# aexoden/snesimage

Measured on AMD Instinct MI355X. Metric: candidate palettes scored/sec, higher is better.
Workload: dtype f32

## Files before the change

### snesimage_amd/csrc/batch_host.inc

```

struct snesimage_batch {
    std::vector<snesimage_ctx *> ctx;
    int device = 0;
    hipStream_t stream = nullptr;
    static constexpr int kRing = 4;
    snes::BatchArgs *h_args[kRing] = {nullptr, nullptr, nullptr, nullptr}, *d_args[kRing] = {nullptr, nullptr, nullptr, nullptr};
    hipEvent_t used[kRing] = {nullptr, nullptr, nullptr, nullptr};
    uint64_t calls = 0;
    bool busy = false, dead = false;
};

namespace {

int32_t batch_quiesce(snesimage_batch *b) {
    if (b && b->busy) { HIPCHK(hipStreamSynchronize(b->stream)); b->busy = false; }
    return SNES_OK;
}

snes::PrepParams make_prep(snesimage_ctx *c, int mode, int sp, int si) {
    snes::PrepParams P{};
    P.orig = c->d_target; P.tile_pal = c->d_tile_pal; P.pal_rgb8 = c->d_pal_rgb8; P.map = c->d_map; P.pack = c->d_pack; P.packT = c->d_packT; P.packC4 = c->d_packC4; P.packR4 = c->d_packR4;
    P.subC4 = c->d_subC4; P.subR4 = c->d_subR4; P.labpx = c->d_labpx_t; P.pal_lab = c->d_pal_lab;
    P.W = (int)c->W; P.H = (int)c->H; P.sub_size = (int)c->sub_size; P.ncol = c->ncol; P.mode = mode; P.sp = sp; P.si = si; P.perceptual = c->perceptual ? 1 : 0;
    return P;
// ... 16 lines not shown
        auto &sp = c->sp;
        const uint32_t j0 = c->sub_size > 1 ? (index + 1u) % c->sub_size : index;
        a.bcolor = c->d_colors + 3 * (size_t)(palette * c->sub_size + j0); a.btab = sp.cand_tab + 8 * (size_t)(sp.lanes * sp.cap);
        a.win_pack = sp.dpack; a.zero = sp.plist_count; a.nzero = 1;
        DitherParams D{};
        D.orig = c->d_orig; D.tile_pal = c->d_tile_pal; D.pal_rgb8 = c->d_pal_rgb8; D.W = (int)c->W; D.H = (int)c->H; D.sub_size = (int)c->sub_size; D.ncol = c->ncol; D.slot_ci = sp.slot_ci;
        a.Db = D; a.Db.cand_tab = a.btab; a.Db.maps = sp.bmap; a.Db.mapsC4 = sp.bmapC4; a.Db.rec_pack = sp.dpack; a.Db.ck_out = sp.ckd;
        a.Db.excl_sub = (int)palette; a.Db.excl_si = (int)index; a.Db.excl_j0 = (int)j0;
        a.Dc = D; a.Dc.cand_tab = sp.cand_tab; a.Dc.maps = const_cast<uint8_t *>(a.Pc.maps); a.Dc.mapsC4 = const_cast<uint8_t *>(a.Pc.mapsC4);
        a.Dc.first_group = sp.first; a.Dc.first_k0 = 0; a.Dc.rec_in = c->dither_rec ? sp.dpack : nullptr; a.Dc.ck_in = sp.ckd; a.Dc.bmap = sp.bmap; a.Dc.bmapC4 = sp.bmapC4; a.Dc.order = sp.lpt ? sp.order : nullptr;
        if (c->perceptual) {
            a.Db.pal_lab = c->d_pal_lab; a.Db.cand_lab = sp.cand_lab + 3 * (size_t)(sp.lanes * sp.cap); a.Db.lab_eotf = c->d_lab_eotf; a.Db.perceptual = 1; a.Db.rec_lab = sp.rec_lab;
            a.Dc.pal_lab = c->d_pal_lab; a.Dc.cand_lab = sp.cand_lab; a.Dc.lab_eotf = c->d_lab_eotf; a.Dc.perceptual = 1;
        }
    }
    a.method = (int)method; a.n = (int)n; a.slot = (int)(palette * c->sub_size + index); a.channel = (int)channel; a.nes = method == SNES_METHOD_NES ? 1 : 0; a.npx = (int)c->npx;
    return SNES_OK;
}

struct BatchSide { hipStream_t stream; hipEvent_t in, h, v, narrow; bool whole; hipStream_t aux = nullptr; hipEvent_t a_scan = nullptr, a_h0 = nullptr, a_v0 = nullptr; };
int32_t enqueue_batched_scoring(hipStream_t st, const snes::BatchArgs *A, uint32_t K, uint32_t n, snesimage_ctx *c0, const BatchSide *side = nullptr, const int *dead = nullptr, bool member_packs = false) {
    const Geom &G = c0->G;
    const unsigned npx_blocks = (unsigned)((c0->npx + 255) / 256);
    const int s_first = sparse_params(c0, 0).s_first;
    hipStream_t bs = side && side->stream ? side->stream : st;
    const bool split = bs != st;
    const bool dith = c0->dither;
    const bool sub16 = c0->sub_size == 16;
    const bool sub15 = c0->sub_size == 15;
    const bool whole = split && side->whole;
    hipStream_t ps = whole ? bs : st;
    const int *bdead = whole ? nullptr : dead;
    if (!dith) hipLaunchKernelGGL(kb_prep, dim3(npx_blocks, 1, K), dim3(256), 0, ps, A, bdead);
    else {
        if (member_packs) hipLaunchKernelGGL(kb_prep, dim3(npx_blocks, 1, K), dim3(256), 0, ps, A, bdead);
        hipLaunchKernelGGL(kb_dither_prep, dim3(1, 1, K), dim3(64), 0, ps, A, bdead);
        if (c0->perceptual) hipLaunchKernelGGL(kb_dither_base_lab, dim3(1, 1, K), dim3(512), 0, ps, A, bdead);
        else if (sub15) hipLaunchKernelGGL(kb_dither_base<15>, dim3(1, 1, K), dim3(512), 0, ps, A, bdead);
        else if (sub16) hipLaunchKernelGGL(kb_dither_base<16>, dim3(1, 1, K), dim3(512), 0, ps, A, bdead);
        else hipLaunchKernelGGL(kb_dither_base<0>, dim3(1, 1, K), dim3(512), 0, ps, A, bdead);
    }
    hipLaunchKernelGGL(kb_build_plist, dim3(npx_blocks, 1, K), dim3(256), 0, ps, A, bdead);
    hipLaunchKernelGGL(kb_base_down, dim3(down_grid(G), 1, K), dim3(256), 0, ps, A, bdead);
    if (split) { HIPCHK(hipEventRecord(side->in, ps)); HIPCHK(hipStreamWaitEvent(whole ? st : bs, side->in, 0)); }
    const bool quad = (size_t)n * K <= c0->sp.h2q_max;
    if (quad) hipLaunchKernelGGL(kb_sparse_h2q_base, dim3((unsigned)((G.sh[0] / 4 * 3 + 3) / 4), (unsigned)(s_first * kColBuckets), K), dim3(64), h2_lds(c0), bs, A, bdead);
    else hipLaunchKernelGGL(kb_sparse_h2_base, dim3((unsigned)((G.sh[0] / 4 * 3 + 15) / 16), (unsigned)(s_first * kColBuckets), K), dim3(64), h2_lds(c0), bs, A, bdead);
    if (split) HIPCHK(hipEventRecord(side->h, bs));
    if (s_first > 0 && c0->sp.vsplit) hipLaunchKernelGGL(kb_sparse_v_base_split, dim3((unsigned)(G.W >> 6), (unsigned)(3 * s_first), K), dim3(128), 0, bs, A, bdead);
    else if (s_first > 0) hipLaunchKernelGGL(kb_sparse_v_base, dim3(3, (unsigned)s_first, K), dim3(256), 0, bs, A, bdead);
    if (split) HIPCHK(hipEventRecord(side->v, bs));
    if (s_first < G.nscales) hipLaunchKernelGGL(kb_sparse_h, dim3((unsigned)((G.sh[s_first] / 4 * 3 + 15) / 16), (unsigned)((G.nscales - s_first) * kColBuckets), K), dim3(64), 0, bs, A, 1, bdead);
    if (s_first < G.nscales) hipLaunchKernelGGL(kb_sparse_v_base_narrow, dim3(3, (unsigned)(G.nscales - s_first), K), dim3(256), 0, bs, A, bdead);
    if (split) HIPCHK(hipEventRecord(side->narrow, bs));
    hipLaunchKernelGGL(kb_candidate_tables, dim3((n + 63) / 64, 1, K), dim3(64), 0, st, A, dead);
    if (dith && c0->perceptual) {
        hipLaunchKernelGGL(kb_candidate_lab, dim3((n + 63) / 64, 1, K), dim3(64), 0, st, A, dead);
        hipLaunchKernelGGL(kb_dither_first_lab, dim3(n, 1, K), dim3(256), 0, st, A, dead);
        if (c0->sp.lpt) hipLaunchKernelGGL(kb_sparse_order, dim3(1, 1, K), dim3(1024), 0, st, A, dead);
        if (c0->dither4 && (size_t)n * K <= c0->dither4_max) hipLaunchKernelGGL(kb_dither_run4_lab, dim3(n, 1, K), dim3(512), 0, st, A, dead);
        else hipLaunchKernelGGL(kb_dither_run_lab, dim3(n, 1, K), dim3(128), 0, st, A, dead);
        hipLaunchKernelGGL(kb_dither_diff, dim3((n + 3) / 4, 1, K), dim3(1024), 0, st, A, dead);
    } else
    if (c0->perceptual) {
        hipLaunchKernelGGL(kb_candidate_lab, dim3((n + 63) / 64, 1, K), dim3(64), 0, st, A, dead);
        hipLaunchKernelGGL(kb_clear_bitmaps, dim3(64, 1, K), dim3(256), 0, st, A, dead);
        hipLaunchKernelGGL(kb_sparse_scan_lab, dim3(n, 1, K), dim3(256), 0, st, A, dead);
    } else if (dith) {
        hipLaunchKernelGGL(kb_dither_first, dim3((n + 15) / 16, 1, K), dim3(1024), 0, st, A, dead);
        if (c0->sp.lpt) hipLaunchKernelGGL(kb_sparse_order, dim3(1, 1, K), dim3(1024), 0, st, A, dead);
        const bool quad_fs = c0->dither4 && (size_t)n * K <= c0->dither4_max;
        if (quad_fs && sub15) hipLaunchKernelGGL(kb_dither_run4<15>, dim3(n, 1, K), dim3(512), 0, st, A, dead);
        else if (quad_fs && sub16) hipLaunchKernelGGL(kb_dither_run4<16>, dim3(n, 1, K), dim3(512), 0, st, A, dead);
        else if (quad_fs) hipLaunchKernelGGL(kb_dither_run4<0>, dim3(n, 1, K), dim3(512), 0, st, A, dead);
        else if (c0->ditherw && sub15) hipLaunchKernelGGL(kb_dither_runw<15>, dim3((n + 3) / 4, 1, K), dim3(256), 0, st, A, dead);
        else if (c0->ditherw && sub16) hipLaunchKernelGGL(kb_dither_runw<16>, dim3((n + 3) / 4, 1, K), dim3(256), 0, st, A, dead);
        else if (c0->ditherw && c0->sub_size > 1) hipLaunchKernelGGL(kb_dither_runw<0>, dim3((n + 3) / 4, 1, K), dim3(256), 0, st, A, dead);
        else if (sub15) hipLaunchKernelGGL(kb_dither_run<15>, dim3(n, 1, K), dim3(128), 0, st, A, dead);
        else if (sub16) hipLaunchKernelGGL(kb_dither_run<16>, dim3(n, 1, K), dim3(128), 0, st, A, dead);
        else hipLaunchKernelGGL(kb_dither_run<0>, dim3(n, 1, K), dim3(128), 0, st, A, dead);
        hipLaunchKernelGGL(kb_dither_diff, dim3((n + 3) / 4, 1, K), dim3(1024), 0, st, A, dead);
    } else if ((size_t)n * K <= c0->sp.scan4_max) hipLaunchKernelGGL(kb_sparse_scan4, dim3((n + 3) / 4, 1, K), dim3(1024), 0, st, A, dead);
    else hipLaunchKernelGGL(kb_sparse_scan, dim3((n + 15) / 16, 1, K), dim3(1024), 0, st, A, 0, dead);
    const bool two = side && side->aux && !quad && (size_t)n * K >= c0->sp.h0_min && c0->sp.h0_min > 0 && s_first > 0 && c0->sp.down1 && G.nscales > 2;
    if (two) {
        hipStream_t ax = side->aux;
        HIPCHK(hipEventRecord(side->a_scan, st)); HIPCHK(hipStreamWaitEvent(ax, side->a_scan, 0));
        if (split) HIPCHK(hipStreamWaitEvent(ax, side->h, 0));
        size_t gx = ((size_t)n * 8 * 3 + 15) / 16; if (gx > c0->sp.hgrid) gx = c0->sp.hgrid; if (gx < 8) gx = 8;
        hipLaunchKernelGGL(kb_sparse_h2_lists, dim3((unsigned)gx, (unsigned)kColBuckets, K), dim3(64), h2_lds(c0), ax, A, dead, 0);
        if (c0->sp.lpt) hipLaunchKernelGGL(kb_sparse_order, dim3(1, 1, K), dim3(1024), 0, ax, A, dead);
        HIPCHK(hipEventRecord(side->a_h0, ax));
        if (split) HIPCHK(hipStreamWaitEvent(ax, side->v, 0));
        hipLaunchKernelGGL(kb_sparse_v2_scales, dim3(n * 3, 1, K), dim3(256), 0, ax, A, dead, 0);
        HIPCHK(hipEventRecord(side->a_v0, ax));
    }
    if (c0->sp.down1 && G.nscales > 2) {
        hipLaunchKernelGGL(kb_sparse_down1, dim3(n * 8, 1, K), dim3(256), 0, st, A, dead);
        if (c0->sp.down_tiles && G.nscales >= 4) {
            unsigned gt = (n * (unsigned)(G.sh[3] / 4) + SNES_DOWN_TILES_U - 1) / SNES_DOWN_TILES_U; if (gt > c0->sp.tiles_grid) gt = c0->sp.tiles_grid;
            hipLaunchKernelGGL(kb_sparse_down_tiles, dim3(gt, 1, K), dim3(256), 0, st, A, dead);
        } else
        hipLaunchKernelGGL(kb_sparse_down, dim3(n, 1, K), dim3(256), 0, st, A, -2, dead);
    } else hipLaunchKernelGGL(kb_sparse_down, dim3(n, 1, K), dim3(256), 0, st, A, 0, dead);
    if (split) HIPCHK(hipStreamWaitEvent(st, side->h, 0));
    { size_t gx = ((size_t)n * 8 * 3 + 15) / 16; if (gx > c0->sp.hgrid) gx = c0->sp.hgrid; if (gx < 8) gx = 8;
      if (quad) hipLaunchKernelGGL(kb_sparse_h2q, dim3((unsigned)(gx * 4), (unsigned)(s_first * kColBuckets), K), dim3(64), h2_lds(c0), st, A, dead);
      else if (two) { if (s_first > 1) hipLaunchKernelGGL(kb_sparse_h2_lists, dim3((unsigned)gx, (unsigned)((s_first - 1) * kColBuckets), K), dim3(64), h2_lds(c0), st, A, dead, (int)kColBuckets); }
      else hipLaunchKernelGGL(kb_sparse_h2, dim3((unsigned)gx, (unsigned)(s_first * kColBuckets), K), dim3(64), h2_lds(c0), st, A, dead);
      if (s_first < G.nscales) hipLaunchKernelGGL(kb_sparse_h, dim3((unsigned)((gx + 7) / 8), (unsigned)((G.nscales - s_first) * kColBuckets), K), dim3(64), 0, st, A, 0, dead); }
    if (two) {
        HIPCHK(hipStreamWaitEvent(st, side->a_h0, 0));
        if (split) { HIPCHK(hipStreamWaitEvent(st, side->v, 0)); HIPCHK(hipStreamWaitEvent(st, side->narrow, 0)); }
        if (s_first < G.nscales) hipLaunchKernelGGL(kb_sparse_v, dim3((n * 3 + 7) / 8, (unsigned)(G.nscales - s_first), K), dim3(256), 0, st, A, dead);
        if (s_first > 1) hipLaunchKernelGGL(kb_sparse_v2_scales, dim3(n * 3, (unsigned)(s_first - 1), K), dim3(256), 0, st, A, dead, 1);
        HIPCHK(hipStreamWaitEvent(st, side->a_v0, 0));
    } else {
    if (c0->sp.lpt) hipLaunchKernelGGL(kb_sparse_order, dim3(1, 1, K), dim3(1024), 0, st, A, dead);
    if (split) HIPCHK(hipStreamWaitEvent(st, side->v, 0));
    hipLaunchKernelGGL(kb_sparse_v2, dim3(n * 3, (unsigned)s_first, K), dim3(256), 0, st, A, dead);
    if (split) HIPCHK(hipStreamWaitEvent(st, side->narrow, 0));
    if (s_first < G.nscales) hipLaunchKernelGGL(kb_sparse_v, dim3((n * 3 + 7) / 8, (unsigned)(G.nscales - s_first), K), dim3(256), 0, st, A, dead);
    }
    hipLaunchKernelGGL(kb_final_score, dim3((n + 3) / 4, 1, K), dim3(256), 0, st, A, dead);
    HIPCHK(hipGetLastError());
    return SNES_OK;
}

}

extern "C" {

void batch_forget(snesimage_batch *b, snesimage_ctx *c) {
    (void)batch_quiesce(b);
    for (auto *m : b->ctx) m->owner = nullptr;
    (void)c;
    b->dead = true;
}

int32_t snesimage_batch_create(snesimage_ctx **ctxs, uint32_t n, snesimage_batch **out) {
    if (!ctxs || !out || n == 0) return fail(SNES_ERR_ARG, "null pointer or empty batch");
    *out = nullptr;
    snesimage_ctx *c0 = ctxs[0];
    for (uint32_t i = 0; i < n; i++) {
        snesimage_ctx *c = ctxs[i];
        if (!c) return fail(SNES_ERR_ARG, "null context in batch");
        if (c->owner) return fail(SNES_ERR_STATE, "context already belongs to a batch");
        if (c->backdrop) return fail(SNES_ERR_UNSUPPORTED, kBackdropRefused);
        if (c->od_L > 1) return fail(SNES_ERR_ARG, kLevelsRefused);
        if (c->device != c0->device || c->W != c0->W || c->H != c0->H || c->sub_count != c0->sub_count || c->sub_size != c0->sub_size || c->chunk != c0->chunk)
            return fail(SNES_ERR_ARG, "contexts of a batch must share device, image size, palette geometry and chunk");
        if (c->perceptual != c0->perceptual) return fail(SNES_ERR_ARG, "contexts of a batch must share their flags");
        if (!c->sp.enabled || (c->dither && c->sub_size == 1)) return fail(SNES_ERR_UNSUPPORTED, "batched calls cover the group-sparse path (not with SNES_SPARSE=0), and with --dither subpalettes of two entries and more");
        if (c->dither != c0->dither) return fail(SNES_ERR_ARG, "contexts of a batch must share their flags");
        if (!ordered_tables_equal(c, c0)) return fail(SNES_ERR_ARG, "contexts of a batch must share their ordered-dither table");
    }
    std::unique_ptr<snesimage_batch> b(new snesimage_batch());
    b->device = c0->device;
    HIPCHK(hipSetDevice(b->device));
    for (uint32_t i = 0; i < n; i++) {
        snesimage_ctx *c = ctxs[i];
        CHECK(alloc_workspace(c, 1));
        CHECK(ensure_tables(c));
        CHECK(ensure_source(c));
        CHECK(sparse_alloc(c, c->chunk));
        CHECK(ensure_cand_capacity(c, c->chunk));
        if (!c->map_synced) CHECK(do_optimize(c));
        CHECK(ensure_incumbent(c));
    }
    for (uint32_t i = 0; i < n; i++) HIPCHK(hipStreamSynchronize(ctxs[i]->stream));
    HIPCHK(hipStreamCreateWithFlags(&b->stream, hipStreamNonBlocking));
    for (int r = 0; r < snesimage_batch::kRing; r++) {
        HIPCHK(hipHostMalloc(&b->h_args[r], sizeof(snes::BatchArgs) * n));
        HIPCHK(hipMalloc(&b->d_args[r], sizeof(snes::BatchArgs) * n));
        HIPCHK(hipEventCreateWithFlags(&b->used[r], hipEventDisableTiming));
    }
    b->ctx.assign(ctxs, ctxs + n);
    for (auto *c : b->ctx) c->owner = b.get();
    *out = b.release();
    return SNES_OK;
}

void snesimage_batch_destroy(snesimage_batch *b) {
    if (!b) return;
    (void)hipSetDevice(b->device);
    if (b->stream) (void)hipStreamSynchronize(b->stream);
    if (!b->dead) for (auto *c : b->ctx) c->owner = nullptr;
    for (int r = 0; r < snesimage_batch::kRing; r++) {
        if (b->h_args[r]) (void)hipHostFree(b->h_args[r]);
        if (b->d_args[r]) (void)hipFree(b->d_args[r]);
        if (b->used[r]) (void)hipEventDestroy(b->used[r]);
    }
    if (b->stream) (void)hipStreamDestroy(b->stream);
    delete b;
}

int32_t snesimage_batch_sync(snesimage_batch *b) {
    if (!b) return fail(SNES_ERR_ARG, "null batch");
    HIPCHK(hipSetDevice(b->device));
    return batch_quiesce(b);
}

}

namespace {

int32_t batch_call(snesimage_batch *b, uint32_t method, uint32_t palette, uint32_t index, uint32_t channel, const uint64_t *seeds, uint64_t step_id, uint32_t n_random, snes::StepResult *joint) {
    snesimage_ctx *c0 = b->ctx[0];
    CHECK(check_slot(c0, palette, index));
    if (method > 2 || channel > 2) return fail(SNES_ERR_ARG, "bad method or channel");
    const uint32_t n = method_count(method, n_random);
    if (n > c0->chunk) return fail(SNES_ERR_ARG, "a batched call holds at most `chunk` candidates per image");
    HIPCHK(hipSetDevice(b->device));
    const uint32_t K = (uint32_t)b->ctx.size();
    const int r = (int)(b->calls % snesimage_batch::kRing);
    if (b->calls >= (uint64_t)snesimage_batch::kRing) HIPCHK(hipEventSynchronize(b->used[r]));
    snes::BatchArgs *ha = b->h_args[r];
    for (uint32_t i = 0; i < K; i++) {
        snesimage_ctx *c = b->ctx[i];
        if (!c->tables_valid || !c->src_valid || !c->inc_valid) return fail(SNES_ERR_STATE, "a member context was modified outside the batch; call snesimage_batch_sync and recreate the batch");
        CHECK(fill_batch_args(ha[i], c, n, method, palette, index, channel, mix64(seeds[i] ^ (step_id * 0x9E3779B97F4A7C15ull) ^ 0xD1B54A32D192ED03ull)));
        if (n > c->cand_cap) return fail(SNES_ERR_STATE, "a member's candidate list is smaller than the call");
        if (c->dither) { ha[i].prep = make_prep(c, 1, -1, -1); ha[i].prep.zero = nullptr; ha[i].prep.nzero = 0; }
    }
    hipStream_t st = b->stream;
    if (!b->busy) for (auto *c : b->ctx) {
        if (!c->ev_own) HIPCHK(hipEventCreateWithFlags(&c->ev_own, hipEventDisableTiming));
        HIPCHK(hipEventRecord(c->ev_own, c->stream));
        HIPCHK(hipStreamWaitEvent(st, c->ev_own, 0));
    }
    const snes::BatchArgs *A = b->d_args[r];
    HIPCHK(hipMemcpyAsync(b->d_args[r], ha, sizeof(snes::BatchArgs) * K, hipMemcpyHostToDevice, st));
    HIPCHK(hipEventRecord(b->used[r], st));
    hipLaunchKernelGGL(kb_gen_candidates, dim3((n + 63) / 64, 1, K), dim3(64), 0, st, A, (const int *)nullptr);
    CHECK(enqueue_batched_scoring(st, A, K, n, c0, nullptr, nullptr, c0->dither));
    if (joint) hipLaunchKernelGGL(ks_commit, dim3(1), dim3(256), 0, st, A, (int)K, joint);
    else hipLaunchKernelGGL(kb_commit, dim3(1, 1, K), dim3(256), 0, st, A, (const int *)nullptr);
// ... 23 lines not shown
```

### snesimage_amd/csrc/capi.hip

```cpp
#include "../../include/snesimage_hip.h"
#include "kernels.hpp"
#include "kernels_opt.hpp"
#include "kernels_fast.hpp"
#include "kernels_sparse.hpp"
#include "kernels_sparse2.hpp"
#include "kernels_batch.hpp"
#include "kernels_shared.hpp"
#include "kernels_tile.hpp"
#include "kernels_level.hpp"
#include "kernels_char.hpp"
#include "kernels_char_set.hpp"

#include <hip/hip_runtime.h>

#include <atomic>
#include <cmath>
#include <cstdio>
#include <cstdlib>
#include <cstring>
#include <string>
#include <utility>
#include <memory>
#include <vector>

// ... 53 lines not shown
        lab_eotf[v] = x <= PALETTE_SRGB_THRESHOLD ? (float)(1.0 / PALETTE_SRGB_LINEAR_DIV_D) * x
                                                  : (float)std::pow((double)std::fmaf(x, (float)(1.0 / PALETTE_SRGB_SCALE_D), (float)(PALETTE_SRGB_OFFSET_D / PALETTE_SRGB_SCALE_D)), (double)PALETTE_SRGB_GAMMA);
    }
}

inline uint64_t mix64(uint64_t z) {
    z = (z ^ (z >> 30)) * 0xBF58476D1CE4E5B9ull;
    z = (z ^ (z >> 27)) * 0x94D049BB133111EBull;
    return z ^ (z >> 31);
}

template <typename T> void dfree(T *&p) { if (p) { (void)hipFree(p); p = nullptr; } }

std::atomic<int> g_fail_alloc_in{-1};
template <typename T> hipError_t dmalloc(T **p, size_t bytes) {
    int left = g_fail_alloc_in.load(std::memory_order_relaxed);
    while (left >= 0) {
        if (g_fail_alloc_in.compare_exchange_weak(left, left - 1, std::memory_order_relaxed)) { if (left == 0) { *p = nullptr; return hipErrorOutOfMemory; } break; }
    }
    return hipMalloc(p, bytes);
}
std::atomic<bool> g_poison_alloc{false};

}

struct snesimage_ctx {
    int device = 0;
    hipStream_t own_stream = nullptr, stream = nullptr;
    uint32_t W = 0, H = 0, sub_count = 0, sub_size = 0, flags = 0;
    int ncol = 0;
    bool dither = false, perceptual = false, nes = false;
    bool backdrop = false, tied_call = false; uint32_t user_size = 0;
    bool dither4 = true; uint32_t dither4_max = 512;
    bool ditherw = true;
    bool dither_rec = true;
    Geom G{};
    BlurK K{};
    size_t npx = 0, src_floats = 0;
    uint32_t chunk = 4096, chunk_alloc = 0;

    std::vector<uint8_t> h_orig; float h_eotf[256], h_lab_eotf[256];

    uint8_t *d_orig = nullptr, *d_tile_pal = nullptr, *d_colors = nullptr, *d_map = nullptr;
    unsigned long long *d_pack = nullptr, *d_packT = nullptr, *d_packC4 = nullptr, *d_packR4 = nullptr;
    float *d_img1C4 = nullptr, *d_mu1R4 = nullptr, *d_sd1R4 = nullptr, *d_a1 = nullptr, *d_a1R4 = nullptr; double *d_r1 = nullptr, *d_r1R4 = nullptr;
    int fast_mask = 0;
    float *d_eotf = nullptr, *d_lab_eotf = nullptr;
    uint32_t *d_pal_rgb8 = nullptr; float *d_pal_lin = nullptr, *d_pal_xyb = nullptr, *d_pal_lab = nullptr;
    float *d_lin0 = nullptr, *d_img1 = nullptr, *d_img1T = nullptr, *d_mu1 = nullptr, *d_sd1 = nullptr;
    float *d_labpx = nullptr, *d_labpxT = nullptr;
    uint8_t *d_target = nullptr, *d_target_own = nullptr; float *d_labpx_t = nullptr, *d_labpxT_t = nullptr, *d_labpx_t_own = nullptr, *d_labpxT_t_own = nullptr;
    uint32_t od_n = 0; int8_t od_tab[256] = {};
    uint32_t od_L = 0; int8_t od_bank[8 * 256] = {}; uint8_t od_level[1024] = {}; uint8_t *d_level = nullptr;
    struct snesimage_levelwork *lvl = nullptr;
    float *d_work = nullptr, *d_cand_tab = nullptr, *d_cand_lab = nullptr;
    double *d_part = nullptr;
    uint8_t *d_maps = nullptr, *d_mapsT = nullptr, *d_mapsC4 = nullptr, *d_mapsR4 = nullptr;
    uint8_t *d_subC4 = nullptr, *d_subR4 = nullptr;
    uint8_t *d_bestmap = nullptr, *d_bestmaps_all = nullptr; BestRec *d_bestrec = nullptr, *d_bestrecs_all = nullptr; int *d_skip = nullptr;
    uint4 *d_rplist = nullptr; int *d_rcount = nullptr;
    float *d_rtab = nullptr, *d_rlab = nullptr; uint32_t rtab_cap = 0;
    bool map_pending = false;
    bool best_valid = false, map_synced = false;
    struct Lane { hipStream_t stream = nullptr; float *d_work = nullptr, *d_cand_tab = nullptr, *d_cand_lab = nullptr; double *d_part = nullptr; uint8_t *d_maps = nullptr, *d_mapsT = nullptr, *d_mapsC4 = nullptr, *d_mapsR4 = nullptr, *d_bestmap = nullptr; BestRec *d_bestrec = nullptr; hipEvent_t done = nullptr; };
    std::vector<Lane> extra; uint32_t nlanes = 2; hipEvent_t ev_ready = nullptr;
    struct Sparse {
        bool lpt = true;
        bool down1 = true;
        bool counters_cleared = false;
        uint32_t h2q_max = 512;
        bool down_tiles = true;
        uint32_t h0_min = 1024;
        bool base_down_side = false;
        uint32_t h0_grid = 8192;
        hipStream_t h0_stream[8] = {}; hipEvent_t ev_scan[8] = {}, ev_h0[8] = {}, ev_hn[8] = {}, ev_vn[8] = {};
        bool v0_aside = true;
        hipEvent_t ev_v0[8] = {};
        bool vn_aside = true;
        uint32_t tiles_grid = 4096;
        uint32_t down1_grid = 32768;
        bool vsplit = true;
        uint32_t scan4_max = 2048;
        uint32_t hgrid = 8192;
        bool dedup = true; uint32_t dedup_min = 1024; int *holder = nullptr; bool holder_dirty = false;
        bool enabled = false, side = true; uint32_t min_n = 1; uint32_t cap = 0, lanes = 0;
        SparseGeom S{};
        float *store = nullptr, *cand_tab = nullptr, *cand_lab = nullptr, *ckf = nullptr, *ckh = nullptr; long long zeros_off = 0; uint32_t *bitmap = nullptr; double *cka = nullptr, *part = nullptr;
        CandMeta *meta = nullptr; unsigned int *items = nullptr; int *item_count = nullptr; long long item_stride = 0; int *order = nullptr, *first = nullptr;
        uint4 *plist = nullptr; int *plist_count = nullptr; bool plist_valid = false;
        hipStream_t base_stream = nullptr; hipEvent_t ev_base_in = nullptr, ev_base_h = nullptr, ev_base_done = nullptr, ev_base_narrow = nullptr;
        uint8_t *dmaps = nullptr, *dmapsC4 = nullptr;
        uint8_t *bmap = nullptr, *bmapC4 = nullptr, *bcand = nullptr; unsigned long long *dpack = nullptr; double *ckd = nullptr; uint32_t slot_ci = 0;
        float *rec_lab = nullptr;
        int base_sp = -1, base_si = -1;
        struct Ahead { uint8_t *bmap = nullptr, *bmapC4 = nullptr, *bcand = nullptr; unsigned long long *dpack = nullptr; double *ckd = nullptr; float *btab = nullptr, *blab = nullptr, *rec_lab = nullptr; int *ok = nullptr;
                       hipEvent_t ev = nullptr; bool on = true, have = false; int sp = -1, si = -1; unsigned long long epoch = 0; } ahead;
    } sp;
    uint8_t *d_cand = nullptr; uint32_t cand_cap = 0;
    uint8_t *d_cand_sel = nullptr;
    double *d_errs = nullptr, *d_errs_sel = nullptr;
    double *d_inc_err = nullptr;
    StepResult *d_last = nullptr;
    double *d_scratch_err = nullptr;
    uint8_t *d_dummy_cand = nullptr;
    KmeansWork km{};
    double *d_tile_cost = nullptr; int *d_tile_any = nullptr; unsigned int *d_tile_moved = nullptr;

    struct snesimage_batch *owner = nullptr;
    struct snesimage_group *group = nullptr;
    hipEvent_t ev_own = nullptr;
    struct snesimage_window *win = nullptr;
    bool win_pend = false;
    bool pack_borrowed = false;
    struct snesimage_tilework *tile = nullptr;
    struct snesimage_charwork *chr = nullptr;

    bool tables_valid = false, src_valid = false, inc_valid = false;
    unsigned long long epoch = 0; bool epoch_by_commit = false;
    int pack_mode = -1, pack_sp = -1, pack_si = -1; bool pack_valid = false;
    uint32_t pend_n = 0, pend_sp = 0, pend_si = 0, pend_method = 0; bool pend = false;

    int timing = 0;
    double t_ms[3] = {0.0, 0.0, 0.0}; uint64_t t_launches = 0, t_cands = 0;
    struct TimingRec { hipEvent_t ev[6]; uint32_t n; bool light; };
    std::vector<TimingRec> t_pending;
};

namespace {

int32_t alloc_lane(snesimage_ctx *c, uint32_t chunk, float *&d_work, float *&d_cand_tab, float *&d_cand_lab, double *&d_part, uint8_t *&d_maps, uint8_t *&d_mapsT, uint8_t *&d_mapsC4, uint8_t *&d_mapsR4) {
    dfree(d_work); dfree(d_cand_tab); dfree(d_cand_lab); dfree(d_part); dfree(d_maps); dfree(d_mapsT); dfree(d_mapsC4); dfree(d_mapsR4);
    HIPCHK(dmalloc(&d_work, sizeof(float) * (size_t)c->G.cand_stride * chunk));
    HIPCHK(dmalloc(&d_cand_tab, sizeof(float) * 8 * (size_t)chunk));
    HIPCHK(dmalloc(&d_cand_lab, sizeof(float) * 3 * (size_t)chunk));
    HIPCHK(dmalloc(&d_part, sizeof(double) * (size_t)chunk * kMaxScales * 18));
    if (c->dither) {
        HIPCHK(dmalloc(&d_maps, c->npx * (size_t)chunk));
        HIPCHK(dmalloc(&d_mapsT, c->npx * (size_t)chunk));
        HIPCHK(dmalloc(&d_mapsC4, c->npx * (size_t)chunk));
        HIPCHK(dmalloc(&d_mapsR4, c->npx * (size_t)chunk));
    }
    return SNES_OK;
}
int32_t alloc_workspace(snesimage_ctx *c, uint32_t chunk, uint32_t lanes = 1) {
    if (c->dither || c->perceptual) lanes = c->nlanes;
    if (lanes > c->nlanes) lanes = c->nlanes;
    if (lanes < c->extra.size() + 1) lanes = (uint32_t)c->extra.size() + 1;
    if (c->chunk_alloc >= chunk && c->extra.size() + 1 >= lanes) return SNES_OK;
    if (chunk < c->chunk_alloc) chunk = c->chunk_alloc;
    HIPCHK(hipStreamSynchronize(c->stream));
    for (auto &L : c->extra) HIPCHK(hipStreamSynchronize(L.stream));
    c->chunk_alloc = 0;
    CHECK(alloc_lane(c, chunk, c->d_work, c->d_cand_tab, c->d_cand_lab, c->d_part, c->d_maps, c->d_mapsT, c->d_mapsC4, c->d_mapsR4));
    if (!c->ev_ready) HIPCHK(hipEventCreateWithFlags(&c->ev_ready, hipEventDisableTiming));
    while (c->extra.size() + 1 < lanes) {
        snesimage_ctx::Lane L;
        HIPCHK(hipStreamCreateWithFlags(&L.stream, hipStreamNonBlocking));
        HIPCHK(hipEventCreateWithFlags(&L.done, hipEventDisableTiming));
        c->extra.push_back(L);
    }
    for (auto &L : c->extra) CHECK(alloc_lane(c, chunk, L.d_work, L.d_cand_tab, L.d_cand_lab, L.d_part, L.d_maps, L.d_mapsT, L.d_mapsC4, L.d_mapsR4));
    if (c->dither && !c->d_bestmaps_all) {
        HIPCHK(dmalloc(&c->d_bestmaps_all, c->npx * (size_t)c->nlanes));
        HIPCHK(dmalloc(&c->d_bestrecs_all, sizeof(BestRec) * c->nlanes));
        HIPCHK(dmalloc(&c->d_skip, sizeof(int)));
    }
// ... 222 lines not shown
        S.off_xybR[s] = off; off += 3 * N;
        S.off_hout[s] = off; off += 9 * N;
        S.off_ckf[s] = okf; okf += 3LL * (G.sh[s] / 4 + 2) * 18 * G.sw[s];
        S.off_cka[s] = oka; oka += 3LL * (G.sh[s] / 4 + 2) * 6 * G.sw[s];
        S.off_ckh[s] = okh; if (G.sw[s] >= 64) okh += 3LL * 3 * 18 * G.sh[s];
        S.goff[s] = go; go += G.sh[s] / 4;
    }
    S.cand_stride = off;
    const size_t ncap = (size_t)lanes * need + 1;
    sp.item_stride = (long long)need * (G.sh[0] / 4) * 3;
    HIPCHK(dmalloc(&sp.store, sizeof(float) * (size_t)S.cand_stride * ncap));
    if (g_poison_alloc.load()) HIPCHK(hipMemsetAsync(sp.store, 0xff, sizeof(float) * (size_t)S.cand_stride * ncap, c->stream));
    HIPCHK(dmalloc(&sp.cand_tab, sizeof(float) * 8 * ncap));
    if (c->perceptual) {
        dfree(sp.cand_lab); dfree(sp.bitmap);
        HIPCHK(dmalloc(&sp.cand_lab, sizeof(float) * 3 * ncap));
        HIPCHK(dmalloc(&sp.bitmap, sizeof(uint32_t) * (c->npx / 32) * ncap));
    }
    HIPCHK(dmalloc(&sp.ckf, sizeof(float) * (size_t)okf));
    dfree(sp.ckh); HIPCHK(dmalloc(&sp.ckh, sizeof(float) * (size_t)(okh + 12LL * G.W + 256)));
    sp.zeros_off = okh;
    HIPCHK(hipMemsetAsync(sp.ckh + okh, 0, sizeof(float) * 12 * (size_t)G.W, c->stream));
    HIPCHK(dmalloc(&sp.cka, sizeof(double) * (size_t)oka));
    HIPCHK(dmalloc(&sp.part, sizeof(double) * ncap * kMaxScales * 18));
    HIPCHK(dmalloc(&sp.meta, sizeof(CandMeta) * ncap));
    dfree(sp.order); HIPCHK(dmalloc(&sp.order, sizeof(int) * ncap));
    dfree(sp.first); HIPCHK(dmalloc(&sp.first, sizeof(int) * ncap));
    HIPCHK(dmalloc(&sp.items, sizeof(unsigned int) * (size_t)sp.item_stride * kItemLists * (c->nlanes + 1)));
    if (!sp.base_stream && sp.side) {
        int prio_lo = 0, prio_hi = 0;
        HIPCHK(hipDeviceGetStreamPriorityRange(&prio_lo, &prio_hi));
        HIPCHK(hipStreamCreateWithPriority(&sp.base_stream, hipStreamNonBlocking, prio_hi));
        HIPCHK(hipEventCreateWithFlags(&sp.ev_base_in, hipEventDisableTiming));
        HIPCHK(hipEventCreateWithFlags(&sp.ev_base_h, hipEventDisableTiming));
        HIPCHK(hipEventCreateWithFlags(&sp.ev_base_narrow, hipEventDisableTiming));
        HIPCHK(hipEventCreateWithFlags(&sp.ev_base_done, hipEventDisableTiming));
    }
    HIPCHK(dmalloc(&sp.item_count, sizeof(int) * (kItemLists * (c->nlanes + 1) + 1)));
    HIPCHK(hipMemsetAsync(sp.item_count, 0, sizeof(int) * (kItemLists * (c->nlanes + 1) + 1), c->stream));
    sp.plist_count = sp.item_count + (size_t)kItemLists * (c->nlanes + 1);
    sp.counters_cleared = true;
    HIPCHK(dmalloc(&sp.plist, sizeof(uint4) * c->npx));
    if (c->dither) {
        dfree(sp.dmaps); dfree(sp.dmapsC4); dfree(sp.bmap); dfree(sp.bmapC4); dfree(sp.bcand); dfree(sp.dpack); dfree(sp.ckd);
        HIPCHK(dmalloc(&sp.dmaps, c->npx * (size_t)need * lanes));
        HIPCHK(dmalloc(&sp.dmapsC4, c->npx * (size_t)need * lanes));
        HIPCHK(dmalloc(&sp.bmap, c->npx)); HIPCHK(dmalloc(&sp.bmapC4, c->npx)); HIPCHK(dmalloc(&sp.bcand, 64));
        HIPCHK(dmalloc(&sp.dpack, sizeof(unsigned long long) * c->npx));
        HIPCHK(dmalloc(&sp.ckd, sizeof(double) * 3 * c->W * (c->H / 4 + 1)));
        dfree(sp.rec_lab); if (c->perceptual) HIPCHK(dmalloc(&sp.rec_lab, sizeof(float) * 3 * c->npx));
        auto &ah = sp.ahead;
        dfree(ah.bmap); dfree(ah.bmapC4); dfree(ah.bcand); dfree(ah.dpack); dfree(ah.ckd); dfree(ah.btab); dfree(ah.blab); dfree(ah.rec_lab); dfree(ah.ok); ah.have = false;
        if (ah.on && sp.side && c->sub_size > 1) {
            HIPCHK(dmalloc(&ah.bmap, c->npx)); HIPCHK(dmalloc(&ah.bmapC4, c->npx)); HIPCHK(dmalloc(&ah.bcand, 64)); HIPCHK(dmalloc(&ah.btab, sizeof(float) * 8)); HIPCHK(dmalloc(&ah.ok, sizeof(int)));
            HIPCHK(dmalloc(&ah.dpack, sizeof(unsigned long long) * c->npx));
            HIPCHK(dmalloc(&ah.ckd, sizeof(double) * 3 * c->W * (c->H / 4 + 1)));
            if (c->perceptual) { HIPCHK(dmalloc(&ah.blab, sizeof(float) * 3)); HIPCHK(dmalloc(&ah.rec_lab, sizeof(float) * 3 * c->npx)); }
            if (!ah.ev) HIPCHK(hipEventCreateWithFlags(&ah.ev, hipEventDisableTiming));
        }
    }
    sp.cap = need; sp.lanes = lanes; sp.plist_valid = false;
    {
        SparseParams P = sparse_params(c, c->nlanes);
        P.is_base = 1; P.ncand = 1; P.k0 = P.base;
        hipLaunchKernelGGL(k_sparse_scan, dim3(1), dim3(1024), 0, c->stream, P);
        HIPCHK(hipGetLastError());
    }
    HIPCHK(hipStreamSynchronize(c->stream));
    return SNES_OK;
}

SparseParams sparse_params(snesimage_ctx *c, uint32_t lane) {
    auto &sp = c->sp;
    SparseParams P{};
    P.G = c->G; P.S = sp.S; P.K = c->K; P.ncol = c->ncol; P.base = (int)(sp.lanes * sp.cap);
    P.pack = c->d_pack; P.packC4 = c->d_packC4; P.packR4 = c->d_packR4; P.plist = sp.plist; P.plist_count = sp.plist_count;
    P.pal_lin = c->d_pal_lin; P.pal_xyb = c->d_pal_xyb; P.cand_tab = sp.cand_tab;
    P.perceptual = c->perceptual ? 1 : 0; P.labpx = c->d_labpx_t; P.cand_lab = sp.cand_lab; P.bitmap = sp.bitmap;
    P.img1C4 = c->d_img1C4; P.mu1R4 = c->d_mu1R4; P.sd1R4 = c->d_sd1R4; P.a1R4 = c->d_a1R4; P.r1R4 = c->d_r1R4;
    P.store = sp.store; P.meta = sp.meta;
    P.items = sp.items + (size_t)lane * sp.item_stride * kItemLists; P.item_count = sp.item_count + (size_t)lane * kItemLists; P.item_stride = sp.item_stride;
    P.ckf = sp.ckf; P.cka = sp.cka; P.part = sp.part; P.first = sp.first; P.ckh = sp.ckh; P.zeros = sp.ckh + sp.zeros_off; P.trash = sp.ckh + sp.zeros_off + 12LL * c->G.W;
    for (P.s_first = 0; P.s_first < c->G.nscales && c->G.sw[P.s_first] >= 64; P.s_first++) {}
    if (c->dither) {
        const uint32_t l = lane < c->nlanes ? lane : 0;
        P.use_maps = 1; P.sub_size = (int)c->sub_size; P.slot_ci = sp.slot_ci; P.subC4 = c->d_subC4; P.tile_pal = c->d_tile_pal;
        P.perceptual = 0; P.labpx = sp.rec_lab;
        P.maps = sp.dmaps + (size_t)l * sp.cap * c->npx; P.mapsC4 = sp.dmapsC4 + (size_t)l * sp.cap * c->npx; P.bmap = sp.bmap; P.bmapC4 = sp.bmapC4;
    }
    return P;
}

static size_t h2_lds(const snesimage_ctx *c) { return sizeof(float) * 3 * (size_t)(c->ncol + 2); }

int32_t sparse_base_pass(snesimage_ctx *c, int sp_idx, int si, uint32_t n_cand) {
    auto &sp = c->sp;
    const Geom &G = c->G;
    if (!sp.plist_valid) {
        if (!sp.counters_cleared) HIPCHK(hipMemsetAsync(sp.plist_count, 0, sizeof(int), c->stream));
        sp.counters_cleared = false;
        const unsigned long long *win_pack = c->d_pack;
        if (c->dither) {
            const uint32_t j0 = c->sub_size > 1 ? ((uint32_t)si + 1u) % c->sub_size : (uint32_t)si;
            sp.slot_ci = (uint32_t)(sp_idx * (int)c->sub_size + si);
            auto &ah = sp.ahead;
            const int *b_done = nullptr;
            const bool same_state = ah.epoch == c->epoch;
            if (ah.have && ah.sp == sp_idx && ah.si == si && (same_state || (ah.epoch + 1 == c->epoch && c->epoch_by_commit))) {
                std::swap(sp.bmap, ah.bmap); std::swap(sp.bmapC4, ah.bmapC4); std::swap(sp.dpack, ah.dpack); std::swap(sp.ckd, ah.ckd); std::swap(sp.rec_lab, ah.rec_lab);
                hipLaunchKernelGGL(k_ahead_ok, dim3(1), dim3(1), 0, c->stream, same_state ? (const StepResult *)nullptr : c->d_last, ah.ok);
                HIPCHK(hipStreamWaitEvent(c->stream, ah.ev, 0));
                b_done = ah.ok;
            }
            ah.have = false;
            HIPCHK(hipMemcpyAsync(sp.bcand, c->d_colors + 3 * (size_t)(sp_idx * (int)c->sub_size + (int)j0), 3, hipMemcpyDeviceToDevice, c->stream));
            float *btab = sp.cand_tab + 8 * (size_t)(sp.lanes * sp.cap);
            hipLaunchKernelGGL(k_candidate_tables, dim3(1), dim3(64), 0, c->stream, sp.bcand, 1, c->d_eotf, btab);
            DitherParams Dp{};
            Dp.orig = c->d_orig; Dp.tile_pal = c->d_tile_pal; Dp.pal_rgb8 = c->d_pal_rgb8; Dp.cand_tab = btab; Dp.maps = sp.bmap; Dp.mapsC4 = sp.bmapC4;
            Dp.W = (int)c->W; Dp.H = (int)c->H; Dp.sub_size = (int)c->sub_size; Dp.ncol = c->ncol; Dp.slot_ci = sp.slot_ci;
            Dp.rec_pack = sp.dpack; Dp.ck_out = sp.ckd; Dp.excl_sub = sp_idx; Dp.excl_si = si; Dp.excl_j0 = (int)j0; Dp.skip = b_done;
            if (c->perceptual) {
                float *blab = sp.cand_lab + 3 * (size_t)(sp.lanes * sp.cap);
                hipLaunchKernelGGL(k_candidate_lab, dim3(1), dim3(64), 0, c->stream, btab, 1, c->d_lab_eotf, blab);
                Dp.pal_lab = c->d_pal_lab; Dp.cand_lab = blab; Dp.lab_eotf = c->d_lab_eotf; Dp.perceptual = 1; Dp.rec_lab = sp.rec_lab;
                if (c->dither4) hipLaunchKernelGGL((k_dither4_lab<1>), dim3(1), dim3(512), 0, c->stream, Dp); else hipLaunchKernelGGL((k_dither<true, 0, 1>), dim3(1), dim3(128), 0, c->stream, Dp);
            } else
            if (c->dither4 && c->sub_size == 15) hipLaunchKernelGGL((k_dither4<15, 1>), dim3(1), dim3(512), 0, c->stream, Dp);
            else if (c->dither4 && c->sub_size == 16) hipLaunchKernelGGL((k_dither4<16, 1>), dim3(1), dim3(512), 0, c->stream, Dp);
            else if (c->dither4) hipLaunchKernelGGL((k_dither4<0, 1>), dim3(1), dim3(512), 0, c->stream, Dp);
            else if (c->sub_size == 15) hipLaunchKernelGGL((k_dither<false, 15, 1>), dim3(1), dim3(128), 0, c->stream, Dp);
            else if (c->sub_size == 16) hipLaunchKernelGGL((k_dither<false, 16, 1>), dim3(1), dim3(128), 0, c->stream, Dp);
            else hipLaunchKernelGGL((k_dither<false, 0, 1>), dim3(1), dim3(128), 0, c->stream, Dp);
            win_pack = sp.dpack;
        }
        hipLaunchKernelGGL(k_build_plist, dim3((unsigned)((c->npx + 255) / 256)), dim3(256), 0, c->stream, win_pack, (int)c->npx, sp.plist, sp.plist_count);
        SparseParams P = sparse_params(c, c->nlanes);
        P.is_base = 1; P.ncand = 1; P.k0 = P.base;
        hipStream_t bs = sp.side ? sp.base_stream : c->stream;
        const bool down_with_sweeps = sp.side && n_cand >= sp.h0_min && sp.h0_min > 0;
        sp.base_down_side = down_with_sweeps;
        if (!down_with_sweeps) hipLaunchKernelGGL(k_base_down, dim3(down_grid(G)), dim3(256), 0, c->stream, P);
        if (sp.side) { HIPCHK(hipEventRecord(sp.ev_base_in, c->stream)); HIPCHK(hipStreamWaitEvent(bs, sp.ev_base_in, 0)); }
        if (down_with_sweeps) hipLaunchKernelGGL(k_base_down, dim3(down_grid(G)), dim3(256), 0, bs, P);
        if (sp.h2q_max > 0) hipLaunchKernelGGL(k_sparse_h2q_base, dim3((unsigned)((G.sh[0] / 4 * 3 + 3) / 4), (unsigned)(P.s_first * kColBuckets)), dim3(64), h2_lds(c), bs, P);
        else hipLaunchKernelGGL(k_sparse_h2_base, dim3((unsigned)((G.sh[0] / 4 * 3 + 15) / 16), (unsigned)(P.s_first * kColBuckets)), dim3(64), h2_lds(c), bs, P);
        if (sp.side) HIPCHK(hipEventRecord(sp.ev_base_h, bs));
        if (P.s_first > 0 && sp.vsplit) hipLaunchKernelGGL(k_sparse_v2_base_split, dim3((unsigned)(G.W >> 6), 3, (unsigned)P.s_first), dim3(128), 0, bs, P);
        else if (P.s_first > 0) hipLaunchKernelGGL(k_sparse_v2_base, dim3(3, (unsigned)P.s_first), dim3(256), 0, bs, P);
        if (sp.side) HIPCHK(hipEventRecord(sp.ev_base_done, bs));
        if (P.s_first < G.nscales) hipLaunchKernelGGL(k_sparse_h, dim3((unsigned)((G.sh[P.s_first] / 4 * 3 + 15) / 16), (unsigned)((G.nscales - P.s_first) * kColBuckets)), dim3(64), 0, bs, P);
        if (P.s_first < G.nscales) hipLaunchKernelGGL(k_sparse_v_base_narrow, dim3(3, (unsigned)(G.nscales - P.s_first)), dim3(256), 0, bs, P);
        HIPCHK(hipGetLastError());
        if (sp.side) HIPCHK(hipEventRecord(sp.ev_base_narrow, bs));
        if (c->dither && sp.side && sp.ahead.dpack) {
            auto &ah = sp.ahead;
            int ni = si + 1, np = sp_idx;
            if (ni == (int)c->sub_size) { ni = 0; np = (np + 1) % (int)c->sub_count; }
            const int nj0 = (ni + 1) % (int)c->sub_size;
            HIPCHK(hipMemcpyAsync(ah.bcand, c->d_colors + 3 * (size_t)(np * (int)c->sub_size + nj0), 3, hipMemcpyDeviceToDevice, bs));
            hipLaunchKernelGGL(k_candidate_tables, dim3(1), dim3(64), 0, bs, ah.bcand, 1, c->d_eotf, ah.btab);
            DitherParams Dn{};
            Dn.orig = c->d_orig; Dn.tile_pal = c->d_tile_pal; Dn.pal_rgb8 = c->d_pal_rgb8; Dn.cand_tab = ah.btab; Dn.maps = ah.bmap; Dn.mapsC4 = ah.bmapC4;
            Dn.W = (int)c->W; Dn.H = (int)c->H; Dn.sub_size = (int)c->sub_size; Dn.ncol = c->ncol; Dn.slot_ci = (uint32_t)(np * (int)c->sub_size + ni);
            Dn.rec_pack = ah.dpack; Dn.ck_out = ah.ckd; Dn.excl_sub = np; Dn.excl_si = ni; Dn.excl_j0 = nj0;
            if (c->perceptual) {
                hipLaunchKernelGGL(k_candidate_lab, dim3(1), dim3(64), 0, bs, ah.btab, 1, c->d_lab_eotf, ah.blab);
                Dn.pal_lab = c->d_pal_lab; Dn.cand_lab = ah.blab; Dn.lab_eotf = c->d_lab_eotf; Dn.perceptual = 1; Dn.rec_lab = ah.rec_lab;
                if (c->dither4) hipLaunchKernelGGL((k_dither4_lab<1>), dim3(1), dim3(512), 0, bs, Dn); else hipLaunchKernelGGL((k_dither<true, 0, 1>), dim3(1), dim3(128), 0, bs, Dn);
            } else
            if (c->dither4 && c->sub_size == 15) hipLaunchKernelGGL((k_dither4<15, 1>), dim3(1), dim3(512), 0, bs, Dn);
            else if (c->dither4 && c->sub_size == 16) hipLaunchKernelGGL((k_dither4<16, 1>), dim3(1), dim3(512), 0, bs, Dn);
            else if (c->dither4) hipLaunchKernelGGL((k_dither4<0, 1>), dim3(1), dim3(512), 0, bs, Dn);
            else if (c->sub_size == 15) hipLaunchKernelGGL((k_dither<false, 15, 1>), dim3(1), dim3(128), 0, bs, Dn);
            else if (c->sub_size == 16) hipLaunchKernelGGL((k_dither<false, 16, 1>), dim3(1), dim3(128), 0, bs, Dn);
            else hipLaunchKernelGGL((k_dither<false, 0, 1>), dim3(1), dim3(128), 0, bs, Dn);
            HIPCHK(hipGetLastError());
            HIPCHK(hipEventRecord(ah.ev, bs));
            ah.have = true; ah.sp = np; ah.si = ni; ah.epoch = c->epoch;
        }
        sp.plist_valid = true;
    }
    return SNES_OK;
}

int32_t sparse_score_chunk(snesimage_ctx *c, uint32_t lane, hipStream_t stream, const uint8_t *d_rgb5, uint32_t nc, double *d_errors, int err_stride, int err_offset, int list0 = -1) {
    auto &sp = c->sp;
    const Geom &G = c->G;
    SparseParams P = sparse_params(c, lane);
    P.is_base = 0; P.ncand = (int)nc; P.k0 = (int)(lane * sp.cap);
    if (list0 >= 0) { P.holder = sp.holder; P.list0 = list0; }
    snesimage_ctx::TimingRec tr{}; tr.n = nc;
    if (c->timing) { for (int i = 0; i < 6; i++) HIPCHK(hipEventCreate(&tr.ev[i])); if (c->timing == 1) HIPCHK(hipEventRecord(tr.ev[0], stream)); }
    if (list0 >= 0) hipLaunchKernelGGL(k_candidate_tables_mark, dim3((nc + 63) / 64), dim3(64), 0, stream, d_rgb5, (int)nc, c->d_eotf, sp.cand_tab + 8 * (size_t)P.k0, sp.holder, list0);
    else
    hipLaunchKernelGGL(k_candidate_tables, dim3((nc + 63) / 64), dim3(64), 0, stream, d_rgb5, (int)nc, c->d_eotf, sp.cand_tab + 8 * (size_t)P.k0);
    if (c->dither) {
        if (c->perceptual) {
            hipLaunchKernelGGL(k_candidate_lab, dim3((nc + 63) / 64), dim3(64), 0, stream, sp.cand_tab + 8 * (size_t)P.k0, (int)nc, c->d_lab_eotf, sp.cand_lab + 3 * (size_t)P.k0);
            hipLaunchKernelGGL(k_dither_first_lab, dim3(nc), dim3(256), 0, stream, P);
        } else
        hipLaunchKernelGGL(k_dither_first, dim3((nc + 15) / 16), dim3(1024), 0, stream, P);
        DitherParams Dp{};
        Dp.orig = c->d_orig; Dp.tile_pal = c->d_tile_pal; Dp.pal_rgb8 = c->d_pal_rgb8; Dp.cand_tab = sp.cand_tab + 8 * (size_t)P.k0;
        Dp.maps = const_cast<uint8_t *>(P.maps); Dp.mapsC4 = const_cast<uint8_t *>(P.mapsC4);
        Dp.W = (int)c->W; Dp.H = (int)c->H; Dp.sub_size = (int)c->sub_size; Dp.ncol = c->ncol; Dp.slot_ci = sp.slot_ci;
        Dp.first_group = sp.first; Dp.first_k0 = P.k0; Dp.ck_in = sp.ckd; Dp.bmap = sp.bmap; Dp.bmapC4 = sp.bmapC4; Dp.rec_in = c->dither_rec ? sp.dpack : nullptr;
        if (c->sp.lpt) {
            hipLaunchKernelGGL(k_sparse_order, dim3(1), dim3(1024), 0, stream, P, sp.order + P.k0); Dp.order = sp.order + P.k0;
        }
        if (c->perceptual) {
            Dp.pal_lab = c->d_pal_lab; Dp.cand_lab = sp.cand_lab + 3 * (size_t)P.k0; Dp.lab_eotf = c->d_lab_eotf; Dp.perceptual = 1;
            if (c->dither4 && nc <= c->dither4_max) hipLaunchKernelGGL((k_dither4_lab<2>), dim3(nc), dim3(512), 0, stream, Dp); else hipLaunchKernelGGL((k_dither<true, 0, 2>), dim3(nc), dim3(128), 0, stream, Dp);
        } else
        if (c->dither4 && nc <= c->dither4_max && c->sub_size == 15) hipLaunchKernelGGL((k_dither4<15, 2>), dim3(nc), dim3(512), 0, stream, Dp);
        else if (c->dither4 && nc <= c->dither4_max && c->sub_size == 16) hipLaunchKernelGGL((k_dither4<16, 2>), dim3(nc), dim3(512), 0, stream, Dp);
        else if (c->dither4 && nc <= c->dither4_max) hipLaunchKernelGGL((k_dither4<0, 2>), dim3(nc), dim3(512), 0, stream, Dp);
        else if (c->ditherw && c->sub_size == 15) hipLaunchKernelGGL((k_ditherw<15>), dim3((nc + 3) / 4), dim3(256), 0, stream, Dp, (int)nc);
        else if (c->ditherw && c->sub_size == 16) hipLaunchKernelGGL((k_ditherw<16>), dim3((nc + 3) / 4), dim3(256), 0, stream, Dp, (int)nc);
        else if (c->ditherw && c->sub_size > 1) hipLaunchKernelGGL((k_ditherw<0>), dim3((nc + 3) / 4), dim3(256), 0, stream, Dp, (int)nc);
        else if (c->sub_size == 15) hipLaunchKernelGGL((k_dither<false, 15, 2>), dim3(nc), dim3(128), 0, stream, Dp);
        else if (c->sub_size == 16) hipLaunchKernelGGL((k_dither<false, 16, 2>), dim3(nc), dim3(128), 0, stream, Dp);
        else hipLaunchKernelGGL((k_dither<false, 0, 2>), dim3(nc), dim3(128), 0, stream, Dp);
        hipLaunchKernelGGL(k_dither_diff, dim3((nc + 3) / 4), dim3(1024), 0, stream, P);
    } else if (c->perceptual) {
        hipLaunchKernelGGL(k_candidate_lab, dim3((nc + 63) / 64), dim3(64), 0, stream, sp.cand_tab + 8 * (size_t)P.k0, (int)nc, c->d_lab_eotf, sp.cand_lab + 3 * (size_t)P.k0);
        HIPCHK(hipMemsetAsync(sp.bitmap + (size_t)P.k0 * (c->npx / 32), 0, sizeof(uint32_t) * (c->npx / 32) * nc, stream));
        hipLaunchKernelGGL(k_sparse_scan_lab, dim3(nc), dim3(256), 0, stream, P);
    } else if (nc <= sp.scan4_max) hipLaunchKernelGGL(k_sparse_scan4, dim3((nc + 3) / 4), dim3(1024), 0, stream, P);
    else hipLaunchKernelGGL(k_sparse_scan, dim3((nc + 15) / 16), dim3(1024), 0, stream, P);
    bool vn_aside = false;
    const bool h0_ahead = sp.side && sp.h0_min > 0 && nc >= sp.h0_min && nc > sp.h2q_max && lane < 8 && P.s_first > 0;
    const bool v0_aside = h0_ahead && sp.v0_aside;
    vn_aside = h0_ahead && !v0_aside && sp.vn_aside && P.s_first < G.nscales;
    if (c->sp.lpt && nc > 512) P.order = sp.order + P.k0;
    if (h0_ahead) {
        if (!sp.h0_stream[lane]) {
            HIPCHK(hipStreamCreateWithFlags(&sp.h0_stream[lane], hipStreamNonBlocking));
            HIPCHK(hipEventCreateWithFlags(&sp.ev_scan[lane], hipEventDisableTiming));
            HIPCHK(hipEventCreateWithFlags(&sp.ev_h0[lane], hipEventDisableTiming));
            HIPCHK(hipEventCreateWithFlags(&sp.ev_hn[lane], hipEventDisableTiming));
            HIPCHK(hipEventCreateWithFlags(&sp.ev_v0[lane], hipEventDisableTiming));
            HIPCHK(hipEventCreateWithFlags(&sp.ev_vn[lane], hipEventDisableTiming));
        }
        hipStream_t hs = sp.h0_stream[lane];
        HIPCHK(hipEventRecord(sp.ev_scan[lane], stream));
        HIPCHK(hipStreamWaitEvent(hs, sp.ev_scan[lane], 0));
        HIPCHK(hipStreamWaitEvent(hs, sp.ev_base_h, 0));
        size_t gx = ((size_t)nc * (G.sh[0] / 4) * 3 + 15) / 16; if (gx > sp.h0_grid) gx = sp.h0_grid;
        hipLaunchKernelGGL(k_sparse_h2, dim3((unsigned)gx, (unsigned)kColBuckets), dim3(64), h2_lds(c), hs, P);
        if (c->sp.lpt) hipLaunchKernelGGL(k_sparse_order, dim3(1), dim3(1024), 0, hs, P, sp.order + P.k0);
        HIPCHK(hipEventRecord(sp.ev_h0[lane], hs));
        if (v0_aside) {
            HIPCHK(hipStreamWaitEvent(hs, sp.ev_base_done, 0));
            if (c->timing) HIPCHK(hipEventRecord(tr.ev[3], hs));
            hipLaunchKernelGGL(k_sparse_v2, dim3(nc * 3, 1), dim3(256), 0, hs, P);
            if (c->timing) HIPCHK(hipEventRecord(tr.ev[4], hs));
            HIPCHK(hipEventRecord(sp.ev_v0[lane], hs));
        }
    }
    if (sp.down1 && G.nscales > 2) {
        size_t gd = (size_t)nc * 8; if (gd > sp.down1_grid) gd = sp.down1_grid;
        hipLaunchKernelGGL(k_sparse_down1, dim3((unsigned)gd), dim3(256), 0, stream, P);
        if (sp.side && sp.base_down_side) HIPCHK(hipStreamWaitEvent(stream, sp.ev_base_h, 0));
        if (sp.down_tiles && G.nscales >= 4) {
            size_t gt = ((size_t)nc * (G.sh[3] / 4) + SNES_DOWN_TILES_U - 1) / SNES_DOWN_TILES_U; if (gt > sp.tiles_grid) gt = sp.tiles_grid;
            hipLaunchKernelGGL(k_sparse_down_tiles, dim3((unsigned)gt), dim3(256), 0, stream, P);
        } else
        hipLaunchKernelGGL(k_sparse_down, dim3(nc), dim3(256), 0, stream, P, -2);
    } else { if (sp.side && sp.base_down_side) HIPCHK(hipStreamWaitEvent(stream, sp.ev_base_h, 0)); hipLaunchKernelGGL(k_sparse_down, dim3(nc), dim3(256), 0, stream, P, 0); }
    if (sp.side && !sp.base_down_side) HIPCHK(hipStreamWaitEvent(stream, sp.ev_base_h, 0));
    if (c->timing == 1) HIPCHK(hipEventRecord(tr.ev[1], stream));
    { size_t gx = ((size_t)nc * (G.sh[0] / 4) * 3 + 15) / 16; if (gx > sp.hgrid) gx = sp.hgrid;
      if (nc <= sp.h2q_max) {
          size_t gq = ((size_t)nc * (G.sh[0] / 4) * 3 + 3) / 4; if (gq > sp.hgrid) gq = sp.hgrid;
          hipLaunchKernelGGL(k_sparse_h2q, dim3((unsigned)gq, (unsigned)(P.s_first * kColBuckets)), dim3(64), h2_lds(c), stream, P);
      } else
      if (h0_ahead) { if (P.s_first > 1) hipLaunchKernelGGL(k_sparse_h2_from, dim3((unsigned)gx, (unsigned)((P.s_first - 1) * kColBuckets)), dim3(64), h2_lds(c), stream, P, (int)kColBuckets); }
      else
      hipLaunchKernelGGL(k_sparse_h2, dim3((unsigned)gx, (unsigned)(P.s_first * kColBuckets)), dim3(64), h2_lds(c), stream, P);
      if (P.s_first < G.nscales) hipLaunchKernelGGL(k_sparse_h, dim3((unsigned)((gx + 7) / 8), (unsigned)((G.nscales - P.s_first) * kColBuckets)), dim3(64), 0, stream, P);
      if (vn_aside) HIPCHK(hipEventRecord(sp.ev_hn[lane], stream));
      if (h0_ahead) HIPCHK(hipStreamWaitEvent(stream, sp.ev_h0[lane], 0)); }
    if (c->timing == 1) HIPCHK(hipEventRecord(tr.ev[2], stream));
    if (sp.side || stream != c->stream) HIPCHK(hipStreamWaitEvent(stream, sp.side ? sp.ev_base_done : c->ev_ready, 0));
    if (c->sp.lpt && nc > 512) {
        if (!h0_ahead) hipLaunchKernelGGL(k_sparse_order, dim3(1), dim3(1024), 0, stream, P, sp.order + P.k0);
        P.order = sp.order + P.k0;
    }
    if (vn_aside) {
        hipStream_t hs = sp.h0_stream[lane];
        HIPCHK(hipStreamWaitEvent(hs, sp.ev_hn[lane], 0));
        HIPCHK(hipStreamWaitEvent(hs, sp.ev_base_narrow, 0));
        hipLaunchKernelGGL(k_sparse_v, dim3((nc * 3 + 7) / 8, (unsigned)(G.nscales - P.s_first)), dim3(256), 0, hs, P);
        HIPCHK(hipEventRecord(sp.ev_vn[lane], hs));
    }
    if (v0_aside) {
        if (sp.side) HIPCHK(hipStreamWaitEvent(stream, sp.ev_base_narrow, 0));
        if (P.s_first < G.nscales) hipLaunchKernelGGL(k_sparse_v, dim3((nc * 3 + 7) / 8, (unsigned)(G.nscales - P.s_first)), dim3(256), 0, stream, P);
        if (P.s_first > 1) hipLaunchKernelGGL(k_sparse_v2_from, dim3(nc * 3, (unsigned)(P.s_first - 1)), dim3(256), 0, stream, P, 1);
    } else {
    if (c->timing) HIPCHK(hipEventRecord(tr.ev[3], stream));
    hipLaunchKernelGGL(k_sparse_v2, dim3(nc * 3, (unsigned)P.s_first), dim3(256), 0, stream, P);
    if (c->timing) HIPCHK(hipEventRecord(tr.ev[4], stream));
    }
    if (vn_aside) HIPCHK(hipStreamWaitEvent(stream, sp.ev_vn[lane], 0));
    else if (!v0_aside) {
    if (sp.side) HIPCHK(hipStreamWaitEvent(stream, sp.ev_base_narrow, 0));
    if (P.s_first < G.nscales) hipLaunchKernelGGL(k_sparse_v, dim3((nc * 3 + 7) / 8, (unsigned)(G.nscales - P.s_first)), dim3(256), 0, stream, P);
    }
    if (v0_aside) HIPCHK(hipStreamWaitEvent(stream, sp.ev_v0[lane], 0));
    hipLaunchKernelGGL(k_final_score_wave, dim3((nc + 3) / 4), dim3(256), 0, stream, sp.part + (size_t)P.k0 * G.nscales * 18, (int)nc, G, d_errors, err_stride, err_offset, P.item_count, (int)kItemLists);
    if (c->dither) {
        uint8_t *bm = lane == 0 ? c->d_bestmap : c->extra[lane - 1].d_bestmap; BestRec *br = lane == 0 ? c->d_bestrec : c->extra[lane - 1].d_bestrec;
        hipLaunchKernelGGL(k_keep_best, dim3(1), dim3(1024), 0, stream, d_errors, err_stride, err_offset, (int)nc, P.maps, (int)c->npx, br, bm);
    }
    HIPCHK(hipGetLastError());
    if (c->timing) { tr.light = c->timing != 1; if (!tr.light) HIPCHK(hipEventRecord(tr.ev[5], stream)); c->t_pending.push_back(tr); }
    return SNES_OK;
}

struct LaneScope {
    snesimage_ctx *c; snesimage_ctx::Lane *L;
    LaneScope(snesimage_ctx *c_, snesimage_ctx::Lane *L_) : c(c_), L(L_) { swap(); }
    ~LaneScope() { swap(); }
    void swap() { std::swap(c->stream, L->stream); std::swap(c->d_work, L->d_work); std::swap(c->d_cand_tab, L->d_cand_tab); std::swap(c->d_cand_lab, L->d_cand_lab);
                  std::swap(c->d_part, L->d_part); std::swap(c->d_maps, L->d_maps); std::swap(c->d_mapsT, L->d_mapsT); std::swap(c->d_mapsC4, L->d_mapsC4); std::swap(c->d_mapsR4, L->d_mapsR4);
                  std::swap(c->d_bestmap, L->d_bestmap); std::swap(c->d_bestrec, L->d_bestrec); }
};

int32_t score_list(snesimage_ctx *c, const uint8_t *d_rgb5, uint32_t n, double *d_errors, int err_stride, int err_offset, int sp, int si, uint8_t *d_maps_out) {
    uint32_t chunk = (c->dither || c->perceptual) ? (n + c->nlanes - 1) / c->nlanes : n;
    if (chunk < 64) chunk = 64;
    if (chunk > c->chunk) chunk = c->chunk;
    if (c->tied_call && chunk > 1024) chunk = 1024;
    const bool sparse = c->sp.enabled && !c->tied_call && !d_maps_out && sp >= 0 && n >= c->sp.min_n && c->pack_mode == (c->dither ? 1 : 2) && !(c->dither && c->sub_size == 1);
    const uint32_t nchunks = (n + chunk - 1) / chunk;
    const uint32_t nl = nchunks < c->nlanes ? nchunks : c->nlanes;
    CHECK(alloc_workspace(c, sparse ? 1 : chunk, nl));
    CHECK(ensure_tables(c));
    CHECK(ensure_source(c));
    if (sparse) {
        CHECK(sparse_alloc(c, chunk, nl));
        if (c->dither && (c->sp.base_sp != sp || c->sp.base_si != si)) c->sp.plist_valid = false;
        CHECK(sparse_base_pass(c, sp, si, n));
        c->sp.base_sp = sp; c->sp.base_si = si;
    }
    if (c->dither) { hipLaunchKernelGGL(k_reset_best, dim3(1), dim3(64), 0, c->stream, c->d_bestrecs_all, (int)c->nlanes); c->best_valid = true; }
    const bool dedup = sparse && !c->dither && c->sp.dedup && n >= c->sp.dedup_min;
    if (dedup) {
        if (!c->sp.holder) { HIPCHK(dmalloc(&c->sp.holder, sizeof(int) * kDedupColours)); c->sp.holder_dirty = true; }
        if (c->sp.holder_dirty) {
            HIPCHK(hipStreamSynchronize(c->stream));
            for (auto &L : c->extra) HIPCHK(hipStreamSynchronize(L.stream));
            HIPCHK(hipMemsetAsync(c->sp.holder, kNoHolder & 0xff, sizeof(int) * kDedupColours, c->stream));
        }
        c->sp.holder_dirty = true;
    }
    if (nl > 1) {
        HIPCHK(hipEventRecord(c->ev_ready, c->stream));
        for (uint32_t l = 1; l < nl; l++) HIPCHK(hipStreamWaitEvent(c->extra[l - 1].stream, c->ev_ready, 0));
    }
    uint32_t i = 0;
    for (uint32_t c0 = 0; c0 < n; c0 += chunk, i++) {
        const uint32_t nc = (n - c0 < chunk) ? (n - c0) : chunk;
        const uint32_t lane = i % nl;
        uint8_t *mo = d_maps_out ? d_maps_out + (size_t)c0 * c->npx : nullptr;
        const int eo = err_offset + (int)c0 * err_stride;
        if (sparse) { CHECK(sparse_score_chunk(c, lane, lane == 0 ? c->stream : c->extra[lane - 1].stream, d_rgb5 + 3 * (size_t)c0, nc, d_errors, err_stride, eo, dedup ? (int)c0 : -1)); continue; }
        if (lane == 0) CHECK(score_chunk(c, d_rgb5 + 3 * (size_t)c0, nc, d_errors, err_stride, eo, sp, si, mo));
        else { LaneScope ls(c, &c->extra[lane - 1]); CHECK(score_chunk(c, d_rgb5 + 3 * (size_t)c0, nc, d_errors, err_stride, eo, sp, si, mo)); }
    }
    for (uint32_t l = 1; l < nl; l++) {
        HIPCHK(hipEventRecord(c->extra[l - 1].done, c->extra[l - 1].stream));
        HIPCHK(hipStreamWaitEvent(c->stream, c->extra[l - 1].done, 0));
    }
    if (dedup) {
        hipLaunchKernelGGL(k_dedup_copy, dim3(1), dim3(1024), 0, c->stream, d_rgb5, (int)n, c->sp.holder, d_errors, err_stride, err_offset);
        HIPCHK(hipGetLastError());
        c->sp.holder_dirty = false;
    }
    return SNES_OK;
}

int32_t ensure_map(snesimage_ctx *c);

// ... 117 lines not shown
    if (c->d_skip) {
        hipLaunchKernelGGL(k_take_best_map, dim3(1), dim3(1024), 0, c->stream, c->d_last, c->d_bestrecs_all, c->best_valid ? (int)c->nlanes : 0, c->d_bestmaps_all, (int)c->npx,
                           c->map_synced ? 1 : 0, c->d_map, c->d_skip);
        may_skip = true;
    }
    c->best_valid = false;
    CHECK(do_optimize(c, may_skip));
    c->inc_valid = was_synced;
    return SNES_OK;
}

}

#include "kmeans_host.inc"

namespace {
int32_t write_backdrop(snesimage_ctx *c, const uint8_t *b) {
    CHECK(ensure_map(c));
    for (uint32_t p = 0; p < c->sub_count; p++)
        HIPCHK(hipMemcpyAsync(c->d_colors + 3 * ((size_t)p * c->sub_size + c->user_size), b, 3, hipMemcpyHostToDevice, c->stream));
    HIPCHK(hipStreamSynchronize(c->stream));
    c->tables_valid = false; c->pack_valid = false; c->inc_valid = false; c->map_synced = false; c->epoch++; c->epoch_by_commit = false;
    return SNES_OK;
}
int32_t read_colors(snesimage_ctx *c, uint8_t *all ) {
    HIPCHK(hipMemcpyAsync(all, c->d_colors, 3 * (size_t)c->ncol, hipMemcpyDeviceToHost, c->stream));
    HIPCHK(hipStreamSynchronize(c->stream));
    return SNES_OK;
}
}

extern "C" {

const char *snesimage_last_error(void) { return g_err.c_str(); }
#ifndef SNES_SRC_HASH
#define SNES_SRC_HASH "unknown"
#endif
const char *snesimage_version(void) { return "snesimage_hip 0.3.0 (gfx950) src:" SNES_SRC_HASH; }

int32_t snesimage_create(const uint8_t *rgba, uint32_t w, uint32_t h, uint32_t sub_count, uint32_t sub_size, uint32_t flags, int32_t device, snesimage_ctx **out) {
    if (!rgba || !out) return fail(SNES_ERR_ARG, "null pointer");
    *out = nullptr;
    if (w != 256) return fail(SNES_ERR_ARG, "image width must be 256 (tile stride is fixed at 32, lib.rs:58)");
    if (h < 8 || h > 256 || (h % 8) != 0) return fail(SNES_ERR_ARG, "image height must be a multiple of 8 in [8,256]");
    if (sub_count < 1 || sub_size < 1 || sub_count > 253 || sub_size > 253 || sub_count * sub_size > 253) return fail(SNES_ERR_ARG, "sub_count*sub_size must be in [1,253]");
    const bool backdrop = (flags & SNES_BACKDROP) != 0;
    if (backdrop && (sub_size > 15 || sub_count * (sub_size + 1) > 253)) return fail(SNES_ERR_ARG, "with SNES_BACKDROP sub_size must be at most 15 and sub_count*(sub_size+1) at most 253");
    if (device < 0) return fail(SNES_ERR_ARG, "device must be a HIP device ordinal >= 0 (this library has no CPU path)");
    int ndev = 0;
    HIPCHK(hipGetDeviceCount(&ndev));
    if (device >= ndev) return fail(SNES_ERR_ARG, "no such HIP device");
    HIPCHK(hipSetDevice(device));
    snesimage_ctx *c = new snesimage_ctx();
    c->backdrop = backdrop; c->user_size = sub_size;
    if (backdrop) sub_size += 1;
    c->device = device; c->W = w; c->H = h; c->sub_count = sub_count; c->sub_size = sub_size; c->flags = flags; c->ncol = (int)(sub_count * sub_size);
    c->dither = flags & SNES_DITHER; c->perceptual = flags & SNES_PERCEPTUAL; c->nes = flags & SNES_NES;
    c->npx = (size_t)w * h;
    c->K = make_blur_constants();
    if (const char *e = getenv("SNES_CHUNK")) { int v = atoi(e); if (v > 0) c->chunk = (uint32_t)v; }
    if (const char *e = getenv("SNES_LANES")) { int v = atoi(e); if (v >= 1 && v <= 8) c->nlanes = (uint32_t)v; }
    c->sp.enabled = true;
    if (const char *e = getenv("SNES_SPARSE")) c->sp.enabled = c->sp.enabled && atoi(e) != 0;
    if (const char *e = getenv("SNES_BASE_STREAM")) c->sp.side = atoi(e) != 0;
    if (const char *e = getenv("SNES_LPT")) c->sp.lpt = atoi(e) != 0;
    if (const char *e = getenv("SNES_DOWN1")) c->sp.down1 = atoi(e) != 0;
    if (const char *e = getenv("SNES_DITHER4")) c->dither4 = atoi(e) != 0;
    if (const char *e = getenv("SNES_DITHERW")) c->ditherw = atoi(e) != 0;
    if (const char *e = getenv("SNES_DITHER_AHEAD")) c->sp.ahead.on = atoi(e) != 0;
    if (const char *e = getenv("SNES_DITHER_REC")) c->dither_rec = atoi(e) != 0;
    if (const char *e = getenv("SNES_DITHER4_MAX")) { int v = atoi(e); if (v >= 0) c->dither4_max = (uint32_t)v; }
    if (const char *e = getenv("SNES_DOWN1_GRID")) { int v = atoi(e); if (v >= 64) c->sp.down1_grid = (uint32_t)v; }
    if (const char *e = getenv("SNES_VSPLIT")) c->sp.vsplit = atoi(e) != 0;
    if (const char *e = getenv("SNES_DOWN_TILES")) c->sp.down_tiles = atoi(e) != 0;
    if (const char *e = getenv("SNES_V0_ASIDE")) c->sp.v0_aside = atoi(e) != 0;
    if (const char *e = getenv("SNES_VN_ASIDE")) c->sp.vn_aside = atoi(e) != 0;
    if (const char *e = getenv("SNES_H0_GRID")) { int v = atoi(e); if (v >= 16) c->sp.h0_grid = (uint32_t)v; }
    if (const char *e = getenv("SNES_H0_MIN")) { int v = atoi(e); if (v >= 0) c->sp.h0_min = (uint32_t)v; }
    if (const char *e = getenv("SNES_TILES_GRID")) { int v = atoi(e); if (v >= 64) c->sp.tiles_grid = (uint32_t)v; }
    if (const char *e = getenv("SNES_SCAN4_MAX")) { int v = atoi(e); if (v >= 0) c->sp.scan4_max = (uint32_t)v; }
    if (const char *e = getenv("SNES_H2Q_MAX")) { int v = atoi(e); if (v >= 0) c->sp.h2q_max = (uint32_t)v; }
    if (const char *e = getenv("SNES_HGRID")) { int v = atoi(e); if (v >= 1) c->sp.hgrid = (uint32_t)v; }
    if (const char *e = getenv("SNES_SPARSE_MIN")) { int v = atoi(e); if (v >= 1) c->sp.min_n = (uint32_t)v; }
    if (const char *e = getenv("SNES_DEDUP")) c->sp.dedup = atoi(e) != 0;
    if (const char *e = getenv("SNES_DEDUP_MIN")) { int v = atoi(e); if (v >= 1) c->sp.dedup_min = (uint32_t)v; }
    Geom &G = c->G;
    G.W = (int)w; G.H = (int)h; G.nscales = 0;
    int P2 = 8;
    while (P2 < (int)h) P2 *= 2;
    for (int s = 0; s < kMaxScales; s++) {
        if (s > 0 && (G.sw[s - 1] < 8 || G.th[s - 1] < 8)) break;
        G.sw[s] = (int)w >> s; G.th[s] = s == 0 ? (int)h : (G.th[s - 1] + 1) / 2; G.sh[s] = s == 0 ? (int)h : P2 >> s; G.nscales = s + 1;
    }
    long long off = 0, soff = 0;
    for (int s = 0; s < G.nscales; s++) {
        long long N = (long long)G.sw[s] * G.sh[s];
        G.src_off[s] = soff; soff += 3 * N;
        if (s >= 1) { G.off_xyb[s] = off; off += 3 * N; G.off_xybT[s] = off; off += 3 * N; } else { G.off_xyb[s] = 0; G.off_xybT[s] = 0; }
        G.off_hout[s] = off; off += 9 * N;
    }
    G.cand_stride = off;
    for (int s = 0; s < G.nscales; s++) if ((G.sw[s] % 64) == 0 && (G.th[s] % 64) == 0 && G.th[s] == G.sh[s]) c->fast_mask |= 1 << s;
    if (const char *e = getenv("SNES_NO_FAST")) { if (atoi(e)) c->fast_mask = 0; }
    c->src_floats = (size_t)soff;

    int32_t rc = SNES_OK;
    auto body = [&]() -> int32_t {
        HIPCHK(hipStreamCreateWithFlags(&c->own_stream, hipStreamNonBlocking));
        c->stream = c->own_stream;
        HIPCHK(hipMalloc(&c->d_orig, c->npx * 4));
        HIPCHK(hipMalloc(&c->d_tile_pal, 1024));
        HIPCHK(hipMalloc(&c->d_colors, 3 * 256));
        HIPCHK(hipMalloc(&c->d_map, c->npx));
        HIPCHK(hipMalloc(&c->d_pack, c->npx * 8));
        HIPCHK(hipMalloc(&c->d_packT, c->npx * 8));
        HIPCHK(hipMalloc(&c->d_packC4, c->npx * 8));
        HIPCHK(hipMalloc(&c->d_packR4, c->npx * 8));
        if (c->dither) { HIPCHK(hipMalloc(&c->d_subC4, c->npx)); HIPCHK(hipMalloc(&c->d_subR4, c->npx)); }
        HIPCHK(hipMalloc(&c->d_eotf, 256 * 4));
        HIPCHK(hipMalloc(&c->d_lab_eotf, 256 * 4));
        HIPCHK(hipMalloc(&c->d_pal_rgb8, 256 * 4));
        HIPCHK(hipMalloc(&c->d_pal_lin, 256 * 3 * 4));
        HIPCHK(hipMalloc(&c->d_pal_xyb, 256 * 3 * 4));
        HIPCHK(hipMalloc(&c->d_pal_lab, 256 * 3 * 4));
        HIPCHK(hipMalloc(&c->d_lin0, c->npx * 3 * 4));
        HIPCHK(hipMalloc(&c->d_img1, c->src_floats * 4));
        HIPCHK(hipMalloc(&c->d_img1T, c->src_floats * 4));
        HIPCHK(hipMalloc(&c->d_mu1, c->src_floats * 4));
        HIPCHK(hipMalloc(&c->d_sd1, c->src_floats * 4));
        HIPCHK(hipMalloc(&c->d_a1, c->src_floats * 4));
        HIPCHK(hipMalloc(&c->d_a1R4, c->src_floats * 4));
        HIPCHK(hipMalloc(&c->d_r1, c->src_floats * 8));
        HIPCHK(hipMalloc(&c->d_r1R4, c->src_floats * 8));
        HIPCHK(hipMalloc(&c->d_img1C4, c->src_floats * 4));
        HIPCHK(hipMalloc(&c->d_mu1R4, c->src_floats * 4));
        HIPCHK(hipMalloc(&c->d_sd1R4, c->src_floats * 4));
        if (c->perceptual) { HIPCHK(hipMalloc(&c->d_labpx, c->npx * 3 * 4)); HIPCHK(hipMalloc(&c->d_labpxT, c->npx * 3 * 4)); }
        c->d_target = c->d_orig; c->d_labpx_t = c->d_labpx; c->d_labpxT_t = c->d_labpxT;
        HIPCHK(hipMalloc(&c->d_inc_err, sizeof(double)));
        HIPCHK(hipMalloc(&c->d_scratch_err, sizeof(double)));
        HIPCHK(hipMalloc(&c->d_last, sizeof(StepResult)));
        HIPCHK(hipMalloc(&c->d_dummy_cand, 64));
        HIPCHK(hipMemsetAsync(c->d_dummy_cand, 0, 64, c->stream));
        HIPCHK(hipMemsetAsync(c->d_last, 0, sizeof(StepResult), c->stream));
        HIPCHK(hipMemcpyAsync(c->d_orig, rgba, c->npx * 4, hipMemcpyHostToDevice, c->stream));
        HIPCHK(hipMemsetAsync(c->d_tile_pal, 0, 1024, c->stream));
        HIPCHK(hipMemsetAsync(c->d_colors, 0, 3 * 256, c->stream));
        HIPCHK(hipMemsetAsync(c->d_map, 0, c->npx, c->stream));
        c->h_orig.assign(rgba, rgba + c->npx * 4);
        make_eotf_tables(c->h_eotf, c->h_lab_eotf);
        HIPCHK(hipMemcpyAsync(c->d_eotf, c->h_eotf, sizeof(c->h_eotf), hipMemcpyHostToDevice, c->stream));
        HIPCHK(hipMemcpyAsync(c->d_lab_eotf, c->h_lab_eotf, sizeof(c->h_lab_eotf), hipMemcpyHostToDevice, c->stream));
        HIPCHK(hipStreamSynchronize(c->stream));
        CHECK(ensure_cand_capacity(c, 64));
        if (c->backdrop) {
            unsigned long long sum[3] = {0, 0, 0}, cnt = 0;
            for (size_t px = 0; px < c->npx; px++)
                if (rgba[4 * px + 3] != 0) { sum[0] += rgba[4 * px]; sum[1] += rgba[4 * px + 1]; sum[2] += rgba[4 * px + 2]; cnt++; }
            uint8_t b[3] = {0, 0, 0};
            if (cnt) for (int ch = 0; ch < 3; ch++) b[ch] = (uint8_t)(((sum[ch] + cnt / 2) / cnt) >> 3);
            if (c->nes) { uint8_t raw[3] = {b[0], b[1], b[2]}; host_new_nes_only(raw, c->perceptual, c->h_lab_eotf, b); }
            CHECK(write_backdrop(c, b));
        }
        return SNES_OK;
    };
    rc = body();
// ... 482 lines not shown
```

### snesimage_amd/csrc/kernels_batch.hpp

```cpp
#pragma once
#include "kernels_sparse2.hpp"

namespace snes {

struct BatchArgs {
    SparseParams Pc, Pb;
    PrepParams prep;
    unsigned long long key; const uint8_t *colors_in; uint8_t *colors; uint8_t *cand; const float *eotf; float *cand_tab;
    const double *part; double *errors; double *inc_err; StepResult *last; PaletteTables T;
    int method, n, slot, channel, nes, npx;
    const float *lab_eotf; float *cand_lab;
    DitherParams Db, Dc; const unsigned long long *win_pack; const uint8_t *bcolor; float *btab; int *zero; int nzero; uint8_t *map;
    int dead_base;
};

#define SNES_BATCH_IMG if (dead && *dead >= A[0].dead_base) return; const BatchArgs &a = A[blockIdx.z]
struct BatchBlock { int img, x, y; };
__device__ __forceinline__ BatchBlock batch_block() {
    BatchBlock b;
    const int X = (int)gridDim.x, Y = (int)gridDim.y, K = (int)gridDim.z;
    const int per = X * Y, K8 = K & ~7;
    const int L = (int)blockIdx.x + X * ((int)blockIdx.y + Y * (int)blockIdx.z);
    int rem;
    if (L < per * K8) { const int idx = L >> 3; b.img = (L & 7) + 8 * (idx / per); rem = idx % per; }
    else { const int L2 = L - per * K8; b.img = K8 + L2 / per; rem = L2 % per; }
    b.x = rem % X; b.y = rem / X;
    return b;
}
#define SNES_BATCH_XCD if (dead && *dead >= A[0].dead_base) return; const BatchBlock bb = batch_block(); const BatchArgs &a = A[bb.img]
__global__ void kb_gen_candidates(const BatchArgs *__restrict__ A, const int *__restrict__ dead) { SNES_BATCH_IMG; gen_candidates_body(a.method, a.n, a.key, a.colors_in, a.slot, a.channel, a.cand, 0, 1, nullptr, nullptr); }
__global__ __launch_bounds__(256) void kb_prep(const BatchArgs *__restrict__ A, const int *__restrict__ dead) { SNES_BATCH_IMG; prep_body(a.prep); }
__global__ __launch_bounds__(256) void kb_build_plist(const BatchArgs *__restrict__ A, const int *__restrict__ dead) {
    SNES_BATCH_IMG;
    build_plist_body(a.win_pack ? a.win_pack : a.Pb.pack, a.npx, const_cast<uint4 *>(a.Pb.plist), const_cast<int *>(a.Pb.plist_count));
}
__global__ void kb_dither_prep(const BatchArgs *__restrict__ A, const int *__restrict__ dead) {
    SNES_BATCH_IMG;
    if ((int)threadIdx.x < a.nzero) a.zero[threadIdx.x] = 0;
    candidate_tables_body(a.bcolor, 1, a.eotf, a.btab);
    if (a.Db.perceptual) candidate_lab_body(a.btab, 1, a.lab_eotf, const_cast<float *>(a.Db.cand_lab));
}
template <int SUB> __global__ __launch_bounds__(512) void kb_dither_base(const BatchArgs *__restrict__ A, const int *__restrict__ dead) { SNES_BATCH_IMG; dither4_body<SUB, 1>(a.Db, 0); }
__global__ __launch_bounds__(512) void kb_dither_base_lab(const BatchArgs *__restrict__ A, const int *__restrict__ dead) { SNES_BATCH_IMG; dither4_body<0, 1, true>(a.Db, 0); }
__global__ __launch_bounds__(256) void kb_dither_first_lab(const BatchArgs *__restrict__ A, const int *__restrict__ dead) { SNES_BATCH_IMG; if ((int)blockIdx.x < a.n) dither_first_lab_body(a.Pc); }
__global__ __launch_bounds__(512) void kb_dither_run4_lab(const BatchArgs *__restrict__ A, const int *__restrict__ dead) { SNES_BATCH_IMG; if ((int)blockIdx.x < a.n) dither4_body<0, 2, true>(a.Dc, (int)blockIdx.x); }
__global__ __launch_bounds__(128) void kb_dither_run_lab(const BatchArgs *__restrict__ A, const int *__restrict__ dead) { SNES_BATCH_IMG; if ((int)blockIdx.x < a.n) dither_body<true, 0, 2>(a.Dc, (int)blockIdx.x); }
__global__ __launch_bounds__(1024) void kb_dither_first(const BatchArgs *__restrict__ A, const int *__restrict__ dead) { SNES_BATCH_IMG; dither_first_body(a.Pc); }
template <int SUB> __global__ __launch_bounds__(512) void kb_dither_run4(const BatchArgs *__restrict__ A, const int *__restrict__ dead) { SNES_BATCH_IMG; if ((int)blockIdx.x < a.n) dither4_body<SUB, 2>(a.Dc, (int)blockIdx.x); }
template <int SUB> __global__ __launch_bounds__(128) void kb_dither_run(const BatchArgs *__restrict__ A, const int *__restrict__ dead) { SNES_BATCH_IMG; if ((int)blockIdx.x < a.n) dither_body<false, SUB, 2>(a.Dc, (int)blockIdx.x); }
template <int SUB> __global__ __launch_bounds__(256) void kb_dither_runw(const BatchArgs *__restrict__ A, const int *__restrict__ dead) { SNES_BATCH_IMG; ditherw_body<SUB>(a.Dc, (int)blockIdx.x, a.n); }
__global__ __launch_bounds__(1024) void kb_dither_diff(const BatchArgs *__restrict__ A, const int *__restrict__ dead) { SNES_BATCH_IMG; dither_diff_body(a.Pc); }
__global__ __launch_bounds__(1024) void kb_sparse_scan(const BatchArgs *__restrict__ A, int base, const int *__restrict__ dead) { SNES_BATCH_IMG; sparse_scan_body<1>(base ? a.Pb : a.Pc); }
__global__ __launch_bounds__(1024) void kb_sparse_scan4(const BatchArgs *__restrict__ A, const int *__restrict__ dead) { SNES_BATCH_IMG; sparse_scan_body<4>(a.Pc); }
__global__ __launch_bounds__(256) void kb_base_down(const BatchArgs *__restrict__ A, const int *__restrict__ dead) { SNES_BATCH_IMG; base_down_body(a.Pb); }
__global__ __launch_bounds__(256) void kb_sparse_down(const BatchArgs *__restrict__ A, int only_scale, const int *__restrict__ dead) { SNES_BATCH_XCD; sparse_down_body(a.Pc, only_scale, bb.x); }
__global__ __launch_bounds__(256) void kb_sparse_down_tiles(const BatchArgs *__restrict__ A, const int *__restrict__ dead) { SNES_BATCH_XCD; sparse_down_tiles_body<SNES_DOWN_TILES_U>(a.Pc, bb.x, (int)gridDim.x); }
__global__ __launch_bounds__(256) void kb_sparse_down1(const BatchArgs *__restrict__ A, const int *__restrict__ dead) { SNES_BATCH_XCD; sparse_down1_body(a.Pc, bb.x, (int)gridDim.x); }
__global__ void kb_candidate_tables(const BatchArgs *__restrict__ A, const int *__restrict__ dead) { SNES_BATCH_IMG; candidate_tables_body(a.cand, a.n, a.eotf, a.cand_tab); }
__global__ void kb_candidate_lab(const BatchArgs *__restrict__ A, const int *__restrict__ dead) { SNES_BATCH_IMG; candidate_lab_body(a.cand_tab, a.n, a.lab_eotf, a.cand_lab); }
__global__ __launch_bounds__(256) void kb_clear_bitmaps(const BatchArgs *__restrict__ A, const int *__restrict__ dead) {
    SNES_BATCH_IMG;
    const size_t words = (size_t)a.n * (a.npx / 32);
    for (size_t i = (size_t)blockIdx.x * 256 + threadIdx.x; i < words; i += (size_t)gridDim.x * 256) a.Pc.bitmap[i] = 0u;
}
__global__ __launch_bounds__(256) void kb_sparse_scan_lab(const BatchArgs *__restrict__ A, const int *__restrict__ dead) { SNES_BATCH_IMG; sparse_scan_lab_body(a.Pc); }
__global__ __launch_bounds__(64) void kb_sparse_h(const BatchArgs *__restrict__ A, int base, const int *__restrict__ dead) { SNES_BATCH_IMG; sparse_h_body(base ? a.Pb : a.Pc); }
__global__ __launch_bounds__(64) void kb_sparse_h2(const BatchArgs *__restrict__ A, const int *__restrict__ dead) { SNES_BATCH_XCD; sparse_h2_dispatch<false>(a.Pc, bb.y, bb.x, (int)gridDim.x); }
__global__ __launch_bounds__(64) void kb_sparse_h2_base(const BatchArgs *__restrict__ A, const int *__restrict__ dead) { SNES_BATCH_XCD; sparse_h2_dispatch<true>(a.Pb, bb.y, bb.x, (int)gridDim.x); }
__global__ __launch_bounds__(64) void kb_sparse_h2_lists(const BatchArgs *__restrict__ A, const int *__restrict__ dead, int list0) { SNES_BATCH_XCD; sparse_h2_dispatch<false>(a.Pc, list0 + bb.y, bb.x, (int)gridDim.x); }
__global__ __launch_bounds__(256, 5) void kb_sparse_v2_scales(const BatchArgs *__restrict__ A, const int *__restrict__ dead, int s0) { SNES_BATCH_XCD; const int s = s0 + bb.y; if (s < a.Pc.G.nscales && a.Pc.G.sw[s] >= 64) sparse_v2_body<false>(a.Pc, s, bb.x); }
__global__ __launch_bounds__(64) void kb_sparse_h2q(const BatchArgs *__restrict__ A, const int *__restrict__ dead) { SNES_BATCH_XCD; sparse_h2q_dispatch<false>(a.Pc, bb.y, bb.x, (int)gridDim.x); }
__global__ __launch_bounds__(64) void kb_sparse_h2q_base(const BatchArgs *__restrict__ A, const int *__restrict__ dead) { SNES_BATCH_XCD; sparse_h2q_dispatch<true>(a.Pb, bb.y, bb.x, (int)gridDim.x); }
__global__ __launch_bounds__(256, 5) void kb_sparse_v2(const BatchArgs *__restrict__ A, const int *__restrict__ dead) { SNES_BATCH_XCD; if (bb.y < a.Pc.G.nscales && a.Pc.G.sw[bb.y] >= 64) sparse_v2_body<false>(a.Pc, bb.y, bb.x); }
__global__ __launch_bounds__(256) void kb_sparse_v_base(const BatchArgs *__restrict__ A, const int *__restrict__ dead) { SNES_BATCH_XCD; if (bb.y < a.Pb.G.nscales && a.Pb.G.sw[bb.y] >= 64) sparse_v2_body<true>(a.Pb, bb.y, bb.x); }
__global__ __launch_bounds__(128) void kb_sparse_v_base_split(const BatchArgs *__restrict__ A, const int *__restrict__ dead) {
    SNES_BATCH_IMG;
    const int s = (int)blockIdx.y / 3, ch = (int)blockIdx.y - 3 * s;
    if (s < a.Pb.G.nscales && a.Pb.G.sw[s] >= 64 && (int)blockIdx.x < (a.Pb.G.sw[s] >> 6)) sparse_v2_base_split_body(a.Pb, s, ch, (int)blockIdx.x);
}
__global__ __launch_bounds__(256, 1) void kb_sparse_v_base_narrow(const BatchArgs *__restrict__ A, const int *__restrict__ dead) { SNES_BATCH_IMG; sparse_v_base_narrow_dispatch(a.Pb); }
__global__ __launch_bounds__(1024) void kb_sparse_order(const BatchArgs *__restrict__ A, const int *__restrict__ dead) { SNES_BATCH_IMG; sparse_order_body(a.Pc, const_cast<int *>(a.Pc.order)); }
__global__ __launch_bounds__(256, 2) void kb_sparse_v(const BatchArgs *__restrict__ A, const int *__restrict__ dead) { SNES_BATCH_IMG; sparse_v_body<false, 2, 2>(a.Pc, (int)blockIdx.y + a.Pc.s_first); }
__global__ __launch_bounds__(256) void kb_final_score(const BatchArgs *__restrict__ A, const int *__restrict__ dead) { SNES_BATCH_IMG; final_score_wave_body(a.part, a.n, a.Pc.G, a.errors, 1, 0, a.Pc.item_count, (int)kItemLists); }
__global__ __launch_bounds__(256) void kb_commit(const BatchArgs *__restrict__ A, const int *__restrict__ dead) { SNES_BATCH_IMG; commit_body(a.errors, a.n, a.cand, a.colors, a.slot, a.nes, a.inc_err, a.last, a.T); }
__global__ __launch_bounds__(1024) void kb_take_map(const BatchArgs *__restrict__ A, const int *__restrict__ dead) {
    SNES_BATCH_IMG;
    const int k = a.last->best_k;
    if (k < 0) return;
    const uint4 *src = reinterpret_cast<const uint4 *>(a.Pc.maps + (size_t)k * a.npx);
    uint4 *dst = reinterpret_cast<uint4 *>(a.map);
    for (int i = threadIdx.x; i < a.npx / 16; i += 1024) dst[i] = src[i];
}
#undef SNES_BATCH_IMG
#undef SNES_BATCH_XCD

struct WindowSlot { int method, n, slot, channel, nes, member; unsigned long long key; int cand0, pad; };
struct WindowResult { int consumed, accepted; };
constexpr int kMaxWindow = 1024;

__global__ void kw_gen_candidates(const WindowSlot *__restrict__ S, const uint8_t *__restrict__ colors, uint8_t *__restrict__ cand, double *__restrict__ errors, int stride, const int *__restrict__ dead, int dead_base) {
    if (*dead >= dead_base) return;
    const WindowSlot w = S[blockIdx.y];
    const int k = blockIdx.x * blockDim.x + threadIdx.x;
    if (k < stride) errors[(size_t)blockIdx.y * stride + k] = __longlong_as_double(0x7ff0000000000000ll);
    gen_candidates_body(w.method, w.n, w.key, colors, w.slot, w.channel, cand + 3 * (size_t)blockIdx.y * stride, 0, 1, nullptr, nullptr);
}

__global__ __launch_bounds__(1024) void kw_commit(const WindowSlot *__restrict__ S, int K, int stride, const double *__restrict__ errors, const uint8_t *__restrict__ cand, uint8_t *__restrict__ colors,
                                                 double *__restrict__ inc_err, StepResult *__restrict__ last, PaletteTables T, WindowResult *__restrict__ res, StepResult *__restrict__ log, int *__restrict__ dead, int dead_base, int seq) {
    if (*dead >= dead_base) { if (threadIdx.x == 0) { res->consumed = 0; res->accepted = 0; } return; }
    __shared__ double s_e[kMaxWindow];
    __shared__ int s_k[kMaxWindow];
    const int l16 = threadIdx.x & 15, q = threadIdx.x >> 4;
    for (int j = q; j < K; j += 64) {
        const int n = S[j].n;
        double be = __longlong_as_double(0x7ff0000000000000ll); int bk = 0x7fffffff;
        for (int k = l16; k < n; k += 16) { const double e = errors[(size_t)j * stride + k]; if (e < be) { be = e; bk = k; } }
#pragma unroll
        for (int o = 8; o > 0; o >>= 1) {
            const double e2 = __shfl_xor(be, o); const int k2 = __shfl_xor(bk, o);
            if (e2 < be || (e2 == be && k2 < bk)) { be = e2; bk = k2; }
        }
        if (l16 == 0) { s_e[j] = be; s_k[j] = bk; }
    }
    __syncthreads();
    int consumed = 0, accepted = 0;
    if (K > 0 && !S[0].nes) {
        __shared__ int s_first;
        if (threadIdx.x == 0) s_first = K;
        __syncthreads();
        const double inc = *inc_err;
        for (int j = threadIdx.x; j < K; j += 1024) if (s_k[j] != 0x7fffffff && s_e[j] < inc) atomicMin(&s_first, j);
        __syncthreads();
        const int first = s_first;
        for (int j = threadIdx.x; j < first; j += 1024) {
            const int slot = S[j].slot;
            StepResult r; r.error = inc; r.best_k = -1; r.rgb5[0] = colors[3 * slot]; r.rgb5[1] = colors[3 * slot + 1]; r.rgb5[2] = colors[3 * slot + 2]; r.changed = 0;
            log[j] = r;
        }
        __syncthreads();
        if (threadIdx.x != 0) return;
        consumed = first;
        if (first < K) {
            commit_decide(s_e[first], s_k[first], cand + 3 * (size_t)first * stride, colors, S[first].slot, 0, inc_err, log + first, T);
            consumed = first + 1; accepted = 1;
        } else if (K > 0) {
            const int slot = S[K - 1].slot;
            StepResult r; r.error = inc; r.best_k = -1; r.rgb5[0] = colors[3 * slot]; r.rgb5[1] = colors[3 * slot + 1]; r.rgb5[2] = colors[3 * slot + 2]; r.changed = 0;
            log[K - 1] = r;
        }
    } else {
        if (threadIdx.x != 0) return;
        for (int j = 0; j < K && !accepted; j++) {
            commit_decide(s_e[j], s_k[j], cand + 3 * (size_t)j * stride, colors, S[j].slot, S[j].nes, inc_err, log + j, T);
            consumed = j + 1;
            accepted = log[j].changed ? 1 : 0;
// ... 25 lines not shown
```

### snesimage_amd/csrc/kernels_sparse.hpp

```cpp
#pragma once
#include "kernels.hpp"

namespace snes {

constexpr int kGroupsTotal = 126;

struct CandMeta {
    int ngroups[kMaxScales];
    int xmin;
    int won;
    unsigned char glist[kGroupsTotal + 2];
    short gslot[kGroupsTotal];
    unsigned char gcb[kGroupsTotal];
};
__device__ __forceinline__ int item_k(unsigned int it) { return (int)(it >> 14); }
__device__ __forceinline__ int item_g(unsigned int it) { return (int)((it >> 8) & 63u); }
__device__ __forceinline__ int item_j(unsigned int it) { return (int)((it >> 2) & 63u); }
__device__ __forceinline__ int item_ch(unsigned int it) { return (int)(it & 3u); }
constexpr int kColBuckets = 4;
constexpr int kItemLists = kMaxScales * kColBuckets;

struct SparseGeom {
    long long off_lin[kMaxScales], off_xybC[kMaxScales], off_xybR[kMaxScales], off_hout[kMaxScales];
    long long cand_stride;
    long long off_ckf[kMaxScales], off_cka[kMaxScales];
    long long off_ckh[kMaxScales];
    int goff[kMaxScales];
};

struct SparseParams {
    Geom G; SparseGeom S; BlurK K;
    int ncand, k0, base, ncol, is_base;
    const unsigned long long *pack, *packC4, *packR4;
    const uint4 *plist; const int *plist_count;
    const float *pal_lin, *pal_xyb, *cand_tab;
    int perceptual; const float *labpx, *cand_lab; uint32_t *bitmap;
    const float *img1C4, *mu1R4, *sd1R4, *a1R4; const double *r1R4;
    float *store; CandMeta *meta;
    unsigned int *items; int *item_count; long long item_stride;
    float *ckf; double *cka; double *part; float *ckh;
    const float *zeros;
    float *trash;
    int use_maps, sub_size; uint32_t slot_ci; const uint8_t *maps, *mapsC4, *bmap, *bmapC4, *subC4, *tile_pal;
    int s_first;
    int *first;
    const int *order;
    const int *holder; int list0;
};

__device__ __forceinline__ uint32_t sparse_ci(uint32_t lo, uint32_t thr, uint32_t crgb, uint32_t ncol) {
    return red_mean_key(crgb, lo & 0x00ffffffu) < thr ? ncol : (lo >> 24);
}

__device__ __forceinline__ uint32_t won_bit(const uint32_t *bm, int px) { return (bm[px >> 5] >> (px & 31)) & 1u; }
__device__ __forceinline__ uint32_t maps_ci(const SparseParams &P, const uint8_t *map, bool is_base, int x0, int y0, uint32_t pack_lo) {
    uint32_t ci = pack_lo >> 24;
    if (ci != (uint32_t)P.ncol + 1u) {
        ci = (uint32_t)P.tile_pal[(x0 >> 3) + (y0 >> 3) * (P.G.W >> 3)] * (uint32_t)P.sub_size + map[y0 * P.G.W + x0];
        if (!is_base && ci == P.slot_ci) ci = (uint32_t)P.ncol;
    }
    return ci;
}

__device__ __forceinline__ unsigned long long pair_or_compress(unsigned long long m) {
    m = (m | (m >> 1)) & 0x5555555555555555ull;
    m = (m | (m >> 1)) & 0x3333333333333333ull;
    m = (m | (m >> 2)) & 0x0f0f0f0f0f0f0f0full;
    m = (m | (m >> 4)) & 0x00ff00ff00ff00ffull;
    m = (m | (m >> 8)) & 0x0000ffff0000ffffull;
    m = (m | (m >> 16)) & 0x00000000ffffffffull;
    return m;
}

template <int NW>
__device__ __forceinline__ void scan_publish(const SparseParams &P, const int k, const bool live, const unsigned long long mask, const int xmin, const int won, const int xg) {
    constexpr int NL = kItemLists;
    __shared__ int s_tot[NW][NL], s_off[NW][NL];
    const Geom &G = P.G;
    const int lane = threadIdx.x & 63, w = threadIdx.x >> 6;
    const unsigned long long below_mask = (1ull << lane) - 1ull;
    unsigned long long ms[kMaxScales]; int cbs[kMaxScales];
    {
        unsigned long long m = live ? mask : 0ull;
        int xgs = xg;
#pragma unroll
        for (int s = 0; s < kMaxScales; s++) {
            ms[s] = 0ull; cbs[s] = 0;
            if (s < G.nscales) {
                if (P.is_base && live) { const int ng = G.sh[s] >> 2; m = ng >= 64 ? ~0ull : ((1ull << ng) - 1ull); }
                const bool flag = ((m >> lane) & 1ull) != 0ull;
                const int nb = G.sw[s] >= 64 ? (G.sw[s] >> 6) : 1;
                const int cb = (flag && nb > 1) ? min(max((xgs >> s) - 4, 0) >> 6, nb - 1) : 0;
                ms[s] = m; cbs[s] = cb;
#pragma unroll
                for (int b = 0; b < kColBuckets; b++) {
                    const unsigned long long mb = __ballot(flag && cb == b);
                    if (lane == 0) s_tot[w][s * kColBuckets + b] = 3 * __popcll(mb);
                }
                m = pair_or_compress(m);
                const int xa = __shfl(xgs, (2 * lane) & 63), xb = __shfl(xgs, (2 * lane + 1) & 63);
                xgs = min(xa, xb);
            } else if (lane == 0) {
#pragma unroll
                for (int b = 0; b < kColBuckets; b++) s_tot[w][s * kColBuckets + b] = 0;
            }
        }
    }
    __syncthreads();
    if ((int)threadIdx.x < NL) {
        const int l = threadIdx.x;
        int sum = 0;
        for (int i = 0; i < NW; i++) { s_off[i][l] = sum; sum += s_tot[i][l]; }
        const int base = sum ? atomicAdd(&P.item_count[l], sum) : 0;
        for (int i = 0; i < NW; i++) s_off[i][l] += base;
    }
    __syncthreads();
    if (!live) return;
    CandMeta *M = P.meta + k;
    if (lane == 0) { M->xmin = xmin; M->won = won; }
#pragma unroll
    for (int s = 0; s < kMaxScales; s++) {
        if (s >= G.nscales) break;
        const int NG = G.sh[s] >> 2;
        const unsigned long long m = ms[s];
        const int cb = cbs[s];
        const bool flag = ((m >> lane) & 1ull) != 0ull;
        const int below = __popcll(m & below_mask);
        if (lane < NG) {
            M->gslot[P.S.goff[s] + lane] = flag ? (short)below : (short)-1;
            M->gcb[P.S.goff[s] + lane] = (unsigned char)cb;
// ... 1111 lines not shown
```

### snesimage_amd/csrc/kernels_sparse2.hpp

```cpp
#pragma once
#include "kernels_sparse.hpp"
#include "kernels_fast.hpp"

namespace snes {

#define SNES_HSTEP(SUM, A, B, OUT)                                                   \
    {                                                                                \
        float o1_ = (SUM) * n2_0, o3_ = (SUM) * n2_1, o5_ = (SUM) * n2_2;            \
        o1_ = fmaf(-1.0f, B[0], o1_); o3_ = fmaf(-1.0f, B[1], o3_); o5_ = fmaf(-1.0f, B[2], o5_); \
        o1_ = fmaf(mp_0, A[0], o1_); o3_ = fmaf(mp_1, A[1], o3_); o5_ = fmaf(mp_2, A[2], o5_);    \
        B[0] = o1_; B[1] = o3_; B[2] = o5_;                                          \
        OUT = o1_ + o3_ + o5_;                                                       \
    }
#define SNES_VSTEP(SUM, A, B, OUT)                                                   \
    {                                                                                \
        float o1_ = fmaf(A[0], d1_0, B[0]), o3_ = fmaf(A[1], d1_1, B[1]), o5_ = fmaf(A[2], d1_2, B[2]); \
        o1_ = fmaf((SUM), n2_0, -o1_); o3_ = fmaf((SUM), n2_1, -o3_); o5_ = fmaf((SUM), n2_2, -o5_);    \
        B[0] = o1_; B[1] = o3_; B[2] = o5_;                                          \
        OUT = o1_ + o3_ + o5_;                                                       \
    }

struct H2Shared {
    __attribute__((aligned(16))) float out[16 * (4 * 32 + 4)];
    long long hbase[16], xbase[16];
};
__device__ __forceinline__ void lds_order() { asm volatile("s_waitcnt lgkmcnt(0)" ::: "memory"); }
template <bool BASE>
__device__ __forceinline__ void h2_resolve(const SparseParams &P, const uint4 pa, const uint4 pb, const uint32_t bw, const int g, const uint32_t crgb, uint32_t (&ci)[4]) {
    if (P.use_maps) resolve4_maps(pa.x, pa.y, BASE ? 0xffffffffu : P.slot_ci, (uint32_t)P.ncol, ci);
    else if (P.perceptual && !BASE) {
        const uint32_t b4 = (bw >> ((g & 7) << 2)) & 0xfu;
        ci[0] = (b4 & 1u) ? (uint32_t)P.ncol : (pa.x >> 24); ci[1] = (b4 & 2u) ? (uint32_t)P.ncol : (pa.z >> 24);
        ci[2] = (b4 & 4u) ? (uint32_t)P.ncol : (pb.x >> 24); ci[3] = (b4 & 8u) ? (uint32_t)P.ncol : (pb.z >> 24);
    } else {
        const uint32_t never = BASE ? 0u : 0xffffffffu;
        ci[0] = sparse_ci(pa.x, pa.y & never, crgb, (uint32_t)P.ncol); ci[1] = sparse_ci(pa.z, pa.w & never, crgb, (uint32_t)P.ncol);
        ci[2] = sparse_ci(pb.x, pb.y & never, crgb, (uint32_t)P.ncol); ci[3] = sparse_ci(pb.z, pb.w & never, crgb, (uint32_t)P.ncol);
    }
}
template <bool S0, bool BASE>
__device__ __forceinline__ void sparse_h2_body(const SparseParams &P, const int list, const int bx, const int gx, H2Shared &sh) {
    constexpr int NP = (S0 || !BASE) ? 4 : 3;
    constexpr int PW = 32;
    constexpr int ISTR = NP * PW + 4;
    extern __shared__ float s_lut[];
    const int lstr = P.ncol + 2;
    float *const s_out = sh.out;
    long long *const s_hbase = sh.hbase, *const s_xbase = sh.xbase;
    const Geom &G = P.G;
    const int s = list / kColBuckets, cb = list % kColBuckets;
    const int W = G.sw[s], H = G.sh[s];
    const int lane = threadIdx.x;
    const int count = P.item_count[list];
    if (bx * 16 >= count) return;
    if (S0) {
        for (int i = lane; i < 3 * lstr; i += 64) { const int c = i / lstr, j = i - c * lstr; s_lut[i] = P.pal_xyb[3 * j + c]; }
        lds_order();
    }
    const float n2_0 = P.K.n2[0], n2_1 = P.K.n2[1], n2_2 = P.K.n2[2];
    const float mp_0 = -P.K.d1[0], mp_1 = -P.K.d1[1], mp_2 = -P.K.d1[2];
    const int G4 = W >> 2, gs = cb << 4;
    const int r = lane & 3;
    const int half = lane >> 5, fl = lane & 31, fp = fl >> 3, fc = fl & 7;
    float *const trash = P.trash + (lane << 2);
    const float4 zero4 = make_float4(0.f, 0.f, 0.f, 0.f);
    for (int i0 = bx * 16; i0 < count; i0 += gx * 16) {
        const int qi = i0 + (lane >> 2);
        const bool valid = qi < count;
        const unsigned int it = P.items[(size_t)list * P.item_stride + (valid ? qi : i0)];
        const int k = item_k(it), j = item_j(it), ch = item_ch(it);
        const int y = 4 * item_g(it) + r;
        const size_t ns = (size_t)W * H;
        const float cand_v = (S0 && !BASE) ? P.cand_tab[8 * (size_t)k + 3 + ch] : 0.0f;
        const uint32_t crgb = (S0 && !BASE) ? __float_as_uint(P.cand_tab[8 * (size_t)k + 6]) : 0u;
        const float4 *in1 = reinterpret_cast<const float4 *>(P.img1C4 + G.src_off[s] + (size_t)ch * ns) + y;
        const uint4 *pk = S0 ? reinterpret_cast<const uint4 *>(P.packC4) + 2 * (size_t)y : nullptr;
        const bool um = S0 && P.use_maps;
        const uint32_t *mw = um ? reinterpret_cast<const uint32_t *>(BASE ? P.bmapC4 : P.mapsC4 + (size_t)(k - P.k0) * ns) + y : nullptr;
        const uint32_t *sw = um ? reinterpret_cast<const uint32_t *>(P.subC4) + y : nullptr;
        const uint32_t *bmrow = (S0 && P.perceptual && !BASE && !um) ? P.bitmap + (size_t)k * (G.W * G.H / 32) + (size_t)y * (W >> 5) : reinterpret_cast<const uint32_t *>(P.img1C4);
        const float4 *in2 = S0 ? nullptr
                               : reinterpret_cast<const float4 *>(P.store + (size_t)k * P.S.cand_stride + P.S.off_xybC[s] + (size_t)j * 12 * W + (size_t)ch * 4 * W) + r;
        lds_order();
        if (r == 0) {
            s_hbase[lane >> 2] = valid ? (long long)k * P.S.cand_stride + P.S.off_hout[s] + (long long)j * 36 * W + (long long)(ch * 3) * 4 * W : -1ll;
            s_xbase[lane >> 2] = valid ? (long long)k * P.S.cand_stride + P.S.off_xybR[s] + (long long)j * 12 * W + (long long)ch * 4 * W : -1ll;
        }
        float sa[3][3], sb[3][3];
        const float *ck = P.ckh + P.S.off_ckh[s] + ((size_t)(ch * 3 + (cb > 0 ? cb - 1 : 0)) * 18) * H + y;
#pragma unroll
        for (int p = 0; p < 3; p++)
#pragma unroll
            for (int q = 0; q < 3; q++) {
                sa[p][q] = gs > 0 ? ck[(size_t)(p * 6 + q) * H] : 0.0f;
                sb[p][q] = gs > 0 ? ck[(size_t)(p * 6 + 3 + q) * H] : 0.0f;
            }
        float4 r1[6], r2[6];
        uint4 pa[3], pb[3]; uint32_t bw[3];
#pragma unroll
        for (int a = 0; a < 6; a++) { r1[a] = zero4; r2[a] = zero4; }
#pragma unroll
        for (int a = 0; a < 3; a++) { pa[a] = make_uint4(0, 0, 0, 0); pb[a] = pa[a]; bw[a] = 0u; }
        auto fetch = [&](const int q, float4 &d1, float4 &d2, uint4 &wa, uint4 &wb, uint32_t &wbm) {
            d1 = in1[(size_t)q * H];
            if (S0) {
                if (um) { wa.x = mw[(size_t)q * H]; wa.y = sw[(size_t)q * H]; } else { wa = pk[(size_t)q * H * 2]; wb = pk[(size_t)q * H * 2 + 1]; }
                wbm = bmrow[q >> 3];
            } else d2 = in2[(size_t)q * 4];
        };
        auto convert = [&](const int g, const uint4 wa, const uint4 wb, const uint32_t wbm, float4 &d2) {
            uint32_t ci[4];
            h2_resolve<BASE>(P, wa, wb, wbm, g, crgb, ci);
            const float *lut = s_lut + ch * lstr;
            d2.x = ci[0] == (uint32_t)P.ncol ? cand_v : lut[ci[0]]; d2.y = ci[1] == (uint32_t)P.ncol ? cand_v : lut[ci[1]];
            d2.z = ci[2] == (uint32_t)P.ncol ? cand_v : lut[ci[2]]; d2.w = ci[3] == (uint32_t)P.ncol ? cand_v : lut[ci[3]];
        };
        if (gs > 0) {
            uint4 ta[3], tb[3]; uint32_t tw[3];
#pragma unroll
            for (int a = 0; a < 3; a++) { ta[a] = make_uint4(0, 0, 0, 0); tb[a] = ta[a]; tw[a] = 0u; fetch(gs - 3 + a, r1[3 + a], r2[3 + a], ta[a], tb[a], tw[a]); }
            if (S0) {
#pragma unroll
                for (int a = 0; a < 3; a++) convert(gs - 3 + a, ta[a], tb[a], tw[a], r2[3 + a]);
            }
        }
        fetch(gs, r1[0], r2[0], pa[0], pb[0], bw[0]);
        fetch(gs + 1, r1[1], r2[1], pa[1], pb[1], bw[1]);
#define SNES_H2_ITER(T, STAGE, FLUSH)                                                                                         \
        {                                                                                                                     \
            constexpr int sl_ = (T) % 6, sf_ = ((T) + 2) % 6, ua_ = ((T) + 3) % 6, ub_ = ((T) + 4) % 6, ul_ = ((T) + 5) % 6; \
            constexpr int wc_ = (T) % 3, wf_ = ((T) + 2) % 3;                                                                 \
            { const int qf_ = min(g + 2, G4 - 1); fetch(qf_, r1[sf_], r2[sf_], pa[wf_], pb[wf_], bw[wf_]); }                  \
            if (g >= G4) { r1[sl_] = zero4; r2[sl_] = zero4; }                                                                \
            else if (S0) convert(g, pa[wc_], pb[wc_], bw[wc_], r2[sl_]);                                                      \
            if (BASE && g > 0 && (g & 15) == 0 && g < G4 && valid) {                \
                float *co = P.ckh + P.S.off_ckh[s] + ((size_t)(ch * 3 + (g >> 4) - 1) * 18) * H + y;                          \
                _Pragma("unroll") for (int p = 0; p < 3; p++)                                                                 \
                    _Pragma("unroll") for (int q = 0; q < 3; q++) { co[(size_t)(p * 6 + q) * H] = sa[p][q]; co[(size_t)(p * 6 + 3 + q) * H] = sb[p][q]; } \
            }                                                                                                                 \
            const float v1[4] = {r1[sl_].x, r1[sl_].y, r1[sl_].z, r1[sl_].w}, v2[4] = {r2[sl_].x, r2[sl_].y, r2[sl_].z, r2[sl_].w};   \
            const float l1[4] = {r1[ua_].z, r1[ua_].w, r1[ub_].x, r1[ub_].y}, l2[4] = {r2[ua_].z, r2[ua_].w, r2[ub_].x, r2[ub_].y};   \
            float outp[3][4];                                                                                                 \
            _Pragma("unroll") for (int q = 0; q < 4; q++) {                                                                   \
                const float s0 = l2[q] + v2[q];                                                                               \
                const float s1 = (l2[q] * l2[q]) + (v2[q] * v2[q]);                                                           \
                const float s2 = (l1[q] * l2[q]) + (v1[q] * v2[q]);                                                           \
                if ((q & 1) == 0) { SNES_HSTEP(s0, sa[0], sb[0], outp[0][q]) SNES_HSTEP(s1, sa[1], sb[1], outp[1][q]) SNES_HSTEP(s2, sa[2], sb[2], outp[2][q]) } \
                else { SNES_HSTEP(s0, sb[0], sa[0], outp[0][q]) SNES_HSTEP(s1, sb[1], sa[1], outp[1][q]) SNES_HSTEP(s2, sb[2], sa[2], outp[2][q]) }             \
            }                                                                                                                 \
            if (STAGE) {  \
                float *so = s_out + (lane >> 2) * ISTR + ((((T) + 1) & 1) << 4) + r;             \
                _Pragma("unroll") for (int p = 0; p < 3; p++) { so[p * PW + 0] = outp[p][0]; so[p * PW + 4] = outp[p][1]; so[p * PW + 8] = outp[p][2]; so[p * PW + 12] = outp[p][3]; } \
                if (NP == 4) { so[3 * PW + 0] = r2[ul_].x; so[3 * PW + 4] = r2[ul_].y; so[3 * PW + 8] = r2[ul_].z; so[3 * PW + 12] = r2[ul_].w; } \
            }                                                                                                                 \
            if (FLUSH) {     \
                lds_order();                                                                                                  \
                 \
                                                              \
                const uint32_t o_l = ((NP == 4 && fp == 3) ? 0u : (uint32_t)fp * 4u * (uint32_t)W) + (uint32_t)((g - 2) << 4) + (uint32_t)(fc << 2); \
                _Pragma("unroll") for (int mb = 0; mb < 16; mb += 8) {                                                        \
                    float4 fv[4]; long long fb[4];                                                                            \
                    _Pragma("unroll") for (int m = 0; m < 4; m++) {                                                           \
                        const int im_ = mb + 2 * m + half;                                                                    \
                        fv[m] = *reinterpret_cast<const float4 *>(s_out + im_ * ISTR + fl * 4);                               \
                        fb[m] = (NP == 4 && fp == 3) ? s_xbase[im_] : s_hbase[im_];                                           \
                    }                                                                                                         \
                    _Pragma("unroll") for (int m = 0; m < 4; m++) {                                                           \
                        float *dst = (fb[m] >= 0 && fl < NP * 8) ? P.store + fb[m] + o_l : trash;                             \
                        *reinterpret_cast<float4 *>(dst) = fv[m];                                                             \
                    }                                                                                                         \
                }                                                                                                             \
                asm volatile("" ::: "memory");                 \
            }                                                                                                                 \
        }
        { const int g = gs; SNES_H2_ITER(0, false, false) }
        for (int g0 = gs + 1; g0 <= G4; g0 += 6) {
            { const int g = g0; SNES_H2_ITER(1, true, false) }
            { const int g = g0 + 1; if (g > G4) break; SNES_H2_ITER(2, true, true) }
            { const int g = g0 + 2; if (g > G4) break; SNES_H2_ITER(3, true, false) }
            { const int g = g0 + 3; if (g > G4) break; SNES_H2_ITER(4, true, true) }
            { const int g = g0 + 4; if (g > G4) break; SNES_H2_ITER(5, true, false) }
            { const int g = g0 + 5; if (g > G4) break; SNES_H2_ITER(6, true, true) }
        }
#undef SNES_H2_ITER
    }
}

template <bool S0, bool BASE>
__device__ __forceinline__ void sparse_h2q_body(const SparseParams &P, const int list, const int bx, const int gx, H2Shared &sh) {
    constexpr int NP = (S0 || !BASE) ? 4 : 3, PW = 32, ISTR = 4 * PW + 4;
    extern __shared__ float s_lut[];
    const int lstr = P.ncol + 2;
    float *const s_out = sh.out;
    long long *const s_hbase = sh.hbase, *const s_xbase = sh.xbase;
    const Geom &G = P.G;
    const int s = list / kColBuckets, cb = list % kColBuckets;
    const int W = G.sw[s], H = G.sh[s];
    const int lane = threadIdx.x;
    const int count = P.item_count[list];
    if (bx * 4 >= count) return;
    if (S0) {
        for (int i = lane; i < 3 * lstr; i += 64) { const int c = i / lstr, j = i - c * lstr; s_lut[i] = P.pal_xyb[3 * j + c]; }
        lds_order();
    }
    const int q = lane & 3, r = (lane >> 2) & 3, im = lane >> 4;
    const int pl = q < 3 ? q : 0;
    const float n2_0 = P.K.n2[0], n2_1 = P.K.n2[1], n2_2 = P.K.n2[2];
    const float mp_0 = -P.K.d1[0], mp_1 = -P.K.d1[1], mp_2 = -P.K.d1[2];
    const int G4 = W >> 2, gs = cb << 4;
    const int half = lane >> 5, fl = lane & 31, fp = fl >> 3, fc = fl & 7;
    float *const trash = P.trash + (lane << 2);
    const float4 zero4 = make_float4(0.f, 0.f, 0.f, 0.f);
    for (int i0 = bx * 4; i0 < count; i0 += gx * 4) {
        const int qi = i0 + im;
        const bool valid = qi < count;
        const unsigned int it = P.items[(size_t)list * P.item_stride + (valid ? qi : i0)];
        const int k = item_k(it), j = item_j(it), ch = item_ch(it);
        const int y = 4 * item_g(it) + r;
        const size_t ns = (size_t)W * H;
        const float cand_v = (S0 && !BASE) ? P.cand_tab[8 * (size_t)k + 3 + ch] : 0.0f;
        const uint32_t crgb = (S0 && !BASE) ? __float_as_uint(P.cand_tab[8 * (size_t)k + 6]) : 0u;
        const float4 *in1 = reinterpret_cast<const float4 *>(P.img1C4 + G.src_off[s] + (size_t)ch * ns) + y;
        const uint4 *pk = S0 ? reinterpret_cast<const uint4 *>(P.packC4) + 2 * (size_t)y : nullptr;
        const bool um = S0 && P.use_maps;
        const uint32_t *mw = um ? reinterpret_cast<const uint32_t *>(BASE ? P.bmapC4 : P.mapsC4 + (size_t)(k - P.k0) * ns) + y : nullptr;
        const uint32_t *sw = um ? reinterpret_cast<const uint32_t *>(P.subC4) + y : nullptr;
        const uint32_t *bmrow = (S0 && P.perceptual && !BASE && !um) ? P.bitmap + (size_t)k * (G.W * G.H / 32) + (size_t)y * (W >> 5) : reinterpret_cast<const uint32_t *>(P.img1C4);
        const float4 *in2 = S0 ? nullptr
                               : reinterpret_cast<const float4 *>(P.store + (size_t)k * P.S.cand_stride + P.S.off_xybC[s] + (size_t)j * 12 * W + (size_t)ch * 4 * W) + r;
        lds_order();
        if ((lane & 15) == 0) {
            s_hbase[im] = valid ? (long long)k * P.S.cand_stride + P.S.off_hout[s] + (long long)j * 36 * W + (long long)(ch * 3) * 4 * W : -1ll;
            s_xbase[im] = valid ? (long long)k * P.S.cand_stride + P.S.off_xybR[s] + (long long)j * 12 * W + (long long)ch * 4 * W : -1ll;
        }
        float sa[3], sb[3];
        const float *ck = P.ckh + P.S.off_ckh[s] + ((size_t)(ch * 3 + (cb > 0 ? cb - 1 : 0)) * 18) * H + y;
#pragma unroll
        for (int e = 0; e < 3; e++) {
            sa[e] = gs > 0 ? ck[(size_t)(pl * 6 + e) * H] : 0.0f;
            sb[e] = gs > 0 ? ck[(size_t)(pl * 6 + 3 + e) * H] : 0.0f;
        }
        float4 r1[6], r2[6];
        uint4 pa[3], pb[3]; uint32_t bw[3];
#pragma unroll
        for (int a = 0; a < 6; a++) { r1[a] = zero4; r2[a] = zero4; }
#pragma unroll
        for (int a = 0; a < 3; a++) { pa[a] = make_uint4(0, 0, 0, 0); pb[a] = pa[a]; bw[a] = 0u; }
        auto fetch = [&](const int qq, float4 &d1, float4 &d2, uint4 &wa, uint4 &wb, uint32_t &wbm) {
            d1 = in1[(size_t)qq * H];
            if (S0) {
                if (um) { wa.x = mw[(size_t)qq * H]; wa.y = sw[(size_t)qq * H]; } else { wa = pk[(size_t)qq * H * 2]; wb = pk[(size_t)qq * H * 2 + 1]; }
                wbm = bmrow[qq >> 3];
            } else d2 = in2[(size_t)qq * 4];
        };
        auto convert = [&](const int g, const uint4 wa, const uint4 wb, const uint32_t wbm, float4 &d2) {
            uint32_t ci[4];
            h2_resolve<BASE>(P, wa, wb, wbm, g, crgb, ci);
            const float *lut = s_lut + ch * lstr;
            d2.x = ci[0] == (uint32_t)P.ncol ? cand_v : lut[ci[0]]; d2.y = ci[1] == (uint32_t)P.ncol ? cand_v : lut[ci[1]];
            d2.z = ci[2] == (uint32_t)P.ncol ? cand_v : lut[ci[2]]; d2.w = ci[3] == (uint32_t)P.ncol ? cand_v : lut[ci[3]];
        };
        if (gs > 0) {
            uint4 ta[3], tb[3]; uint32_t tw[3];
#pragma unroll
            for (int a = 0; a < 3; a++) { ta[a] = make_uint4(0, 0, 0, 0); tb[a] = ta[a]; tw[a] = 0u; fetch(gs - 3 + a, r1[3 + a], r2[3 + a], ta[a], tb[a], tw[a]); }
            if (S0) {
#pragma unroll
                for (int a = 0; a < 3; a++) convert(gs - 3 + a, ta[a], tb[a], tw[a], r2[3 + a]);
            }
        }
        fetch(gs, r1[0], r2[0], pa[0], pb[0], bw[0]);
        fetch(gs + 1, r1[1], r2[1], pa[1], pb[1], bw[1]);
#define SNES_H2Q_ITER(T, STAGE, FLUSH)                                                                                        \
        {                                                                                                                     \
            constexpr int sl_ = (T) % 6, sf_ = ((T) + 2) % 6, ua_ = ((T) + 3) % 6, ub_ = ((T) + 4) % 6, ul_ = ((T) + 5) % 6; \
            constexpr int wc_ = (T) % 3, wf_ = ((T) + 2) % 3;                                                                 \
            { const int qf_ = min(g + 2, G4 - 1); fetch(qf_, r1[sf_], r2[sf_], pa[wf_], pb[wf_], bw[wf_]); }                  \
            if (g >= G4) { r1[sl_] = zero4; r2[sl_] = zero4; }                                                                \
            else if (S0) convert(g, pa[wc_], pb[wc_], bw[wc_], r2[sl_]);                                                      \
            if (BASE && q < 3 && g > 0 && (g & 15) == 0 && g < G4 && valid) {  \
                float *co = P.ckh + P.S.off_ckh[s] + ((size_t)(ch * 3 + (g >> 4) - 1) * 18) * H + y;                          \
                _Pragma("unroll") for (int e = 0; e < 3; e++) { co[(size_t)(pl * 6 + e) * H] = sa[e]; co[(size_t)(pl * 6 + 3 + e) * H] = sb[e]; } \
            }                                                                                                                 \
            const float v1[4] = {r1[sl_].x, r1[sl_].y, r1[sl_].z, r1[sl_].w}, v2[4] = {r2[sl_].x, r2[sl_].y, r2[sl_].z, r2[sl_].w};   \
            const float l1[4] = {r1[ua_].z, r1[ua_].w, r1[ub_].x, r1[ub_].y}, l2[4] = {r2[ua_].z, r2[ua_].w, r2[ub_].x, r2[ub_].y};   \
            float outp[4];                                                                                                    \
            _Pragma("unroll") for (int c = 0; c < 4; c++) {                                                                   \
                 \
                const float s0 = l2[c] + v2[c];                                                                               \
                const float s1 = (l2[c] * l2[c]) + (v2[c] * v2[c]);                                                           \
                const float s2 = (l1[c] * l2[c]) + (v1[c] * v2[c]);                                                           \
                const float sum = q == 0 ? s0 : (q == 1 ? s1 : s2);                                                           \
                if ((c & 1) == 0) { SNES_HSTEP(sum, sa, sb, outp[c]) } else { SNES_HSTEP(sum, sb, sa, outp[c]) }              \
            }                                                                                                                 \
            if (STAGE) {                                                                                                      \
                float *so = s_out + im * ISTR + ((((T) + 1) & 1) << 4) + r + q * PW;                                          \
                if (q < 3) { so[0] = outp[0]; so[4] = outp[1]; so[8] = outp[2]; so[12] = outp[3]; }                           \
                else if (NP == 4) { so[0] = r2[ul_].x; so[4] = r2[ul_].y; so[8] = r2[ul_].z; so[12] = r2[ul_].w; }            \
            }                                                                                                                 \
            if (FLUSH) {                                                                                                      \
                lds_order();                                                                                                  \
                const uint32_t o_l = ((fp == 3) ? 0u : (uint32_t)fp * 4u * (uint32_t)W) + (uint32_t)((g - 2) << 4) + (uint32_t)(fc << 2); \
                float4 fv[2]; long long fb[2];                                                                                \
                _Pragma("unroll") for (int m = 0; m < 2; m++) {                                                               \
                    const int im_ = 2 * m + half;                                                                             \
                    fv[m] = *reinterpret_cast<const float4 *>(s_out + im_ * ISTR + fl * 4);                                   \
                    fb[m] = (fp == 3) ? s_xbase[im_] : s_hbase[im_];                                                          \
                }                                                                                                             \
                _Pragma("unroll") for (int m = 0; m < 2; m++) {                                                               \
                    float *dst = (fb[m] >= 0 && fl < NP * 8) ? P.store + fb[m] + o_l : trash;                                 \
                    *reinterpret_cast<float4 *>(dst) = fv[m];                                                                 \
                }                                                                                                             \
                asm volatile("" ::: "memory");                                                                               \
            }                                                                                                                 \
        }
        { const int g = gs; SNES_H2Q_ITER(0, false, false) }
        for (int g0 = gs + 1; g0 <= G4; g0 += 6) {
            { const int g = g0; SNES_H2Q_ITER(1, true, false) }
            { const int g = g0 + 1; if (g > G4) break; SNES_H2Q_ITER(2, true, true) }
            { const int g = g0 + 2; if (g > G4) break; SNES_H2Q_ITER(3, true, false) }
            { const int g = g0 + 3; if (g > G4) break; SNES_H2Q_ITER(4, true, true) }
            { const int g = g0 + 4; if (g > G4) break; SNES_H2Q_ITER(5, true, false) }
            { const int g = g0 + 5; if (g > G4) break; SNES_H2Q_ITER(6, true, true) }
        }
#undef SNES_H2Q_ITER
    }
}
template <bool BASE>
__device__ __forceinline__ void sparse_h2q_dispatch(const SparseParams &P, const int list, const int bx, const int gx) {
    const int s = list / kColBuckets;
    if (s >= P.G.nscales || P.G.sw[s] < 64 || (list % kColBuckets) >= (P.G.sw[s] >> 6)) return;
    __shared__ H2Shared sh;
    if (s == 0) sparse_h2q_body<true, BASE>(P, list, bx, gx, sh); else sparse_h2q_body<false, BASE>(P, list, bx, gx, sh);
}

__device__ __forceinline__ int uni(int v) { return __builtin_amdgcn_readfirstlane(v); }
template <typename T> __device__ __forceinline__ T ld_at(const void *sbase, uint32_t voff) { return *reinterpret_cast<const T *>(reinterpret_cast<const char *>(sbase) + voff); }
typedef __amdgpu_buffer_rsrc_t rsrc_t;
typedef unsigned int u32x4 __attribute__((ext_vector_type(4)));
__device__ __forceinline__ rsrc_t make_rsrc(const void *p) {
    const unsigned long long a = (unsigned long long)p;
    const unsigned long long u = ((unsigned long long)(uint32_t)__builtin_amdgcn_readfirstlane((int)(a >> 32)) << 32) | (uint32_t)__builtin_amdgcn_readfirstlane((int)a);
    return __builtin_amdgcn_make_buffer_rsrc(reinterpret_cast<void *>(u), 0, 0x7fffffff, 0x00020000);
}
__device__ __forceinline__ float4 buf_ld4(rsrc_t r, uint32_t voff, uint32_t soff) {
    const u32x4 v = __builtin_amdgcn_raw_buffer_load_b128(r, (int)voff, (int)soff, 0);
    return make_float4(__uint_as_float(v.x), __uint_as_float(v.y), __uint_as_float(v.z), __uint_as_float(v.w));
}
__device__ __forceinline__ double2 buf_ld2d(rsrc_t r, uint32_t voff, uint32_t soff) {
    const u32x4 v = __builtin_amdgcn_raw_buffer_load_b128(r, (int)voff, (int)soff, 0);
    return make_double2(__hiloint2double((int)v.y, (int)v.x), __hiloint2double((int)v.w, (int)v.z));
}

template <bool BASE>
__device__ __forceinline__ void sparse_v2_body(const SparseParams &P, const int s, const int bx) {
    __shared__ short s_slot[4][64];
    __shared__ __attribute__((aligned(16))) unsigned char s_raw[(2 + 3) * 3 * 256 * sizeof(float2)];
    double (*red)[6] = reinterpret_cast<double (*)[6]>(s_raw);
    static_assert(sizeof(s_raw) >= 256 * 6 * sizeof(double), "reduction scratch must fit the tail ring");
    const Geom &G = P.G;
    const int W = uni(G.sw[s]), H = uni(G.sh[s]), H4 = H >> 2;
    const int t = threadIdx.x, lane = t & 63;
    const int wv = uni(t >> 6);
    const int wpp = W >> 6, ppw = 4 / wpp;
    const int npairs = BASE ? 3 : P.ncand * 3;
    if (bx * ppw >= npairs) return;
    const int ql = wv / wpp, xw = (wv - ql * wpp) << 6;
    const int pair_raw = bx * ppw + ql;
    const bool active = pair_raw < npairs;
    const int pair = active ? pair_raw : 0;
    const int ch = BASE ? pair : pair / P.ncand, ci = BASE ? 0 : pair - ch * P.ncand;
    const int k = BASE ? P.base : uni(P.k0 + (P.order ? P.order[ci] : ci));
    const CandMeta *M = P.meta + k;
    int gs;
    {
        const int g = lane;
        short sl = -1;
        if (!BASE && g < H4) { sl = M->gslot[P.S.goff[s] + g]; if (sl >= 0 && ((int)M->gcb[P.S.goff[s] + g] << 6) > xw) sl = -1; }
        s_slot[wv][lane] = sl;
        const unsigned long long own = __ballot(sl >= 0);
        gs = BASE ? 0 : uni(own ? __ffsll((long long)own) - 1 : H4 + 1);
    }
    __syncthreads();

    const size_t ns = (size_t)W * H;
    const float *store_k = P.store + (size_t)k * P.S.cand_stride, *store_b = P.store + (size_t)P.base * P.S.cand_stride;
    const rsrc_t h_own = make_rsrc(store_k + P.S.off_hout[s] + (size_t)(ch * 3) * 4 * W + ((size_t)(xw >> 6) << 8));
    const rsrc_t h_b = make_rsrc(store_b + P.S.off_hout[s] + (size_t)(ch * 3) * 4 * W + ((size_t)(xw >> 6) << 8));
    const rsrc_t h_zero = make_rsrc(P.zeros);
    const rsrc_t x_own = make_rsrc(store_k + P.S.off_xybR[s] + (size_t)ch * 4 * W + (size_t)xw * 4);
    const rsrc_t x_b = make_rsrc(store_b + P.S.off_xybR[s] + (size_t)ch * 4 * W + (size_t)xw * 4);
    const rsrc_t m1_b = make_rsrc(P.mu1R4 + G.src_off[s] + (size_t)ch * ns + (size_t)xw * 4);
    const rsrc_t sd1_b = make_rsrc(P.sd1R4 + G.src_off[s] + (size_t)ch * ns + (size_t)xw * 4);
    const rsrc_t a1_b = make_rsrc(P.a1R4 + G.src_off[s] + (size_t)ch * ns + (size_t)xw * 4);
    const rsrc_t r1_b = make_rsrc(P.r1R4 + G.src_off[s] + (size_t)ch * ns + (size_t)xw * 4);
    const uint32_t l4 = (uint32_t)lane << 2, l8 = (uint32_t)lane << 3, l16 = (uint32_t)lane << 4, l32 = (uint32_t)lane << 5;
    const uint32_t W16 = (uint32_t)W * 16u;

    const float n2_0 = P.K.n2[0], n2_1 = P.K.n2[1], n2_2 = P.K.n2[2];
    const float d1_0 = P.K.d1[0], d1_1 = P.K.d1[1], d1_2 = P.K.d1[2];
    float sa[3][3], sb[3][3];
    double acc[6];
    float *ck_f = P.ckf + P.S.off_ckf[s] + ((size_t)ch * (H4 + 2)) * 18 * W + xw + lane;
    double *ck_a = P.cka + P.S.off_cka[s] + ((size_t)ch * (H4 + 2)) * 6 * W + xw + lane;
    if (BASE) {
#pragma unroll
        for (int p = 0; p < 3; p++)
#pragma unroll
            for (int q = 0; q < 3; q++) { sa[p][q] = 0.0f; sb[p][q] = 0.0f; }
#pragma unroll
        for (int q = 0; q < 6; q++) acc[q] = 0.0;
    } else {
        const float *cf = P.ckf + P.S.off_ckf[s] + ((size_t)ch * (H4 + 2) + gs) * 18 * W + xw;
        const double *ca = P.cka + P.S.off_cka[s] + ((size_t)ch * (H4 + 2) + gs) * 6 * W + xw;
#pragma unroll
        for (int p = 0; p < 3; p++)
#pragma unroll
            for (int q = 0; q < 3; q++) { sa[p][q] = ld_at<float>(cf + (size_t)(p * 6 + q) * W, l4); sb[p][q] = ld_at<float>(cf + (size_t)(p * 6 + 3 + q) * W, l4); }
#pragma unroll
        for (int q = 0; q < 6; q++) acc[q] = ld_at<double>(ca + (size_t)q * W, l8);
    }
#define SNES_HLOAD(GG, DST)                                                                                                   \
    {                                                                                                                         \
        const int gg_ = (GG);                                                                                                 \
        const bool below_ = gg_ >= H4;                                                                                        \
        const int sl_ = uni((int)s_slot[wv][below_ ? 0 : gg_]);                                                               \
        const rsrc_t r_ = below_ ? h_zero : (sl_ >= 0 ? h_own : h_b);                                                         \
        const uint32_t so_ = below_ ? 0u : (uint32_t)(sl_ >= 0 ? sl_ : gg_) * 9u * W16;                                       \
        DST[0] = buf_ld4(r_, l16, so_); DST[1] = buf_ld4(r_, l16, so_ + W16); DST[2] = buf_ld4(r_, l16, so_ + 2u * W16);      \
    }
    const float4 zero4 = make_float4(0.f, 0.f, 0.f, 0.f);
    float2 *ring_xy = reinterpret_cast<float2 *>(s_raw) + t;
    float2 *ring_zw = reinterpret_cast<float2 *>(s_raw + 2 * 3 * 256 * sizeof(float2)) + t;
    float4 bufA[3], bufB[3];
    float4 t1[3] = {zero4, zero4, zero4}, t2[3] = {zero4, zero4, zero4}, t3[3] = {zero4, zero4, zero4};
#pragma unroll
    for (int p = 0; p < 3; p++) { bufA[p] = zero4; bufB[p] = zero4; }
    if (gs <= H4) {
        if (gs < H4) SNES_HLOAD(gs, bufA)
        if (gs - 1 >= 0) SNES_HLOAD(gs - 1, t1)
        if (gs - 2 >= 0) SNES_HLOAD(gs - 2, t2)
        if (gs - 3 >= 0) SNES_HLOAD(gs - 3, t3)
    }
#pragma unroll
    for (int p = 0; p < 3; p++) {
        const float4 g1 = t1[p], g2 = t2[p], g3 = t3[p];
        ring_xy[(1 * 3 + p) * 256] = make_float2(g1.x, g1.y); ring_zw[(2 * 3 + p) * 256] = make_float2(g1.z, g1.w);
        ring_xy[(0 * 3 + p) * 256] = make_float2(g2.x, g2.y); ring_zw[(1 * 3 + p) * 256] = make_float2(g2.z, g2.w);
        ring_zw[(0 * 3 + p) * 256] = make_float2(g3.z, g3.w);
    }
    int r2 = 0, r3 = 0;
#define SNES_V2GROUP(CUR, NXT)                                                                                                \
    {                                                                                                                         \
        if (BASE && active) {                                                                                   \
            _Pragma("unroll") for (int p = 0; p < 3; p++)                                                                     \
                _Pragma("unroll") for (int q = 0; q < 3; q++) { ck_f[(size_t)(p * 6 + q) * W] = sa[p][q]; ck_f[(size_t)(p * 6 + 3 + q) * W] = sb[p][q]; } \
            _Pragma("unroll") for (int q = 0; q < 6; q++) ck_a[(size_t)q * W] = acc[q];                                       \
            ck_f += (size_t)18 * W; ck_a += (size_t)6 * W;                                                                    \
        }                                                                                                                     \
        SNES_HLOAD(g + 1, NXT)                                                                                                \
                \
        float4 c_m1, c_sd1, c_a1, c_x;                                                                                        \
        double2 c_ra, c_rb;                                                                                                   \
        {                                                                                                                     \
            const int gm = g >= 1 ? g - 1 : 0;                                                                                \
            const uint32_t go = (uint32_t)gm * W16;                                                                           \
            c_m1 = buf_ld4(m1_b, l16, go); c_sd1 = buf_ld4(sd1_b, l16, go); c_a1 = buf_ld4(a1_b, l16, go);                    \
            c_ra = buf_ld2d(r1_b, l32, 2u * go); c_rb = buf_ld2d(r1_b, l32 + 16u, 2u * go);                                   \
            const int sl = uni((int)s_slot[wv][gm]);                                                                          \
            c_x = buf_ld4(sl >= 0 ? x_own : x_b, l16, (uint32_t)(sl >= 0 ? sl : gm) * 3u * W16);                              \
        }                                                                                                                     \
        float outp[3][4];                                                                                                     \
        _Pragma("unroll") for (int p = 0; p < 3; p++) {                                                                       \
            float2 *pz = ring_zw + (r3 * 3 + p) * 256, *px = ring_xy + (r2 * 3 + p) * 256;                                    \
            const float2 tz = *pz, tx = *px;                                       \
            *pz = make_float2(CUR[p].z, CUR[p].w);                                                                            \
            *px = make_float2(CUR[p].x, CUR[p].y);                                                                            \
            SNES_VSTEP(tz.x + CUR[p].x, sa[p], sb[p], outp[p][0])                                                             \
            SNES_VSTEP(tz.y + CUR[p].y, sb[p], sa[p], outp[p][1])                                                             \
            SNES_VSTEP(tx.x + CUR[p].z, sa[p], sb[p], outp[p][2])                                                             \
            SNES_VSTEP(tx.y + CUR[p].w, sb[p], sa[p], outp[p][3])                                                             \
        }                                                                                                                     \
          \
        asm volatile("" : "+v"(c_a1.x), "+v"(c_a1.y), "+v"(c_a1.z), "+v"(c_a1.w));                                            \
        if (g >= 1) {                                                                                                         \
            const float m1v[4] = {c_m1.x, c_m1.y, c_m1.z, c_m1.w}, sd1v[4] = {c_sd1.x, c_sd1.y, c_sd1.z, c_sd1.w};              \
            const float a1v[4] = {c_a1.x, c_a1.y, c_a1.z, c_a1.w}, i2v[4] = {c_x.x, c_x.y, c_x.z, c_x.w};                     \
            const double r1v[4] = {c_ra.x, c_ra.y, c_rb.x, c_rb.y};                                                           \
            _Pragma("unroll") for (int q = 0; q < 4; q++)                                                                     \
                maps_accumulate(acc, m1v[q], sd1v[q], a1v[q], r1v[q], outp[0][q], outp[1][q], outp[2][q], i2v[q]);            \
        }                                                                                                                     \
        r2 ^= 1; r3 = r3 == 2 ? 0 : r3 + 1;                                                                                   \
    }
    for (int g = gs; g <= H4; g++) {
        SNES_V2GROUP(bufA, bufB)
        g++;
        if (g > H4) break;
        SNES_V2GROUP(bufB, bufA)
    }
#undef SNES_V2GROUP
#undef SNES_HLOAD
    if (BASE && active) {
#pragma unroll
        for (int q = 0; q < 6; q++) ck_a[(size_t)q * W] = acc[q];
    }
    __syncthreads();
#pragma unroll
    for (int q = 0; q < 6; q++) red[t][q] = active ? acc[q] : 0.0;
    __syncthreads();
    const int xp = t & (W - 1);
    for (int stride = W >> 1; stride > 0; stride >>= 1) {
        if (xp < stride) {
#pragma unroll
            for (int q = 0; q < 6; q++) red[t][q] += red[t + stride][q];
        }
        __syncthreads();
    }
    if (xp == 0 && active) {
        double *o = P.part + (((size_t)k * G.nscales + s) * 3 + ch) * 6;
#pragma unroll
        for (int q = 0; q < 6; q++) o[q] = red[t][q];
    }
}
__device__ __forceinline__ void lds_barrier() { asm volatile("s_waitcnt lgkmcnt(0)\n\ts_barrier" ::: "memory"); }
__device__ __forceinline__ void sparse_v2_base_split_body(const SparseParams &P, const int s, const int ch, const int cb) {
    __shared__ __attribute__((aligned(16))) float s_x[2][3][64][4];
    const Geom &G = P.G;
    const int W = uni(G.sw[s]), H = uni(G.sh[s]), H4 = H >> 2;
    const int lane = threadIdx.x & 63;
    const bool is_r = uni((int)(threadIdx.x >> 6)) == 0;
    const int xw = cb << 6;
    const size_t ns = (size_t)W * H;
    const float *store_b = P.store + (size_t)P.base * P.S.cand_stride;
    const uint32_t l16 = (uint32_t)lane << 4, l32 = (uint32_t)lane << 5;
    const uint32_t W16 = (uint32_t)W * 16u;
    const float4 zero4 = make_float4(0.f, 0.f, 0.f, 0.f);
    if (is_r) {
        const rsrc_t h_b = make_rsrc(store_b + P.S.off_hout[s] + (size_t)(ch * 3) * 4 * W + ((size_t)(xw >> 6) << 8));
        const rsrc_t h_zero = make_rsrc(P.zeros);
        const float n2_0 = P.K.n2[0], n2_1 = P.K.n2[1], n2_2 = P.K.n2[2];
        const float d1_0 = P.K.d1[0], d1_1 = P.K.d1[1], d1_2 = P.K.d1[2];
        float sa[3][3], sb[3][3];
#pragma unroll
        for (int p = 0; p < 3; p++)
#pragma unroll
            for (int q = 0; q < 3; q++) { sa[p][q] = 0.0f; sb[p][q] = 0.0f; }
        float *ck_f = P.ckf + P.S.off_ckf[s] + ((size_t)ch * (H4 + 2)) * 18 * W + xw + lane;
        float4 ring[3][3];
        float4 nxt[3];
#pragma unroll
        for (int p = 0; p < 3; p++) { ring[p][0] = zero4; ring[p][1] = zero4; ring[p][2] = zero4; }
#define SNES_V2S_HLOAD(GG, DST) { const int gg_ = (GG); const bool below_ = gg_ >= H4; const rsrc_t r_ = below_ ? h_zero : h_b; const uint32_t so_ = below_ ? 0u : (uint32_t)gg_ * 9u * W16; \
            DST[0] = buf_ld4(r_, l16, so_); DST[1] = buf_ld4(r_, l16, so_ + W16); DST[2] = buf_ld4(r_, l16, so_ + 2u * W16); }
        SNES_V2S_HLOAD(0, nxt)
#define SNES_V2S_RITER(T)                                                                                   \
        {                                                                                                                     \
            constexpr int u_ = (T) % 3, ux_ = ((T) + 1) % 3;                                                                  \
            _Pragma("unroll") for (int p = 0; p < 3; p++)                                                                     \
                _Pragma("unroll") for (int q = 0; q < 3; q++) { ck_f[(size_t)(p * 6 + q) * W] = sa[p][q]; ck_f[(size_t)(p * 6 + 3 + q) * W] = sb[p][q]; } \
            ck_f += (size_t)18 * W;                                                                                           \
            float4 cur[3] = {nxt[0], nxt[1], nxt[2]};                                                                         \
            SNES_V2S_HLOAD(g + 1, nxt)                                                                                        \
            _Pragma("unroll") for (int p = 0; p < 3; p++) {                                                                   \
                const float4 tz = ring[p][u_], tx = ring[p][ux_];        \
                float4 o;                                                                                                     \
                SNES_VSTEP(tz.z + cur[p].x, sa[p], sb[p], o.x)                                                                \
                SNES_VSTEP(tz.w + cur[p].y, sb[p], sa[p], o.y)                                                                \
                SNES_VSTEP(tx.x + cur[p].z, sa[p], sb[p], o.z)                                                                \
                SNES_VSTEP(tx.y + cur[p].w, sb[p], sa[p], o.w)                                                                \
                ring[p][u_] = cur[p];                                                                                         \
                *reinterpret_cast<float4 *>(&s_x[g & 1][p][lane][0]) = o;                                                     \
            }                                                                                                                 \
        }
        for (int g0 = 0; g0 <= H4 + 1; g0 += 3) {
            { const int g = g0; if (g <= H4) SNES_V2S_RITER(0) lds_barrier(); }
            { const int g = g0 + 1; if (g > H4 + 1) break; if (g <= H4) SNES_V2S_RITER(1) lds_barrier(); }
            { const int g = g0 + 2; if (g > H4 + 1) break; if (g <= H4) SNES_V2S_RITER(2) lds_barrier(); }
        }
#undef SNES_V2S_RITER
#undef SNES_V2S_HLOAD
    } else {
        const rsrc_t x_b = make_rsrc(store_b + P.S.off_xybR[s] + (size_t)ch * 4 * W + (size_t)xw * 4);
        const rsrc_t m1_b = make_rsrc(P.mu1R4 + G.src_off[s] + (size_t)ch * ns + (size_t)xw * 4);
        const rsrc_t sd1_b = make_rsrc(P.sd1R4 + G.src_off[s] + (size_t)ch * ns + (size_t)xw * 4);
        const rsrc_t a1_b = make_rsrc(P.a1R4 + G.src_off[s] + (size_t)ch * ns + (size_t)xw * 4);
        const rsrc_t r1_b = make_rsrc(P.r1R4 + G.src_off[s] + (size_t)ch * ns + (size_t)xw * 4);
        double acc[6] = {0.0, 0.0, 0.0, 0.0, 0.0, 0.0};
        double *ck_a = P.cka + P.S.off_cka[s] + ((size_t)ch * (H4 + 2)) * 6 * W + xw + lane;
        float4 n_m1, n_sd1, n_a1, n_x; double2 n_ra, n_rb;
#define SNES_V2S_MLOAD(GM) { const uint32_t go_ = (uint32_t)(GM) * W16; n_m1 = buf_ld4(m1_b, l16, go_); n_sd1 = buf_ld4(sd1_b, l16, go_); n_a1 = buf_ld4(a1_b, l16, go_); \
            n_ra = buf_ld2d(r1_b, l32, 2u * go_); n_rb = buf_ld2d(r1_b, l32 + 16u, 2u * go_); n_x = buf_ld4(x_b, l16, (uint32_t)(GM) * 3u * W16); }
        SNES_V2S_MLOAD(0)
        for (int t = 0; t <= H4 + 1; t++) {
            if (t >= 1) {
                const int g = t - 1;
#pragma unroll
                for (int q = 0; q < 6; q++) ck_a[(size_t)q * W] = acc[q];
                ck_a += (size_t)6 * W;
                if (g >= 1) {
                    const float4 c_m1 = n_m1, c_sd1 = n_sd1, c_a1 = n_a1, c_x = n_x; const double2 c_ra = n_ra, c_rb = n_rb;
                    { const int gn = g < H4 ? g : H4 - 1; SNES_V2S_MLOAD(gn) }
                    const float4 o0 = *reinterpret_cast<const float4 *>(&s_x[g & 1][0][lane][0]), o1 = *reinterpret_cast<const float4 *>(&s_x[g & 1][1][lane][0]),
                                 o2 = *reinterpret_cast<const float4 *>(&s_x[g & 1][2][lane][0]);
                    const float m1v[4] = {c_m1.x, c_m1.y, c_m1.z, c_m1.w}, sd1v[4] = {c_sd1.x, c_sd1.y, c_sd1.z, c_sd1.w};
                    const float a1v[4] = {c_a1.x, c_a1.y, c_a1.z, c_a1.w}, i2v[4] = {c_x.x, c_x.y, c_x.z, c_x.w};
                    const double r1v[4] = {c_ra.x, c_ra.y, c_rb.x, c_rb.y};
                    const float p0[4] = {o0.x, o0.y, o0.z, o0.w}, p1[4] = {o1.x, o1.y, o1.z, o1.w}, p2[4] = {o2.x, o2.y, o2.z, o2.w};
#pragma unroll
                    for (int q = 0; q < 4; q++) maps_accumulate(acc, m1v[q], sd1v[q], a1v[q], r1v[q], p0[q], p1[q], p2[q], i2v[q]);
                }
            }
            lds_barrier();
        }
#undef SNES_V2S_MLOAD
#pragma unroll
        for (int q = 0; q < 6; q++) ck_a[(size_t)q * W] = acc[q];
    }
}

#undef SNES_HSTEP
#undef SNES_VSTEP

template <bool BASE>
__device__ __forceinline__ void sparse_h2_dispatch(const SparseParams &P, const int list, const int bx, const int gx) {
    const int s = list / kColBuckets;
    if (s >= P.G.nscales || P.G.sw[s] < 64 || (list % kColBuckets) >= (P.G.sw[s] >> 6)) return;
    __shared__ H2Shared sh;
    if (s == 0) sparse_h2_body<true, BASE>(P, list, bx, gx, sh); else sparse_h2_body<false, BASE>(P, list, bx, gx, sh);
}
__global__ __launch_bounds__(64) void k_sparse_h2(SparseParams P) { sparse_h2_dispatch<false>(P, (int)blockIdx.y, (int)blockIdx.x, (int)gridDim.x); }
__global__ __launch_bounds__(64) void k_sparse_h2_from(SparseParams P, int list0) { sparse_h2_dispatch<false>(P, list0 + (int)blockIdx.y, (int)blockIdx.x, (int)gridDim.x); }
__global__ __launch_bounds__(64) void k_sparse_h2q(SparseParams P) { sparse_h2q_dispatch<false>(P, (int)blockIdx.y, (int)blockIdx.x, (int)gridDim.x); }
__global__ __launch_bounds__(64) void k_sparse_h2q_base(SparseParams P) { sparse_h2q_dispatch<true>(P, (int)blockIdx.y, (int)blockIdx.x, (int)gridDim.x); }
__global__ __launch_bounds__(64) void k_sparse_h2_base(SparseParams P) { sparse_h2_dispatch<true>(P, (int)blockIdx.y, (int)blockIdx.x, (int)gridDim.x); }
__global__ __launch_bounds__(256, 5) void k_sparse_v2(SparseParams P) { if ((int)blockIdx.y < P.G.nscales && P.G.sw[blockIdx.y] >= 64) sparse_v2_body<false>(P, (int)blockIdx.y, (int)blockIdx.x); }
__global__ __launch_bounds__(256, 5) void k_sparse_v2_from(SparseParams P, int s0) { const int s = s0 + (int)blockIdx.y; if (s < P.G.nscales && P.G.sw[s] >= 64) sparse_v2_body<false>(P, s, (int)blockIdx.x); }
__global__ __launch_bounds__(128) void k_sparse_v2_base_split(SparseParams P) { const int s = (int)blockIdx.z; if (s < P.G.nscales && P.G.sw[s] >= 64 && (int)blockIdx.x < (P.G.sw[s] >> 6)) sparse_v2_base_split_body(P, s, (int)blockIdx.y, (int)blockIdx.x); }
__global__ __launch_bounds__(256) void k_sparse_v2_base(SparseParams P) { if ((int)blockIdx.y < P.G.nscales && P.G.sw[blockIdx.y] >= 64) sparse_v2_body<true>(P, (int)blockIdx.y, (int)blockIdx.x); }
__device__ __forceinline__ void sparse_v_base_narrow_dispatch(const SparseParams &P) { const int s = (int)blockIdx.y + P.s_first; if (s < P.G.nscales) sparse_v_body<false, 0, 1>(P, s); }
__global__ __launch_bounds__(256, 1) void k_sparse_v_base_narrow(SparseParams P) { sparse_v_base_narrow_dispatch(P); }

}
```

Baseline: 2.927 million.

## Add won-pixel mask variants of sparse h2/v2 kernels for candidate scale 0

Adds templated mask variants of the horizontal and vertical sparse SSIM passes. At candidate scale 0 they write three planes instead of four, and the v2 sweep rebuilds its XYB inputs from a per-pixel mask that selects between the candidate and base values. The aim is to cut scale-0 intermediate storage and global traffic. The variants are enabled by default for non-dither contexts, with an environment switch to turn them off and a resource-budget check script. In exchange there are more kernel instantiations, extra mask loads, and a risk of register pressure in the v2 sweep.

```diff
diff --git a/snesimage_amd/csrc/batch_host.inc b/snesimage_amd/csrc/batch_host.inc
--- a/snesimage_amd/csrc/batch_host.inc
+++ b/snesimage_amd/csrc/batch_host.inc
@@ -122,17 +122,18 @@
         hipLaunchKernelGGL(kb_dither_diff, dim3((n + 3) / 4, 1, K), dim3(1024), 0, st, A, dead);
     } else if ((size_t)n * K <= c0->sp.scan4_max) hipLaunchKernelGGL(kb_sparse_scan4, dim3((n + 3) / 4, 1, K), dim3(1024), 0, st, A, dead);
     else hipLaunchKernelGGL(kb_sparse_scan, dim3((n + 15) / 16, 1, K), dim3(1024), 0, st, A, 0, dead);
+    const bool masks = c0->sp.xyb_masks && !c0->dither;
     const bool two = side && side->aux && !quad && (size_t)n * K >= c0->sp.h0_min && c0->sp.h0_min > 0 && s_first > 0 && c0->sp.down1 && G.nscales > 2;
     if (two) {
         hipStream_t ax = side->aux;
         HIPCHK(hipEventRecord(side->a_scan, st)); HIPCHK(hipStreamWaitEvent(ax, side->a_scan, 0));
         if (split) HIPCHK(hipStreamWaitEvent(ax, side->h, 0));
         size_t gx = ((size_t)n * 8 * 3 + 15) / 16; if (gx > c0->sp.hgrid) gx = c0->sp.hgrid; if (gx < 8) gx = 8;
-        hipLaunchKernelGGL(kb_sparse_h2_lists, dim3((unsigned)gx, (unsigned)kColBuckets, K), dim3(64), h2_lds(c0), ax, A, dead, 0);
+        hipLaunchKernelGGL(masks ? kb_sparse_h2_listsm : kb_sparse_h2_lists, dim3((unsigned)gx, (unsigned)kColBuckets, K), dim3(64), h2_lds(c0), ax, A, dead, 0);
         if (c0->sp.lpt) hipLaunchKernelGGL(kb_sparse_order, dim3(1, 1, K), dim3(1024), 0, ax, A, dead);
         HIPCHK(hipEventRecord(side->a_h0, ax));
         if (split) HIPCHK(hipStreamWaitEvent(ax, side->v, 0));
-        hipLaunchKernelGGL(kb_sparse_v2_scales, dim3(n * 3, 1, K), dim3(256), 0, ax, A, dead, 0);
+        hipLaunchKernelGGL(masks ? kb_sparse_v2_scalesm : kb_sparse_v2_scales, dim3(n * 3, 1, K), dim3(256), 0, ax, A, dead, 0);
         HIPCHK(hipEventRecord(side->a_v0, ax));
     }
     if (c0->sp.down1 && G.nscales > 2) {
@@ -145,9 +146,9 @@
     } else hipLaunchKernelGGL(kb_sparse_down, dim3(n, 1, K), dim3(256), 0, st, A, 0, dead);
     if (split) HIPCHK(hipStreamWaitEvent(st, side->h, 0));
     { size_t gx = ((size_t)n * 8 * 3 + 15) / 16; if (gx > c0->sp.hgrid) gx = c0->sp.hgrid; if (gx < 8) gx = 8;
-      if (quad) hipLaunchKernelGGL(kb_sparse_h2q, dim3((unsigned)(gx * 4), (unsigned)(s_first * kColBuckets), K), dim3(64), h2_lds(c0), st, A, dead);
+      if (quad) hipLaunchKernelGGL(masks ? kb_sparse_h2qm : kb_sparse_h2q, dim3((unsigned)(gx * 4), (unsigned)(s_first * kColBuckets), K), dim3(64), h2_lds(c0), st, A, dead);
       else if (two) { if (s_first > 1) hipLaunchKernelGGL(kb_sparse_h2_lists, dim3((unsigned)gx, (unsigned)((s_first - 1) * kColBuckets), K), dim3(64), h2_lds(c0), st, A, dead, (int)kColBuckets); }
-      else hipLaunchKernelGGL(kb_sparse_h2, dim3((unsigned)gx, (unsigned)(s_first * kColBuckets), K), dim3(64), h2_lds(c0), st, A, dead);
+      else hipLaunchKernelGGL(masks ? kb_sparse_h2m : kb_sparse_h2, dim3((unsigned)gx, (unsigned)(s_first * kColBuckets), K), dim3(64), h2_lds(c0), st, A, dead);
       if (s_first < G.nscales) hipLaunchKernelGGL(kb_sparse_h, dim3((unsigned)((gx + 7) / 8), (unsigned)((G.nscales - s_first) * kColBuckets), K), dim3(64), 0, st, A, 0, dead); }
     if (two) {
         HIPCHK(hipStreamWaitEvent(st, side->a_h0, 0));
@@ -158,7 +159,7 @@
     } else {
     if (c0->sp.lpt) hipLaunchKernelGGL(kb_sparse_order, dim3(1, 1, K), dim3(1024), 0, st, A, dead);
     if (split) HIPCHK(hipStreamWaitEvent(st, side->v, 0));
-    hipLaunchKernelGGL(kb_sparse_v2, dim3(n * 3, (unsigned)s_first, K), dim3(256), 0, st, A, dead);
+    hipLaunchKernelGGL(masks ? kb_sparse_v2m : kb_sparse_v2, dim3(n * 3, (unsigned)s_first, K), dim3(256), 0, st, A, dead);
     if (split) HIPCHK(hipStreamWaitEvent(st, side->narrow, 0));
     if (s_first < G.nscales) hipLaunchKernelGGL(kb_sparse_v, dim3((n * 3 + 7) / 8, (unsigned)(G.nscales - s_first), K), dim3(256), 0, st, A, dead);
     }
@@ -193,6 +194,7 @@
         if (c->perceptual != c0->perceptual) return fail(SNES_ERR_ARG, "contexts of a batch must share their flags");
         if (!c->sp.enabled || (c->dither && c->sub_size == 1)) return fail(SNES_ERR_UNSUPPORTED, "batched calls cover the group-sparse path (not with SNES_SPARSE=0), and with --dither subpalettes of two entries and more");
         if (c->dither != c0->dither) return fail(SNES_ERR_ARG, "contexts of a batch must share their flags");
+        if (c->sp.xyb_masks != c0->sp.xyb_masks) return fail(SNES_ERR_ARG, "contexts of a batch must share their flags");
         if (!ordered_tables_equal(c, c0)) return fail(SNES_ERR_ARG, "contexts of a batch must share their ordered-dither table");
     }
     std::unique_ptr<snesimage_batch> b(new snesimage_batch());
diff --git a/snesimage_amd/csrc/capi.hip b/snesimage_amd/csrc/capi.hip
--- a/snesimage_amd/csrc/capi.hip
+++ b/snesimage_amd/csrc/capi.hip
@@ -159,6 +159,7 @@
         bool vsplit = true;
         uint32_t scan4_max = 2048;
         uint32_t hgrid = 8192;
+        bool xyb_masks = true;
         bool dedup = true; uint32_t dedup_min = 1024; int *holder = nullptr; bool holder_dirty = false;
         bool enabled = false, side = true; uint32_t min_n = 1; uint32_t cap = 0, lanes = 0;
         SparseGeom S{};
@@ -547,6 +548,7 @@
     P.items = sp.items + (size_t)lane * sp.item_stride * kItemLists; P.item_count = sp.item_count + (size_t)lane * kItemLists; P.item_stride = sp.item_stride;
     P.ckf = sp.ckf; P.cka = sp.cka; P.part = sp.part; P.first = sp.first; P.ckh = sp.ckh; P.zeros = sp.ckh + sp.zeros_off; P.trash = sp.ckh + sp.zeros_off + 12LL * c->G.W;
     for (P.s_first = 0; P.s_first < c->G.nscales && c->G.sw[P.s_first] >= 64; P.s_first++) {}
+    P.xyb_masks = (sp.xyb_masks && !c->dither) ? 1 : 0;
     if (c->dither) {
         const uint32_t l = lane < c->nlanes ? lane : 0;
         P.use_maps = 1; P.sub_size = (int)c->sub_size; P.slot_ci = sp.slot_ci; P.subC4 = c->d_subC4; P.tile_pal = c->d_tile_pal;
@@ -713,13 +715,13 @@
         HIPCHK(hipStreamWaitEvent(hs, sp.ev_scan[lane], 0));
         HIPCHK(hipStreamWaitEvent(hs, sp.ev_base_h, 0));
         size_t gx = ((size_t)nc * (G.sh[0] / 4) * 3 + 15) / 16; if (gx > sp.h0_grid) gx = sp.h0_grid;
-        hipLaunchKernelGGL(k_sparse_h2, dim3((unsigned)gx, (unsigned)kColBuckets), dim3(64), h2_lds(c), hs, P);
+        hipLaunchKernelGGL(P.xyb_masks ? k_sparse_h2m : k_sparse_h2, dim3((unsigned)gx, (unsigned)kColBuckets), dim3(64), h2_lds(c), hs, P);
         if (c->sp.lpt) hipLaunchKernelGGL(k_sparse_order, dim3(1), dim3(1024), 0, hs, P, sp.order + P.k0);
         HIPCHK(hipEventRecord(sp.ev_h0[lane], hs));
         if (v0_aside) {
             HIPCHK(hipStreamWaitEvent(hs, sp.ev_base_done, 0));
             if (c->timing) HIPCHK(hipEventRecord(tr.ev[3], hs));
-            hipLaunchKernelGGL(k_sparse_v2, dim3(nc * 3, 1), dim3(256), 0, hs, P);
+            hipLaunchKernelGGL(P.xyb_masks ? k_sparse_v2m : k_sparse_v2, dim3(nc * 3, 1), dim3(256), 0, hs, P);
             if (c->timing) HIPCHK(hipEventRecord(tr.ev[4], hs));
             HIPCHK(hipEventRecord(sp.ev_v0[lane], hs));
         }
@@ -739,11 +741,11 @@
     { size_t gx = ((size_t)nc * (G.sh[0] / 4) * 3 + 15) / 16; if (gx > sp.hgrid) gx = sp.hgrid;
       if (nc <= sp.h2q_max) {
           size_t gq = ((size_t)nc * (G.sh[0] / 4) * 3 + 3) / 4; if (gq > sp.hgrid) gq = sp.hgrid;
-          hipLaunchKernelGGL(k_sparse_h2q, dim3((unsigned)gq, (unsigned)(P.s_first * kColBuckets)), dim3(64), h2_lds(c), stream, P);
+          hipLaunchKernelGGL(P.xyb_masks ? k_sparse_h2qm : k_sparse_h2q, dim3((unsigned)gq, (unsigned)(P.s_first * kColBuckets)), dim3(64), h2_lds(c), stream, P);
       } else
       if (h0_ahead) { if (P.s_first > 1) hipLaunchKernelGGL(k_sparse_h2_from, dim3((unsigned)gx, (unsigned)((P.s_first - 1) * kColBuckets)), dim3(64), h2_lds(c), stream, P, (int)kColBuckets); }
       else
-      hipLaunchKernelGGL(k_sparse_h2, dim3((unsigned)gx, (unsigned)(P.s_first * kColBuckets)), dim3(64), h2_lds(c), stream, P);
+      hipLaunchKernelGGL(P.xyb_masks ? k_sparse_h2m : k_sparse_h2, dim3((unsigned)gx, (unsigned)(P.s_first * kColBuckets)), dim3(64), h2_lds(c), stream, P);
       if (P.s_first < G.nscales) hipLaunchKernelGGL(k_sparse_h, dim3((unsigned)((gx + 7) / 8), (unsigned)((G.nscales - P.s_first) * kColBuckets)), dim3(64), 0, stream, P);
       if (vn_aside) HIPCHK(hipEventRecord(sp.ev_hn[lane], stream));
       if (h0_ahead) HIPCHK(hipStreamWaitEvent(stream, sp.ev_h0[lane], 0)); }
@@ -766,7 +768,7 @@
         if (P.s_first > 1) hipLaunchKernelGGL(k_sparse_v2_from, dim3(nc * 3, (unsigned)(P.s_first - 1)), dim3(256), 0, stream, P, 1);
     } else {
     if (c->timing) HIPCHK(hipEventRecord(tr.ev[3], stream));
-    hipLaunchKernelGGL(k_sparse_v2, dim3(nc * 3, (unsigned)P.s_first), dim3(256), 0, stream, P);
+    hipLaunchKernelGGL(P.xyb_masks ? k_sparse_v2m : k_sparse_v2, dim3(nc * 3, (unsigned)P.s_first), dim3(256), 0, stream, P);
     if (c->timing) HIPCHK(hipEventRecord(tr.ev[4], stream));
     }
     if (vn_aside) HIPCHK(hipStreamWaitEvent(stream, sp.ev_vn[lane], 0));
@@ -1050,6 +1052,7 @@
     if (const char *e = getenv("SNES_H2Q_MAX")) { int v = atoi(e); if (v >= 0) c->sp.h2q_max = (uint32_t)v; }
     if (const char *e = getenv("SNES_HGRID")) { int v = atoi(e); if (v >= 1) c->sp.hgrid = (uint32_t)v; }
     if (const char *e = getenv("SNES_SPARSE_MIN")) { int v = atoi(e); if (v >= 1) c->sp.min_n = (uint32_t)v; }
+    if (const char *e = getenv("SNES_XYB_MASKS")) c->sp.xyb_masks = atoi(e) != 0;
     if (const char *e = getenv("SNES_DEDUP")) c->sp.dedup = atoi(e) != 0;
     if (const char *e = getenv("SNES_DEDUP_MIN")) { int v = atoi(e); if (v >= 1) c->sp.dedup_min = (uint32_t)v; }
     Geom &G = c->G;
diff --git a/snesimage_amd/csrc/check_resources.py b/snesimage_amd/csrc/check_resources.py
--- /dev/null
+++ b/snesimage_amd/csrc/check_resources.py
@@ -0,0 +1,66 @@
+#!/usr/bin/env python3
+import re
+import sys
+
+V_SWEEPS = ("k_sparse_v2", "k_sparse_v2m", "k_sparse_v2_from")
+H_PASSES = ("k_sparse_h2", "k_sparse_h2m", "k_sparse_h2_from", "k_sparse_h2q", "k_sparse_h2qm")
+KEYS = ("VGPRs", "TotalSGPRs", "ScratchSize [bytes/lane]", "VGPRs Spill", "LDS Size [bytes/block]", "Occupancy [waves/SIMD]")
+
+
+def kernel_name(mangled):
+    m = re.match(r"_ZN(.*)", mangled)
+    if not m:
+        return mangled
+    rest, parts = m.group(1), []
+    while rest and rest[0].isdigit():
+        n = int(re.match(r"\d+", rest).group(0))
+        rest = rest[len(str(n)):]
+        parts.append(rest[:n])
+        rest = rest[n:]
+    return parts[-1] if parts else mangled
+
+
+def parse(path):
+    out, cur = {}, None
+    with open(path, errors="replace") as f:
+        for line in f:
+            m = re.search(r"remark:\s+(.*?): (.*?) \[-Rpass-analysis=kernel-resource-usage\]", line)
+            if not m:
+                continue
+            key, val = m.group(1).strip(), m.group(2).strip()
+            if key == "Function Name":
+                cur = out.setdefault(kernel_name(val), {})
+            elif cur is not None:
+                cur[key] = val
+    return out
+
+
+def main(argv):
+    if len(argv) < 2:
+        sys.exit(__doc__)
+    res = parse(argv[1])
+    if "--table" in argv:
+        print("| kernel | VGPRs | SGPRs | scratch B/lane | VGPRs spilled | LDS B/block | waves/SIMD |")
+        print("|---|---|---|---|---|---|---|")
+        for k in sorted(res):
+            if "sparse" in k:
+                print("| `%s` | %s |" % (k, " | ".join(res[k].get(q, "?") for q in KEYS)))
+        return 0
+    bad = []
+    for k in V_SWEEPS + H_PASSES:
+        r = res.get(k)
+        if r is None:
+            bad.append("%s: no resource figures in %s" % (k, argv[1]))
+            continue
+        vgpr, scratch, spill, occ = (int(r[q]) for q in ("VGPRs", "ScratchSize [bytes/lane]", "VGPRs Spill", "Occupancy [waves/SIMD]"))
+        if k in V_SWEEPS and (vgpr > 96 or scratch or spill or occ < 5):
+            bad.append("%s: %d VGPRs, %d bytes of scratch, %d spilled, %d waves/SIMD (budget: 96, 0, 0, 5)" % (k, vgpr, scratch, spill, occ))
+        if k in H_PASSES and (scratch or spill or occ < 2):
+            bad.append("%s: %d bytes of scratch, %d spilled, %d waves/SIMD (budget: 0, 0, 2)" % (k, scratch, spill, occ))
+    for b in bad:
+        print("check_resources: " + b, file=sys.stderr)
+    return 1 if bad else 0
+
+
+if __name__ == "__main__":
+    sys.exit(main(sys.argv))
diff --git a/snesimage_amd/csrc/kernels_batch.hpp b/snesimage_amd/csrc/kernels_batch.hpp
--- a/snesimage_amd/csrc/kernels_batch.hpp
+++ b/snesimage_amd/csrc/kernels_batch.hpp
@@ -72,6 +72,11 @@
 __global__ __launch_bounds__(64) void kb_sparse_h2q(const BatchArgs *__restrict__ A, const int *__restrict__ dead) { SNES_BATCH_XCD; sparse_h2q_dispatch<false>(a.Pc, bb.y, bb.x, (int)gridDim.x); }
 __global__ __launch_bounds__(64) void kb_sparse_h2q_base(const BatchArgs *__restrict__ A, const int *__restrict__ dead) { SNES_BATCH_XCD; sparse_h2q_dispatch<true>(a.Pb, bb.y, bb.x, (int)gridDim.x); }
 __global__ __launch_bounds__(256, 5) void kb_sparse_v2(const BatchArgs *__restrict__ A, const int *__restrict__ dead) { SNES_BATCH_XCD; if (bb.y < a.Pc.G.nscales && a.Pc.G.sw[bb.y] >= 64) sparse_v2_body<false>(a.Pc, bb.y, bb.x); }
+__global__ __launch_bounds__(64) void kb_sparse_h2m(const BatchArgs *__restrict__ A, const int *__restrict__ dead) { SNES_BATCH_XCD; sparse_h2_dispatch<false, true>(a.Pc, bb.y, bb.x, (int)gridDim.x); }
+__global__ __launch_bounds__(64) void kb_sparse_h2_listsm(const BatchArgs *__restrict__ A, const int *__restrict__ dead, int list0) { SNES_BATCH_XCD; sparse_h2_dispatch<false, true>(a.Pc, list0 + bb.y, bb.x, (int)gridDim.x); }
+__global__ __launch_bounds__(64) void kb_sparse_h2qm(const BatchArgs *__restrict__ A, const int *__restrict__ dead) { SNES_BATCH_XCD; sparse_h2q_dispatch<false, true>(a.Pc, bb.y, bb.x, (int)gridDim.x); }
+__global__ __launch_bounds__(256, 5) void kb_sparse_v2_scalesm(const BatchArgs *__restrict__ A, const int *__restrict__ dead, int s0) { SNES_BATCH_XCD; const int s = s0 + bb.y; if (s < a.Pc.G.nscales && a.Pc.G.sw[s] >= 64) sparse_v2_body<false, true>(a.Pc, s, bb.x); }
+__global__ __launch_bounds__(256, 5) void kb_sparse_v2m(const BatchArgs *__restrict__ A, const int *__restrict__ dead) { SNES_BATCH_XCD; if (bb.y < a.Pc.G.nscales && a.Pc.G.sw[bb.y] >= 64) sparse_v2_body<false, true>(a.Pc, bb.y, bb.x); }
 __global__ __launch_bounds__(256) void kb_sparse_v_base(const BatchArgs *__restrict__ A, const int *__restrict__ dead) { SNES_BATCH_XCD; if (bb.y < a.Pb.G.nscales && a.Pb.G.sw[bb.y] >= 64) sparse_v2_body<true>(a.Pb, bb.y, bb.x); }
 __global__ __launch_bounds__(128) void kb_sparse_v_base_split(const BatchArgs *__restrict__ A, const int *__restrict__ dead) {
     SNES_BATCH_IMG;
diff --git a/snesimage_amd/csrc/kernels_sparse.hpp b/snesimage_amd/csrc/kernels_sparse.hpp
--- a/snesimage_amd/csrc/kernels_sparse.hpp
+++ b/snesimage_amd/csrc/kernels_sparse.hpp
@@ -46,6 +46,7 @@
     int *first;
     const int *order;
     const int *holder; int list0;
+    int xyb_masks;
 };
 
 __device__ __forceinline__ uint32_t sparse_ci(uint32_t lo, uint32_t thr, uint32_t crgb, uint32_t ncol) {
diff --git a/snesimage_amd/csrc/kernels_sparse2.hpp b/snesimage_amd/csrc/kernels_sparse2.hpp
--- a/snesimage_amd/csrc/kernels_sparse2.hpp
+++ b/snesimage_amd/csrc/kernels_sparse2.hpp
@@ -25,9 +25,9 @@
     long long hbase[16], xbase[16];
 };
 __device__ __forceinline__ void lds_order() { asm volatile("s_waitcnt lgkmcnt(0)" ::: "memory"); }
-template <bool BASE>
+template <bool BASE, bool NOMAPS = false>
 __device__ __forceinline__ void h2_resolve(const SparseParams &P, const uint4 pa, const uint4 pb, const uint32_t bw, const int g, const uint32_t crgb, uint32_t (&ci)[4]) {
-    if (P.use_maps) resolve4_maps(pa.x, pa.y, BASE ? 0xffffffffu : P.slot_ci, (uint32_t)P.ncol, ci);
+    if (!NOMAPS && P.use_maps) resolve4_maps(pa.x, pa.y, BASE ? 0xffffffffu : P.slot_ci, (uint32_t)P.ncol, ci);
     else if (P.perceptual && !BASE) {
         const uint32_t b4 = (bw >> ((g & 7) << 2)) & 0xfu;
         ci[0] = (b4 & 1u) ? (uint32_t)P.ncol : (pa.x >> 24); ci[1] = (b4 & 2u) ? (uint32_t)P.ncol : (pa.z >> 24);
@@ -38,9 +38,10 @@
         ci[2] = sparse_ci(pb.x, pb.y & never, crgb, (uint32_t)P.ncol); ci[3] = sparse_ci(pb.z, pb.w & never, crgb, (uint32_t)P.ncol);
     }
 }
-template <bool S0, bool BASE>
+template <bool S0, bool BASE, bool MK = false>
 __device__ __forceinline__ void sparse_h2_body(const SparseParams &P, const int list, const int bx, const int gx, H2Shared &sh) {
-    constexpr int NP = (S0 || !BASE) ? 4 : 3;
+    static_assert(!MK || (S0 && !BASE), "won-pixel masks: the candidates' scale 0 only");
+    constexpr int NP = ((S0 || !BASE) && !MK) ? 4 : 3;
     constexpr int PW = 32;
     constexpr int ISTR = NP * PW + 4;
     extern __shared__ float s_lut[];
@@ -64,6 +65,12 @@
     const int half = lane >> 5, fl = lane & 31, fp = fl >> 3, fc = fl & 7;
     float *const trash = P.trash + (lane << 2);
     const float4 zero4 = make_float4(0.f, 0.f, 0.f, 0.f);
+    int rd_it[3]; uint32_t rd_lds[3], rd_off[3];
+#pragma unroll
+    for (int m = 0; m < 3; m++) {
+        const int n = m * 64 + lane, ri = (n * 171) >> 12, w = n - ri * 24;
+        rd_it[m] = ri; rd_lds[m] = (uint32_t)(ri * ISTR + w * 4); rd_off[m] = (uint32_t)(w >> 3) * 4u * (uint32_t)W + (uint32_t)((w & 7) << 2);
+    }
     for (int i0 = bx * 16; i0 < count; i0 += gx * 16) {
         const int qi = i0 + (lane >> 2);
         const bool valid = qi < count;
@@ -75,12 +82,15 @@
         const uint32_t crgb = (S0 && !BASE) ? __float_as_uint(P.cand_tab[8 * (size_t)k + 6]) : 0u;
         const float4 *in1 = reinterpret_cast<const float4 *>(P.img1C4 + G.src_off[s] + (size_t)ch * ns) + y;
         const uint4 *pk = S0 ? reinterpret_cast<const uint4 *>(P.packC4) + 2 * (size_t)y : nullptr;
-        const bool um = S0 && P.use_maps;
+        const bool um = S0 && !MK && P.use_maps;
         const uint32_t *mw = um ? reinterpret_cast<const uint32_t *>(BASE ? P.bmapC4 : P.mapsC4 + (size_t)(k - P.k0) * ns) + y : nullptr;
         const uint32_t *sw = um ? reinterpret_cast<const uint32_t *>(P.subC4) + y : nullptr;
         const uint32_t *bmrow = (S0 && P.perceptual && !BASE && !um) ? P.bitmap + (size_t)k * (G.W * G.H / 32) + (size_t)y * (W >> 5) : reinterpret_cast<const uint32_t *>(P.img1C4);
         const float4 *in2 = S0 ? nullptr
                                : reinterpret_cast<const float4 *>(P.store + (size_t)k * P.S.cand_stride + P.S.off_xybC[s] + (size_t)j * 12 * W + (size_t)ch * 4 * W) + r;
+        unsigned char *const mrow = (MK && valid) ? reinterpret_cast<unsigned char *>(P.store + (size_t)k * P.S.cand_stride + P.S.off_xybR[s] + (size_t)j * 12 * W + (size_t)ch * 4 * W) + 8 * r
+                                                  : reinterpret_cast<unsigned char *>(P.trash) + lane;
+        uint32_t mh = 0u;
         lds_order();
         if (r == 0) {
             s_hbase[lane >> 2] = valid ? (long long)k * P.S.cand_stride + P.S.off_hout[s] + (long long)j * 36 * W + (long long)(ch * 3) * 4 * W : -1ll;
@@ -108,12 +118,13 @@
                 wbm = bmrow[q >> 3];
             } else d2 = in2[(size_t)q * 4];
         };
-        auto convert = [&](const int g, const uint4 wa, const uint4 wb, const uint32_t wbm, float4 &d2) {
+        auto convert = [&](const int g, const uint4 wa, const uint4 wb, const uint32_t wbm, float4 &d2, uint32_t &won) {
             uint32_t ci[4];
-            h2_resolve<BASE>(P, wa, wb, wbm, g, crgb, ci);
+            h2_resolve<BASE, MK>(P, wa, wb, wbm, g, crgb, ci);
             const float *lut = s_lut + ch * lstr;
             d2.x = ci[0] == (uint32_t)P.ncol ? cand_v : lut[ci[0]]; d2.y = ci[1] == (uint32_t)P.ncol ? cand_v : lut[ci[1]];
             d2.z = ci[2] == (uint32_t)P.ncol ? cand_v : lut[ci[2]]; d2.w = ci[3] == (uint32_t)P.ncol ? cand_v : lut[ci[3]];
+            if (MK) won = (ci[0] == (uint32_t)P.ncol ? 1u : 0u) | (ci[1] == (uint32_t)P.ncol ? 2u : 0u) | (ci[2] == (uint32_t)P.ncol ? 4u : 0u) | (ci[3] == (uint32_t)P.ncol ? 8u : 0u);
         };
         if (gs > 0) {
             uint4 ta[3], tb[3]; uint32_t tw[3];
@@ -121,7 +132,7 @@
             for (int a = 0; a < 3; a++) { ta[a] = make_uint4(0, 0, 0, 0); tb[a] = ta[a]; tw[a] = 0u; fetch(gs - 3 + a, r1[3 + a], r2[3 + a], ta[a], tb[a], tw[a]); }
             if (S0) {
 #pragma unroll
-                for (int a = 0; a < 3; a++) convert(gs - 3 + a, ta[a], tb[a], tw[a], r2[3 + a]);
+                for (int a = 0; a < 3; a++) { uint32_t wn_; convert(gs - 3 + a, ta[a], tb[a], tw[a], r2[3 + a], wn_); }
             }
         }
         fetch(gs, r1[0], r2[0], pa[0], pb[0], bw[0]);
@@ -131,8 +142,9 @@
             constexpr int sl_ = (T) % 6, sf_ = ((T) + 2) % 6, ua_ = ((T) + 3) % 6, ub_ = ((T) + 4) % 6, ul_ = ((T) + 5) % 6; \
             constexpr int wc_ = (T) % 3, wf_ = ((T) + 2) % 3;                                                                 \
             { const int qf_ = min(g + 2, G4 - 1); fetch(qf_, r1[sf_], r2[sf_], pa[wf_], pb[wf_], bw[wf_]); }                  \
+            uint32_t won_ = 0u;                                                                                               \
             if (g >= G4) { r1[sl_] = zero4; r2[sl_] = zero4; }                                                                \
-            else if (S0) convert(g, pa[wc_], pb[wc_], bw[wc_], r2[sl_]);                                                      \
+            else if (S0) convert(g, pa[wc_], pb[wc_], bw[wc_], r2[sl_], won_);                                                \
             if (BASE && g > 0 && (g & 15) == 0 && g < G4 && valid) {                \
                 float *co = P.ckh + P.S.off_ckh[s] + ((size_t)(ch * 3 + (g >> 4) - 1) * 18) * H + y;                          \
                 _Pragma("unroll") for (int p = 0; p < 3; p++)                                                                 \
@@ -158,6 +170,20 @@
                  \
                                                               \
                 const uint32_t o_l = ((NP == 4 && fp == 3) ? 0u : (uint32_t)fp * 4u * (uint32_t)W) + (uint32_t)((g - 2) << 4) + (uint32_t)(fc << 2); \
+                if (MK) {           \
+                    _Pragma("unroll") for (int mb = 0; mb < 2; mb++) {                                                        \
+                        float4 fv[3]; long long fb[3];                                                                        \
+                        _Pragma("unroll") for (int m = 0; m < 3; m++) {                                                       \
+                            fv[m] = *reinterpret_cast<const float4 *>(s_out + rd_lds[m] + mb * 8 * ISTR);                     \
+                            fb[m] = s_hbase[rd_it[m] + mb * 8];                                                               \
+                        }                                                                                                     \
+                        _Pragma("unroll") for (int m = 0; m < 3; m++) {                                                       \
+                            float *dst = fb[m] >= 0 ? P.store + fb[m] + rd_off[m] + (uint32_t)((g - 2) << 4) : trash;         \
+                            *reinterpret_cast<float4 *>(dst) = fv[m];                                                         \
+                        }                                                                                                     \
+                    }                                                                                                         \
+                    mrow[(((g - 2) >> 4) << 5) + (((g - 2) & 15) >> 1)] = (unsigned char)mh;                                  \
+                } else {                                                                                                      \
                 _Pragma("unroll") for (int mb = 0; mb < 16; mb += 8) {                                                        \
                     float4 fv[4]; long long fb[4];                                                                            \
                     _Pragma("unroll") for (int m = 0; m < 4; m++) {                                                           \
@@ -169,9 +195,10 @@
                         float *dst = (fb[m] >= 0 && fl < NP * 8) ? P.store + fb[m] + o_l : trash;                             \
                         *reinterpret_cast<float4 *>(dst) = fv[m];                                                             \
                     }                                                                                                         \
-                }                                                                                                             \
+                } }                                                                                                           \
                 asm volatile("" ::: "memory");                 \
             }                                                                                                                 \
+            if (MK) mh = (mh >> 4) | (won_ << 4);                                                                             \
         }
         { const int g = gs; SNES_H2_ITER(0, false, false) }
         for (int g0 = gs + 1; g0 <= G4; g0 += 6) {
@@ -186,9 +213,10 @@
     }
 }
 
-template <bool S0, bool BASE>
+template <bool S0, bool BASE, bool MK = false>
 __device__ __forceinline__ void sparse_h2q_body(const SparseParams &P, const int list, const int bx, const int gx, H2Shared &sh) {
-    constexpr int NP = (S0 || !BASE) ? 4 : 3, PW = 32, ISTR = 4 * PW + 4;
+    static_assert(!MK || (S0 && !BASE), "won-pixel masks: the candidates' scale 0 only");
+    constexpr int NP = ((S0 || !BASE) && !MK) ? 4 : 3, PW = 32, ISTR = 4 * PW + 4;
     extern __shared__ float s_lut[];
     const int lstr = P.ncol + 2;
     float *const s_out = sh.out;
@@ -222,12 +250,15 @@
         const uint32_t crgb = (S0 && !BASE) ? __float_as_uint(P.cand_tab[8 * (size_t)k + 6]) : 0u;
         const float4 *in1 = reinterpret_cast<const float4 *>(P.img1C4 + G.src_off[s] + (size_t)ch * ns) + y;
         const uint4 *pk = S0 ? reinterpret_cast<const uint4 *>(P.packC4) + 2 * (size_t)y : nullptr;
-        const bool um = S0 && P.use_maps;
+        const bool um = S0 && !MK && P.use_maps;
         const uint32_t *mw = um ? reinterpret_cast<const uint32_t *>(BASE ? P.bmapC4 : P.mapsC4 + (size_t)(k - P.k0) * ns) + y : nullptr;
         const uint32_t *sw = um ? reinterpret_cast<const uint32_t *>(P.subC4) + y : nullptr;
         const uint32_t *bmrow = (S0 && P.perceptual && !BASE && !um) ? P.bitmap + (size_t)k * (G.W * G.H / 32) + (size_t)y * (W >> 5) : reinterpret_cast<const uint32_t *>(P.img1C4);
         const float4 *in2 = S0 ? nullptr
                                : reinterpret_cast<const float4 *>(P.store + (size_t)k * P.S.cand_stride + P.S.off_xybC[s] + (size_t)j * 12 * W + (size_t)ch * 4 * W) + r;
+        unsigned char *const mrow = (MK && valid) ? reinterpret_cast<unsigned char *>(P.store + (size_t)k * P.S.cand_stride + P.S.off_xybR[s] + (size_t)j * 12 * W + (size_t)ch * 4 * W) + 8 * r
+                                                  : reinterpret_cast<unsigned char *>(P.trash) + lane;
+        uint32_t mh = 0u;
         lds_order();
         if ((lane & 15) == 0) {
             s_hbase[im] = valid ? (long long)k * P.S.cand_stride + P.S.off_hout[s] + (long long)j * 36 * W + (long long)(ch * 3) * 4 * W : -1ll;
@@ -253,12 +284,13 @@
                 wbm = bmrow[qq >> 3];
             } else d2 = in2[(size_t)qq * 4];
         };
-        auto convert = [&](const int g, const uint4 wa, const uint4 wb, const uint32_t wbm, float4 &d2) {
+        auto convert = [&](const int g, const uint4 wa, const uint4 wb, const uint32_t wbm, float4 &d2, uint32_t &won) {
             uint32_t ci[4];
-            h2_resolve<BASE>(P, wa, wb, wbm, g, crgb, ci);
+            h2_resolve<BASE, MK>(P, wa, wb, wbm, g, crgb, ci);
             const float *lut = s_lut + ch * lstr;
             d2.x = ci[0] == (uint32_t)P.ncol ? cand_v : lut[ci[0]]; d2.y = ci[1] == (uint32_t)P.ncol ? cand_v : lut[ci[1]];
             d2.z = ci[2] == (uint32_t)P.ncol ? cand_v : lut[ci[2]]; d2.w = ci[3] == (uint32_t)P.ncol ? cand_v : lut[ci[3]];
+            if (MK) won = (ci[0] == (uint32_t)P.ncol ? 1u : 0u) | (ci[1] == (uint32_t)P.ncol ? 2u : 0u) | (ci[2] == (uint32_t)P.ncol ? 4u : 0u) | (ci[3] == (uint32_t)P.ncol ? 8u : 0u);
         };
         if (gs > 0) {
             uint4 ta[3], tb[3]; uint32_t tw[3];
@@ -266,7 +298,7 @@
             for (int a = 0; a < 3; a++) { ta[a] = make_uint4(0, 0, 0, 0); tb[a] = ta[a]; tw[a] = 0u; fetch(gs - 3 + a, r1[3 + a], r2[3 + a], ta[a], tb[a], tw[a]); }
             if (S0) {
 #pragma unroll
-                for (int a = 0; a < 3; a++) convert(gs - 3 + a, ta[a], tb[a], tw[a], r2[3 + a]);
+                for (int a = 0; a < 3; a++) { uint32_t wn_; convert(gs - 3 + a, ta[a], tb[a], tw[a], r2[3 + a], wn_); }
             }
         }
         fetch(gs, r1[0], r2[0], pa[0], pb[0], bw[0]);
@@ -276,8 +308,9 @@
             constexpr int sl_ = (T) % 6, sf_ = ((T) + 2) % 6, ua_ = ((T) + 3) % 6, ub_ = ((T) + 4) % 6, ul_ = ((T) + 5) % 6; \
             constexpr int wc_ = (T) % 3, wf_ = ((T) + 2) % 3;                                                                 \
             { const int qf_ = min(g + 2, G4 - 1); fetch(qf_, r1[sf_], r2[sf_], pa[wf_], pb[wf_], bw[wf_]); }                  \
+            uint32_t won_ = 0u;                                                                                               \
             if (g >= G4) { r1[sl_] = zero4; r2[sl_] = zero4; }                                                                \
-            else if (S0) convert(g, pa[wc_], pb[wc_], bw[wc_], r2[sl_]);                                                      \
+            else if (S0) convert(g, pa[wc_], pb[wc_], bw[wc_], r2[sl_], won_);                                                \
             if (BASE && q < 3 && g > 0 && (g & 15) == 0 && g < G4 && valid) {  \
                 float *co = P.ckh + P.S.off_ckh[s] + ((size_t)(ch * 3 + (g >> 4) - 1) * 18) * H + y;                          \
                 _Pragma("unroll") for (int e = 0; e < 3; e++) { co[(size_t)(pl * 6 + e) * H] = sa[e]; co[(size_t)(pl * 6 + 3 + e) * H] = sb[e]; } \
@@ -301,6 +334,7 @@
             if (FLUSH) {                                                                                                      \
                 lds_order();                                                                                                  \
                 const uint32_t o_l = ((fp == 3) ? 0u : (uint32_t)fp * 4u * (uint32_t)W) + (uint32_t)((g - 2) << 4) + (uint32_t)(fc << 2); \
+                if (MK) mrow[(((g - 2) >> 4) << 5) + (((g - 2) & 15) >> 1)] = (unsigned char)mh;                              \
                 float4 fv[2]; long long fb[2];                                                                                \
                 _Pragma("unroll") for (int m = 0; m < 2; m++) {                                                               \
                     const int im_ = 2 * m + half;                                                                             \
@@ -309,10 +343,11 @@
                 }                                                                                                             \
                 _Pragma("unroll") for (int m = 0; m < 2; m++) {                                                               \
                     float *dst = (fb[m] >= 0 && fl < NP * 8) ? P.store + fb[m] + o_l : trash;                                 \
-                    *reinterpret_cast<float4 *>(dst) = fv[m];                                                                 \
+                    if (!MK || fl < NP * 8) *reinterpret_cast<float4 *>(dst) = fv[m];  \
                 }                                                                                                             \
                 asm volatile("" ::: "memory");                                                                               \
             }                                                                                                                 \
+            if (MK) mh = (mh >> 4) | (won_ << 4);                                                                             \
         }
         { const int g = gs; SNES_H2Q_ITER(0, false, false) }
         for (int g0 = gs + 1; g0 <= G4; g0 += 6) {
@@ -326,12 +361,12 @@
 #undef SNES_H2Q_ITER
     }
 }
-template <bool BASE>
+template <bool BASE, bool MKD = false>
 __device__ __forceinline__ void sparse_h2q_dispatch(const SparseParams &P, const int list, const int bx, const int gx) {
     const int s = list / kColBuckets;
     if (s >= P.G.nscales || P.G.sw[s] < 64 || (list % kColBuckets) >= (P.G.sw[s] >> 6)) return;
     __shared__ H2Shared sh;
-    if (s == 0) sparse_h2q_body<true, BASE>(P, list, bx, gx, sh); else sparse_h2q_body<false, BASE>(P, list, bx, gx, sh);
+    if (s == 0) sparse_h2q_body<true, BASE, MKD>(P, list, bx, gx, sh); else sparse_h2q_body<false, BASE>(P, list, bx, gx, sh);
 }
 
 __device__ __forceinline__ int uni(int v) { return __builtin_amdgcn_readfirstlane(v); }
@@ -352,8 +387,18 @@
     return make_double2(__hiloint2double((int)v.y, (int)v.x), __hiloint2double((int)v.w, (int)v.z));
 }
 
-template <bool BASE>
+typedef unsigned long long mask4_t __attribute__((ext_vector_type(4), aligned(4)));
+typedef const __attribute__((address_space(4))) mask4_t *mask4_ptr;
+__device__ __forceinline__ void mask_sel4(const mask4_t m, const float won_v, float (&x)[4]) {
+    unsigned long long ex;
+    asm("s_mov_b64 %4, exec\n\ts_mov_b64 exec, %5\n\tv_mov_b32 %0, %9\n\ts_mov_b64 exec, %6\n\tv_mov_b32 %1, %9\n\t"
+        "s_mov_b64 exec, %7\n\tv_mov_b32 %2, %9\n\ts_mov_b64 exec, %8\n\tv_mov_b32 %3, %9\n\ts_mov_b64 exec, %4"
+        : "+v"(x[0]), "+v"(x[1]), "+v"(x[2]), "+v"(x[3]), "=&s"(ex) : "s"(m.x), "s"(m.y), "s"(m.z), "s"(m.w), "s"(won_v));
+}
+
+template <bool BASE, bool MK = false>
 __device__ __forceinline__ void sparse_v2_body(const SparseParams &P, const int s, const int bx) {
+    static_assert(!MK || !BASE, "won-pixel masks: the candidates' sweeps only");
     __shared__ short s_slot[4][64];
     __shared__ __attribute__((aligned(16))) unsigned char s_raw[(2 + 3) * 3 * 256 * sizeof(float2)];
     double (*red)[6] = reinterpret_cast<double (*)[6]>(s_raw);
@@ -394,6 +439,11 @@
     const rsrc_t sd1_b = make_rsrc(P.sd1R4 + G.src_off[s] + (size_t)ch * ns + (size_t)xw * 4);
     const rsrc_t a1_b = make_rsrc(P.a1R4 + G.src_off[s] + (size_t)ch * ns + (size_t)xw * 4);
     const rsrc_t r1_b = make_rsrc(P.r1R4 + G.src_off[s] + (size_t)ch * ns + (size_t)xw * 4);
+    const bool mk = MK && P.xyb_masks && s == 0;
+    const float cand_v = mk ? P.cand_tab[8 * (size_t)k + 3 + ch] : 0.0f;
+    const unsigned long long m_own = (unsigned long long)(store_k + P.S.off_xybR[s] + (size_t)ch * 4 * W) + (unsigned long long)((xw >> 6) << 5);
+    const unsigned long long m_zero = (unsigned long long)P.zeros;
+    mask4_t c_mk = {0ull, 0ull, 0ull, 0ull};
     const uint32_t l4 = (uint32_t)lane << 2, l8 = (uint32_t)lane << 3, l16 = (uint32_t)lane << 4, l32 = (uint32_t)lane << 5;
     const uint32_t W16 = (uint32_t)W * 16u;
 
@@ -420,7 +470,7 @@
 #pragma unroll
         for (int q = 0; q < 6; q++) acc[q] = ld_at<double>(ca + (size_t)q * W, l8);
     }
-#define SNES_HLOAD(GG, DST)                                                                                                   \
+#define SNES_HLOAD(GG, DST, SLOT)            \
     {                                                                                                                         \
         const int gg_ = (GG);                                                                                                 \
         const bool below_ = gg_ >= H4;                                                                                        \
@@ -428,6 +478,7 @@
         const rsrc_t r_ = below_ ? h_zero : (sl_ >= 0 ? h_own : h_b);                                                         \
         const uint32_t so_ = below_ ? 0u : (uint32_t)(sl_ >= 0 ? sl_ : gg_) * 9u * W16;                                       \
         DST[0] = buf_ld4(r_, l16, so_); DST[1] = buf_ld4(r_, l16, so_ + W16); DST[2] = buf_ld4(r_, l16, so_ + 2u * W16);      \
+        SLOT = below_ ? -1 : sl_;                                                                                             \
     }
     const float4 zero4 = make_float4(0.f, 0.f, 0.f, 0.f);
     float2 *ring_xy = reinterpret_cast<float2 *>(s_raw) + t;
@@ -436,11 +487,14 @@
     float4 t1[3] = {zero4, zero4, zero4}, t2[3] = {zero4, zero4, zero4}, t3[3] = {zero4, zero4, zero4};
 #pragma unroll
     for (int p = 0; p < 3; p++) { bufA[p] = zero4; bufB[p] = zero4; }
+    int sl_g = -1, sl_gm = -1;
     if (gs <= H4) {
-        if (gs < H4) SNES_HLOAD(gs, bufA)
-        if (gs - 1 >= 0) SNES_HLOAD(gs - 1, t1)
-        if (gs - 2 >= 0) SNES_HLOAD(gs - 2, t2)
-        if (gs - 3 >= 0) SNES_HLOAD(gs - 3, t3)
+        int sl_t;
+        if (gs < H4) SNES_HLOAD(gs, bufA, sl_g)
+        if (gs - 1 >= 0) SNES_HLOAD(gs - 1, t1, sl_t)
+        if (gs - 2 >= 0) SNES_HLOAD(gs - 2, t2, sl_t)
+        if (gs - 3 >= 0) SNES_HLOAD(gs - 3, t3, sl_t)
+        (void)sl_t;
     }
 #pragma unroll
     for (int p = 0; p < 3; p++) {
@@ -458,7 +512,8 @@
             _Pragma("unroll") for (int q = 0; q < 6; q++) ck_a[(size_t)q * W] = acc[q];                                       \
             ck_f += (size_t)18 * W; ck_a += (size_t)6 * W;                                                                    \
         }                                                                                                                     \
-        SNES_HLOAD(g + 1, NXT)                                                                                                \
+        int sl_nx;                                                                                                            \
+        SNES_HLOAD(g + 1, NXT, sl_nx)                                                                                         \
                 \
         float4 c_m1, c_sd1, c_a1, c_x;                                                                                        \
         double2 c_ra, c_rb;                                                                                                   \
@@ -467,8 +522,9 @@
             const uint32_t go = (uint32_t)gm * W16;                                                                           \
             c_m1 = buf_ld4(m1_b, l16, go); c_sd1 = buf_ld4(sd1_b, l16, go); c_a1 = buf_ld4(a1_b, l16, go);                    \
             c_ra = buf_ld2d(r1_b, l32, 2u * go); c_rb = buf_ld2d(r1_b, l32 + 16u, 2u * go);                                   \
-            const int sl = uni((int)s_slot[wv][gm]);                                                                          \
-            c_x = buf_ld4(sl >= 0 ? x_own : x_b, l16, (uint32_t)(sl >= 0 ? sl : gm) * 3u * W16);                              \
+            const int sl = sl_gm;                                                                                             \
+            const bool xo = sl >= 0 && !mk;                                       \
+            c_x = buf_ld4(xo ? x_own : x_b, l16, (uint32_t)(xo ? sl : gm) * 3u * W16);                                        \
         }                                                                                                                     \
         float outp[3][4];                                                                                                     \
         _Pragma("unroll") for (int p = 0; p < 3; p++) {                                                                       \
@@ -483,13 +539,22 @@
         }                                                                                                                     \
           \
         asm volatile("" : "+v"(c_a1.x), "+v"(c_a1.y), "+v"(c_a1.z), "+v"(c_a1.w));                                            \
+        float i2v[4] = {c_x.x, c_x.y, c_x.z, c_x.w};                                                                          \
+        if (MK) {                                                                                                             \
+            mask_sel4(c_mk, cand_v, i2v);                                                                                     \
+               \
+                                                         \
+            const unsigned long long ma_ = (mk && sl_g >= 0) ? m_own + (unsigned long long)((uint32_t)sl_g * 3u * W16) : m_zero; \
+            c_mk = *reinterpret_cast<volatile const __attribute__((address_space(4))) mask4_t *>(ma_);                        \
+        }                                                                                                                     \
         if (g >= 1) {                                                                                                         \
             const float m1v[4] = {c_m1.x, c_m1.y, c_m1.z, c_m1.w}, sd1v[4] = {c_sd1.x, c_sd1.y, c_sd1.z, c_sd1.w};              \
-            const float a1v[4] = {c_a1.x, c_a1.y, c_a1.z, c_a1.w}, i2v[4] = {c_x.x, c_x.y, c_x.z, c_x.w};                     \
+            const float a1v[4] = {c_a1.x, c_a1.y, c_a1.z, c_a1.w};                                                            \
             const double r1v[4] = {c_ra.x, c_ra.y, c_rb.x, c_rb.y};                                                           \
             _Pragma("unroll") for (int q = 0; q < 4; q++)                                                                     \
                 maps_accumulate(acc, m1v[q], sd1v[q], a1v[q], r1v[q], outp[0][q], outp[1][q], outp[2][q], i2v[q]);            \
         }                                                                                                                     \
+        sl_gm = sl_g; sl_g = sl_nx;                                                                                           \
         r2 ^= 1; r3 = r3 == 2 ? 0 : r3 + 1;                                                                                   \
     }
     for (int g = gs; g <= H4; g++) {
@@ -621,15 +686,18 @@
 #undef SNES_HSTEP
 #undef SNES_VSTEP
 
-template <bool BASE>
+template <bool BASE, bool MKD = false>
 __device__ __forceinline__ void sparse_h2_dispatch(const SparseParams &P, const int list, const int bx, const int gx) {
     const int s = list / kColBuckets;
     if (s >= P.G.nscales || P.G.sw[s] < 64 || (list % kColBuckets) >= (P.G.sw[s] >> 6)) return;
     __shared__ H2Shared sh;
-    if (s == 0) sparse_h2_body<true, BASE>(P, list, bx, gx, sh); else sparse_h2_body<false, BASE>(P, list, bx, gx, sh);
+    if (s == 0) sparse_h2_body<true, BASE, MKD>(P, list, bx, gx, sh); else sparse_h2_body<false, BASE>(P, list, bx, gx, sh);
 }
 __global__ __launch_bounds__(64) void k_sparse_h2(SparseParams P) { sparse_h2_dispatch<false>(P, (int)blockIdx.y, (int)blockIdx.x, (int)gridDim.x); }
 __global__ __launch_bounds__(64) void k_sparse_h2_from(SparseParams P, int list0) { sparse_h2_dispatch<false>(P, list0 + (int)blockIdx.y, (int)blockIdx.x, (int)gridDim.x); }
+__global__ __launch_bounds__(64) void k_sparse_h2m(SparseParams P) { sparse_h2_dispatch<false, true>(P, (int)blockIdx.y, (int)blockIdx.x, (int)gridDim.x); }
+__global__ __launch_bounds__(64) void k_sparse_h2qm(SparseParams P) { sparse_h2q_dispatch<false, true>(P, (int)blockIdx.y, (int)blockIdx.x, (int)gridDim.x); }
+__global__ __launch_bounds__(256, 5) void k_sparse_v2m(SparseParams P) { if ((int)blockIdx.y < P.G.nscales && P.G.sw[blockIdx.y] >= 64) sparse_v2_body<false, true>(P, (int)blockIdx.y, (int)blockIdx.x); }
 __global__ __launch_bounds__(64) void k_sparse_h2q(SparseParams P) { sparse_h2q_dispatch<false>(P, (int)blockIdx.y, (int)blockIdx.x, (int)gridDim.x); }
 __global__ __launch_bounds__(64) void k_sparse_h2q_base(SparseParams P) { sparse_h2q_dispatch<true>(P, (int)blockIdx.y, (int)blockIdx.x, (int)gridDim.x); }
 __global__ __launch_bounds__(64) void k_sparse_h2_base(SparseParams P) { sparse_h2_dispatch<true>(P, (int)blockIdx.y, (int)blockIdx.x, (int)gridDim.x); }
```

New measurement: 3.005 million, median of 5. +2.7%, better.
